# Wuziyi616/SlotDiffusion

Measured on AMD Instinct MI355X. Metric: train-step images/sec, 128x128 7-slot (DPM-Solver denoise-steps/sec in `denoise`), higher is better.
Workload: dtype bf16; 1 GPU; BASELINE configs[1]: img_based SlotDiffusion, CLEVRTex 128x128, 7 slots: train step = slot encoder + frozen VQ-VAE encode + q-sample + UNet eps + MSE, backward, clip, Adam (dropout 0.1); batch_per_gpu=64, hip_graph=True, parallelism=dp1

## Files before the change

### include/sdmi.h

```cpp
#ifndef SDMI_H_
#define SDMI_H_

#ifdef __cplusplus
extern "C" {
#endif

#define SDMI_VERSION 100

enum { SDMI_F32 = 0, SDMI_BF16 = 1, SDMI_FP8 = 2  };
enum { SDMI_ACT_NONE = 0, SDMI_ACT_RELU = 1, SDMI_ACT_SILU = 2, SDMI_ACT_GELU = 3 };
enum { SDMI_OK = 0, SDMI_EINVAL = -1, SDMI_ELAUNCH = -2, SDMI_EUNSUPPORTED = -3 };

int sdmi_version(void);
const char* sdmi_last_error(void);

typedef struct {
  const void* a;
  const void* w;
  void* out;
  const float* bias;
  const float* rowvec;
  const void* residual;
  float* workspace;
  int dtype, out_dtype;
  int M, N, K;
  int lda, ldw, ldc, ldr;
  int B, H, W, Cin, Ho, Wo, KH, KW, stride, pad_t, pad_l, ups;
  int act;
  float alpha;
  int bias_m;
  int split_k;
  int batch;
  int ldrv;
  int zins;
  long long sa, sw, sc, sr;
  int oH, oW, osy, osx, ooy, oox;
  const float* ln_colsum;
  float ln_eps;
  int geglu;
  const void* a2;
  int lda2, K1;
  const void* a3;
  int lda3, K2;
  int softmax8;
  long long s_colsum, s_bias;
  void* out2;
  int ldc2;
  int defer_epilogue;
  float* gn_part;
  int gn_groups;
  const float* alpha_dev;
  int parity4;
} SdmiGemmArgs;
int sdmi_igemm(const SdmiGemmArgs* a, void* stream);
int sdmi_igemm_split_plan(const SdmiGemmArgs* a, void* stream);
int sdmi_splitk_finish(const SdmiGemmArgs* a, void* stream);
enum {
  SDMI_ROUTE_NONE = 0,
  SDMI_ROUTE_CFG = 1,
  SDMI_ROUTE_DMA = 2,
  SDMI_ROUTE_SYM = 3,
  SDMI_ROUTE_HALO = 4,
  SDMI_ROUTE_C64 = 5
};
int sdmi_igemm_last_route(void);

typedef struct {
  const void* a;
  const void* dy;
  float* dw;
  float* dbias;
  float* workspace;
  int dtype;
  int M, N, K, lda, ldy;
  int B, H, W, Cin, Ho, Wo, KH, KW, stride, pad_t, pad_l, ups;
  int splits;
  int accumulate;
  int defer_fold;
} SdmiWgradArgs;
int sdmi_wgrad(const SdmiWgradArgs* a, void* stream);
enum {
  SDMI_WGRAD_KERNEL_IGEMM = 0,
  SDMI_WGRAD_KERNEL_C64 = 1,
  SDMI_WGRAD_KERNEL_HALO = 2,
  SDMI_WGRAD_KERNEL_F32_T128 = 3,
  SDMI_WGRAD_KERNEL_F32_T64 = 4
};
int sdmi_wgrad_kernel(const SdmiWgradArgs* a, void* stream);
int sdmi_wgrad_route(const SdmiWgradArgs* a, void* stream);

typedef struct { const void* problems; int n; } SdmiWgradGroupArgs;
int sdmi_wgrad_group(const SdmiWgradGroupArgs* a, void* stream);
int sdmi_wgrad_fold_group(const SdmiWgradGroupArgs* a, void* stream);

typedef struct {
  const void* dgrad; const void* wgrad; const void* fold;
  int dgrad_cap, wgrad_tile;
} SdmiBwdPairArgs;
int sdmi_bwd_pair(const SdmiBwdPairArgs* a, void* stream);
int sdmi_bwd_pair_route(const SdmiBwdPairArgs* a, void* stream);

typedef struct {
  const void* x;
  void* y;
  const float* gamma;
  const float* beta;
  float* stats;
  float* partial;
  int dtype;
  int B, HW, C, groups;
  float eps;
  int act;
  int nsplit;
  const void* residual;
  float drop_p;
  long long drop_seed;
  const long long* drop_seed_dev;
  void* y8;
  float y8_scale;
  const void* x2;
  int C1;
  const float* part;
  int part_splits;
  float part_alpha;
  const float* part_bias;
  const float* part_rowvec;
  int part_ldrv;
  const void* part_residual;
  void* raw_out;
} SdmiGroupNormArgs;
int sdmi_groupnorm_stats(const SdmiGroupNormArgs* a, void* stream);
int sdmi_groupnorm_apply(const SdmiGroupNormArgs* a, void* stream);
int sdmi_groupnorm(const SdmiGroupNormArgs* a, void* stream);

typedef struct {
  const void* x;
  const void* dy;
  void* dx;
  const float* gamma;
  const float* beta;
  const float* stats;
  float* dgamma;
  float* dbeta;
  float* partial;
  int dtype;
  int B, HW, C, groups;
  int act;
  int nsplit;
  const void* residual;
  void* dresidual;
  int accumulate;
  const void* dextra0;
  const void* dextra1;
  float drop_p;
  long long drop_seed;
  const long long* drop_seed_dev;
  float* dxsum;
  int ld_dxsum;
  int defer_colsum;
} SdmiGroupNormBwdArgs;
int sdmi_groupnorm_bwd(const SdmiGroupNormBwdArgs* a, void* stream);
int sdmi_groupnorm_bwd_fused(const SdmiGroupNormBwdArgs* a, void* unused);
int sdmi_groupnorm_bwd_entries(const SdmiGroupNormBwdArgs* a, void* stream);

typedef struct {
  const void* x; void* y; const float* gamma; const float* beta;
  float* stats;
  int dtype; int rows, C, ldx, ldy; float eps;
} SdmiLayerNormArgs;
int sdmi_layernorm(const SdmiLayerNormArgs* a, void* stream);

typedef struct {
  const void* x; const void* dy; void* dx; const float* gamma; const float* stats;
  float* dgamma; float* dbeta;
  float* partial;
  int dtype; int rows, C; int nblk; int accumulate;
  const void* dextra;
  int defer_colsum;
} SdmiLayerNormBwdArgs;
int sdmi_layernorm_bwd(const SdmiLayerNormBwdArgs* a, void* stream);

typedef struct { const float* partial; float* out0; float* out1; int nblk, C; } SdmiColsumItem;
typedef struct { const void* items; int n; } SdmiColsumGroupArgs;
int sdmi_colsum_group(const SdmiColsumGroupArgs* a, void* stream);


typedef struct {
  const void* q; const void* k; const void* v; void* out; float* lse;
  int dtype; int B, heads, Sq, Skv; int ldq, ldk, ldv, ldo; float scale;
  int head_dim;
} SdmiAttnArgs;
int sdmi_attention(const SdmiAttnArgs* a, void* stream);

typedef struct {
  const void* q; const void* k; const void* v; const void* out; const void* dout; const float* lse;
  void* dq; void* dk; void* dv;
  int dtype; int B, heads, Sq, Skv; int ldq, ldk, ldv, ldo; float scale;
  int head_dim;
} SdmiAttnBwdArgs;
int sdmi_attention_bwd(const SdmiAttnBwdArgs* a, void* stream);

typedef struct { void* x; int dtype; int rows, cols, ld; float scale; } SdmiSoftmaxArgs;
int sdmi_softmax_rows(const SdmiSoftmaxArgs* a, void* stream);

typedef struct {
  const void* k; const void* v;
  const float* slots_in;
  float* slots_out;
  float* seg;
  const float *lnq_g, *lnq_b, *wq;
  const float *w_ih, *w_hh, *b_ih, *b_hh;
  const float *lnm_g, *lnm_b, *w1, *b1, *w2, *b2;
  float* trace;
  int dtype; int B, M, N, D, Hid, iters, ldkv; long long slots_bstride; float eps, scale;
} SdmiSlotAttnArgs;
int sdmi_slot_attention(const SdmiSlotAttnArgs* a, void* stream);

typedef struct {
  const float* z; const float* codebook; long long* idx; float* zq;
  int R, dim, ldz, n_codes; float scale;
  const float* z2; float zc0, zc1, zdiv;
} SdmiVqArgs;
int sdmi_vq_nearest(const SdmiVqArgs* a, void* stream);

enum { SDMI_DPM_EPS = 0, SDMI_DPM_X0 = 1, SDMI_DPM_V = 2 };
enum { SDMI_DPM_UPD_NONE = 0, SDMI_DPM_UPD_FIRST = 1, SDMI_DPM_UPD_SINGLE = 2, SDMI_DPM_UPD_MULTI2 = 3,
       SDMI_DPM_UPD_MULTI3 = 4 };
typedef struct {
  const float* x; const float* out; const float* codebook;
  long long* idx; float* m0;
  const float* base; const float* h1; const float* h2; float* y;
  int R, n_codes, target, mode;
  float scale, sigma, alpha;
  float c0, c1, c2, c3, k0, k1, g, k2;
} SdmiDpmStepArgs;
int sdmi_dpm_step(const SdmiDpmStepArgs* a, void* stream);

typedef struct {
  const float* x; const float* out; const float* codebook;
  long long* idx; float* m0;
  int R, n_codes, target;
  float scale, sigma, alpha;
// ... 373 lines not shown
```

### slotdiffusion_amd/bwd.py

```python
import ctypes
from typing import NamedTuple, Optional

import torch

from . import _lib

_DT = {torch.float32: _lib.F32, torch.bfloat16: _lib.BF16}


def _p(t):
    return 0 if t is None else t.data_ptr()


def _st():
    return torch.cuda.current_stream().cuda_stream


def _cdiv(a, b):
    return (a + b - 1) // b


class LayerProblem(NamedTuple):
    is_conv: bool
    B: int
    H: int
    W: int
    Ho: int
    Wo: int
    Cin: int
    N: int
    K: int
    M: int
    kh: int
    kw: int
    stride: int
    pad: tuple
    ups: bool
    lda: int
    ldy: int
    dt: torch.dtype

    @classmethod
    def of(cls, x, dy, geom, dt, N):
        kh, kw, stride, pad, ups = geom
        Cin = x.shape[-1]
        if x.dim() == 4 and (kh, kw) != (0, 0):
            return cls.conv(x.shape[0], x.shape[1], x.shape[2], dy.shape[1], dy.shape[2], Cin, N, dy.shape[-1], kh, kw,
                            stride, pad, dt, ups)
        rows = x.numel() // Cin
        return cls(False, rows, 1, 1, 1, 1, Cin, N, Cin, rows, 1, 1, 1, (0, 0, 0, 0), False, x.stride(-2), dy.shape[-1], dt)

    @classmethod
    def conv(cls, B, H, W, Ho, Wo, Cin, N, ldy, kh, kw, stride, pad, dt, ups=False):
        return cls(True, B, H, W, Ho, Wo, Cin, N, kh * kw * Cin, B * Ho * Wo, kh, kw, stride, tuple(pad), bool(ups), Cin,
                   ldy, dt)

    @classmethod
    def transposed(cls, x, Cout, k, stride, pad):
        B, H, W, Cin = x.shape
        Ho = (H - 1) * stride - 2 * pad + k + (stride - 1)
        Wo = (W - 1) * stride - 2 * pad + k + (stride - 1)
        return cls.conv(B, Ho, Wo, H, W, Cout, Cin, Cin, k, k, stride, (pad,) * 4, x.dtype)

    @classmethod
    def upsampled(cls, x, Cout):
        B, H, W, Cin = x.shape
        return cls.conv(B, 2 * H, 2 * W, H, W, Cout, Cin, Cin, 4, 4, 2, (1, 1, 1, 1), x.dtype)

    def wgrad_fields(self):
        return dict(dtype=_DT[self.dt], M=self.M, N=self.N, K=self.K, lda=self.lda, ldy=self.ldy, B=self.B, H=self.H,
                    W=self.W, Cin=self.Cin, Ho=self.Ho, Wo=self.Wo, KH=self.kh, KW=self.kw, stride=self.stride,
                    pad_t=self.pad[0], pad_l=self.pad[2], ups=int(self.ups))

    def dgrad_fields(self):
        Hs, Ws = (2 * self.H, 2 * self.W) if self.ups else (self.H, self.W)
        kd = self.kh * self.kw * self.ldy
        return dict(dtype=_DT[self.dt], out_dtype=_DT[self.dt], M=self.B * Hs * Ws, N=self.Cin, K=kd, lda=self.ldy, ldw=kd,
                    ldc=self.Cin, B=self.B, H=self.Ho, W=self.Wo, Cin=self.ldy, Ho=Hs, Wo=Ws, KH=self.kh, KW=self.kw,
                    stride=1, pad_t=self.kh - 1 - self.pad[0], pad_l=self.kw - 1 - self.pad[2], ups=0, act=0, alpha=1.0,
                    batch=1, zins=(self.stride if self.stride > 1 else 0), ldr=self.Cin)

    def parity_dgrads(self):
        s, kh, kw, pad = self.stride, self.kh, self.kw, self.pad
        full = all(len(range((p + pd) % s, k, s)) > 0 for k, pd in ((kh, pad[0]), (kw, pad[2])) for p in range(s))
        subs = []
        for py in range(s):
            ay = (py + pad[0]) % s
            nky, hs = len(range(ay, kh, s)), len(range(py, self.H, s))
            for px in range(s):
                ax = (px + pad[2]) % s
                nkx, ws = len(range(ax, kw, s)), len(range(px, self.W, s))
                if nky == 0 or nkx == 0 or hs == 0 or ws == 0:
                    continue
                K = nky * nkx * self.ldy
                subs.append(((kh - 1 - ay) % s, (kw - 1 - ax) % s, dict(
                    dtype=_DT[self.dt], out_dtype=_DT[self.dt], M=self.B * hs * ws, N=self.Cin, K=K, lda=self.ldy, ldw=K,
                    ldc=self.Cin, B=self.B, H=self.Ho, W=self.Wo, Cin=self.ldy, Ho=hs, Wo=ws, KH=nky, KW=nkx, stride=1,
                    pad_t=(nky - 1) - (py + pad[0] - ay) // s, pad_l=(nkx - 1) - (px + pad[2] - ax) // s, ups=0, act=0,
                    alpha=1.0, batch=1, oH=self.H, oW=self.W, osy=s, osx=s, ooy=py, oox=px, ldr=self.Cin)))
        return full, subs


WG_TARGET, MIN_STEPS, MAX_SPLITS = 192, 8, 512
PAIR_SLOTS, PAIR_DGRAD, PAIR_MIN_STEPS, PAIR_WT64 = 512, 256, 8, 96
WQ_TARGET, WQ_MAX_SPLITS = 512.0, 64


class PairPlan(NamedTuple):
    wgrad_tile: int
    dgrad_cap: int
    splits: int


class LayerPlan(NamedTuple):
    path: str
    splits: int
    kernel: str
    pair: Optional[PairPlan]


def _mstep(P):
    return 64 if P.dt == torch.bfloat16 else 32


def standalone_splits(P):
    tiles = _cdiv(P.N, 128) * _cdiv(P.K, 128)
    return max(1, min(_cdiv(WG_TARGET, tiles), P.M // (MIN_STEPS * _mstep(P)), MAX_SPLITS))


def _standalone(P, n_cus, wgrad_halo):
    splits = 1 if P.M <= 16 * _mstep(P) else standalone_splits(P)
    same3x3 = (P.dt == torch.bfloat16 and P.is_conv and P.kh == 3 and P.kw == 3 and P.stride == 1 and not P.ups
               and P.pad == (1, 1, 1, 1))
    if (same3x3 and P.Cin == 64 and P.N == 64 and P.W % 64 == 0 and P.H % 4 == 0
            and P.B * (P.H // 4) * (P.W // 64) >= 2 * n_cus):
        return n_cus, 'c64'
    hw = P.H * P.W
    if (same3x3 and wgrad_halo and P.W in (16, 32, 64) and P.Cin % 64 == 0 and P.N % 64 == 0 and P.Ho == P.H
            and P.Wo == P.W and hw % 256 == 0 and (hw & (hw - 1)) == 0):
        pairs = (P.N // 64) * (P.Cin // 64)
        halo = min(n_cus // pairs, P.M // 256)
        if halo >= 2 and pairs * halo >= 128:
            return halo, 'halo'
    return splits, 'gemm'


def _pairable(P, direct, has_bias, bias_dst, dalias_cols):
    kh, kw, pad = P.kh, P.kw, P.pad
    same = P.is_conv and P.stride == 1 and not P.ups and P.Ho == P.H and P.Wo == P.W
    one = kh == 1 and kw == 1 and P.stride == 1 and not P.ups and pad[0] == 0 and pad[2] == 0
    kd = kh * kw * P.ldy
    bk = 64 if kd * 2 >= 512 else 32
    return (P.dt == torch.bfloat16 and direct and P.N > 64 and P.K > 64 and P.Cin > 64
            and (not has_bias or bias_dst) and P.Cin % 8 == 0 and P.ldy % 8 == 0
            and (one or (same and kh * kw <= 32 and P.ldy % bk == 0
                         and pad[0] == pad[1] == (kh - 1) // 2 and pad[2] == pad[3] == (kw - 1) // 2))
            and (dalias_cols is None or dalias_cols == P.Cin)
            and (P.M + (kh + 1) * P.W + 128) * max(P.lda, P.ldy, P.Cin) * 2 < (1 << 31) and P.N * kd * 2 < (1 << 31))


def _pair_plan(P, has_bias):
    Md, Nd, Kd = P.B * P.H * P.W, P.Cin, P.kh * P.kw * P.ldy
    t128 = _cdiv(Md, 128) * _cdiv(Nd, 128)
    shallow = P.kh == 1 and P.kw == 1 and Kd * 2 <= 512
    big = t128 >= 192 and not shallow
    tiles_d = t128 if big else _cdiv(Md, 64) * _cdiv(Nd, 64)
    steps = _cdiv(P.M, 64)

    def plan(wt, slots, min_steps):
        tn = _cdiv(P.N, wt)
        tiles_w = tn * _cdiv(P.K, wt) + (tn if has_bias else 0)
        n_d = min(tiles_d, PAIR_DGRAD)
        return tiles_w, n_d, max(1, min((slots - n_d) // tiles_w, steps // min_steps, 256))
    wt = 128
    tiles_w, n_d, splits = plan(128, PAIR_SLOTS, PAIR_MIN_STEPS)
    if not big and PAIR_WT64 and tiles_w * splits < PAIR_WT64:
        wt = 64
        tiles_w, n_d, splits = plan(64, PAIR_SLOTS * 3 // 2, max(2, PAIR_MIN_STEPS // 2))
    return PairPlan(wt, _cdiv(n_d, 8) * 8, splits)


def plan_layer(P, *, need_dx, direct, has_bias, bias_dst, dalias_cols, n_cus, pair_bwd=True, wgrad_halo=True):
    splits, kernel = _standalone(P, n_cus, wgrad_halo)
    if pair_bwd and need_dx and _pairable(P, direct, has_bias, bias_dst, dalias_cols):
        return LayerPlan('pair', splits, kernel, _pair_plan(P, has_bias))
    return LayerPlan('side', splits, kernel, None)


def plan_group(problems):
    tiles = [_cdiv(P.N, 128) * (_cdiv(P.K, 128) + (1 if bias else 0)) for P, bias in problems]
    steps = [_cdiv(P.M, 64) for P, _ in problems]
    total = float(sum(t * st for t, st in zip(tiles, steps)))
    return [max(1, min(max(1, int(round(WQ_TARGET * (t * st) / total / t))), st // MIN_STEPS, WQ_MAX_SPLITS))
            for t, st in zip(tiles, steps)]


class GradSchedule:
    N_SIDE = 4

    def __init__(self, overlap):
        self.overlap = overlap
        self._sides, self._side_of = [], {}
        self._keep = []
        self._pfold = None
        self._side_dst = {}
        self._cq, self._cq_after = [], []
        self._groups = 0
        self._join_queued = False

    def _side_stream(self, key):
        if not self.overlap:
            return None
        if not self._sides:
            self._sides = [torch.cuda.Stream() for _ in range(self.N_SIDE)]
        i = self._side_of.get(key)
        if i is None:
            i = self._side_of[key] = len(self._side_of) % self.N_SIDE
        return self._sides[i]

    def _fold_first(self, dst_ptrs=None):
        pf = self._pfold
        if pf is None:
            return
        if dst_ptrs is not None and pf[0]['dw'] not in dst_ptrs and (not pf[0]['dbias'] or pf[0]['dbias'] not in dst_ptrs):
            return
        self._pfold = None
        self._after_side_writers(pf[0]['dw'], pf[0]['dbias'])
        arr = _lib.struct_array('SdmiWgradArgs', [pf[0]])
        _lib.call('sdmi_wgrad_fold_group', _st(), problems=ctypes.addressof(arr), n=1)

    def _after_side_writers(self, *ptrs):
        for p_ in ptrs:
            side = self._side_dst.pop(p_, None) if p_ else None
            if side is not None:
                torch.cuda.current_stream().wait_stream(side)

    def _on_side(self, side, launch, dst_ptrs):
        if side is None:
            launch()
            return
        ev = torch.cuda.Event()
        ev.record()
        side.wait_event(ev)
        with torch.cuda.stream(side):
            launch()
        for p_ in dst_ptrs:
            if p_:
                self._side_dst[p_] = side

    def _ensure_join(self):
        if not self._join_queued:
            self._join_queued = True
            torch.autograd.Variable._execution_engine.queue_callback(self.join)

    def join_by_hand(self):
        self._join_queued = True

    def launch_pair(self, P, plan, dgrad, wgrad, device):
        N, K, splits = P.N, P.K, plan.splits
        self._fold_first((wgrad['dw'], wgrad['dbias']))
        self._after_side_writers(wgrad['dw'], wgrad['dbias'])
        ws = torch.empty((splits * (N * K + N),), dtype=torch.float32, device=device) if splits > 1 else None
        pf, self._pfold = self._pfold, None
        if pf is not None:
            self._after_side_writers(pf[0]['dw'], pf[0]['dbias'])
# ... 80 lines not shown
```

### slotdiffusion_amd/csrc/bwd_pair.hip

```cpp
#include "common.h"
#include "igemm_body.h"
#include "wgrad_body.h"

namespace {

struct PairGeom {
  int n_fold, n_wgrad, d_begin, n_dgrad;
  int w_tiles_n, w_tiles_k, w_per_split, w_mps;
  int d_tiles_m, d_tiles_n, d_ktps, d_hw_shift;
};

constexpr int pair_wg_lds(int wt) { return 2 * 64 * (wt * 2 + 64 + wt * 2 + 64); }

template <int BM, int BN, int BKB, int MODE, int WT>
__global__ __launch_bounds__(512) __attribute__((amdgpu_waves_per_eu(4, 4))) void bwd_pair_kernel(
    SdmiGemmArgs d, SdmiWgradArgs w, SdmiWgradArgs f, PairGeom g) {
  const int b = (int)blockIdx.x;
  if (b < g.n_fold) {
    wgrad_reduce_body<512>(f, b, g.n_fold);
    return;
  }
  if (b < g.n_fold + g.n_wgrad) {
    const int j = b - g.n_fold;
    const int xc = j & 7, q8 = g.n_wgrad >> 3, r8 = g.n_wgrad & 7;
// ... 2 lines not shown
    wgrad_tr_body<WT, WT, MODE>(w, g.w_tiles_n, g.w_tiles_k, g.w_mps, idx - split * g.w_per_split, split);
    return;
  }
  if (b < g.d_begin) return;
  igemm_body<bf16_t, BM, BN, BKB, MODE>(d, g.d_tiles_m, g.d_tiles_n, g.d_ktps, g.d_hw_shift, b - g.d_begin,
                                        g.n_dgrad, 0);
}

template <int BM, int BN, int BKB, int MODE, int WT>
int launch_pair(const SdmiGemmArgs& d, const SdmiWgradArgs& w, const SdmiWgradArgs* f, int dgrad_cap,
                int hw_shift, hipStream_t st) {
  constexpr int BK = BKB / 2;
  constexpr int d_lds = 2 * (BM + BN) * (BKB + 16);
  constexpr int smem = d_lds > pair_wg_lds(WT) ? d_lds : pair_wg_lds(WT);
  auto kern = bwd_pair_kernel<BM, BN, BKB, MODE, WT>;
  SDMI_OPTIN_LDS(kern, smem, "bwd_pair");
  PairGeom g;
  SdmiWgradArgs fz = {};
  if (f) {
    fz = *f;
    const long long v4 = (long long)f->N * f->K / 4 * wgrad_fold_lanes(f->splits);
    long long nf = (v4 + 512 * 4 - 1) / (512 * 4);
    g.n_fold = (int)(nf < 1 ? 1 : (nf > 128 ? 128 : nf));
  } else {
    g.n_fold = 0;
  }
  g.w_tiles_n = (w.N + WT - 1) / WT;
  g.w_tiles_k = (w.K + WT - 1) / WT;
  g.w_per_split = g.w_tiles_n * g.w_tiles_k + (w.dbias ? g.w_tiles_n : 0);
  int mps = (w.M + w.splits - 1) / w.splits;
  g.w_mps = (mps + 63) / 64 * 64;
  g.n_wgrad = g.w_per_split * w.splits;
  g.d_begin = (g.n_fold + g.n_wgrad + 7) & ~7;
  g.d_tiles_m = (d.M + BM - 1) / BM;
  g.d_tiles_n = (d.N + BN - 1) / BN;
  g.d_ktps = (d.K + BK - 1) / BK;
  g.d_hw_shift = hw_shift;
  const int tiles = g.d_tiles_m * g.d_tiles_n;
  constexpr int SLOTS = smem <= 49152 ? 768 : 512;
  int cap = dgrad_cap > 0 ? dgrad_cap : SLOTS - g.d_begin;
  cap = cap < 64 ? 64 : (cap > SLOTS ? SLOTS : cap);
  cap &= ~7;
  g.n_dgrad = tiles <= cap ? tiles : cap;
  SdmiGemmArgs q = d;
  q.split_k = 1;
  hipLaunchKernelGGL(kern, dim3(g.d_begin + g.n_dgrad), dim3(512), smem, st, q, w, fz, g);
  return sdmi_check_launch("bwd_pair");
}

struct PairRoute { int bm, bn, bkb, mode, wt, hw_shift; };

#define PAIR_REQUIRE(cond, msg)              \
  do {                                       \
    if (!(cond)) {                           \
      sdmi_set_error("%s: %s", who, msg);    \
      return SDMI_EINVAL;                    \
    }                                        \
  } while (0)
int pair_route(const SdmiBwdPairArgs* a, PairRoute& route, const char* who) {
  PAIR_REQUIRE(a && a->dgrad && a->wgrad, "null pointer");
  const SdmiGemmArgs& d = *(const SdmiGemmArgs*)a->dgrad;
  const SdmiWgradArgs& w = *(const SdmiWgradArgs*)a->wgrad;
  const SdmiWgradArgs* f = (const SdmiWgradArgs*)a->fold;
  PAIR_REQUIRE(d.a && d.w && d.out && w.a && w.dy && w.dw, "null operand");
  PAIR_REQUIRE(d.dtype == SDMI_BF16 && d.out_dtype == SDMI_BF16 && w.dtype == SDMI_BF16, "bf16 operands only");
  const bool d1x1 = d.KH == 1 && d.KW == 1 && d.stride == 1 && d.pad_t == 0 && d.pad_l == 0 && !d.ups && d.zins <= 1;
  const bool dplain = !d1x1 && !d.ups && d.zins <= 1 && d.stride == 1;
  PAIR_REQUIRE(d1x1 || dplain, "data gradient: 1x1 or plain stride-1 convolution");
  PAIR_REQUIRE(d.M > 0 && d.N > 64 && d.K > 0 && d.K == d.KH * d.KW * d.Cin && d.M == d.B * d.Ho * d.Wo, "bad dgrad geometry");
  PAIR_REQUIRE(d.Cin % 8 == 0 && d.lda % 8 == 0 && d.ldw % 8 == 0 && ((uintptr_t)d.a & 15) == 0 && ((uintptr_t)d.w & 15) == 0,
               "dgrad operands must keep 16-byte vectors");
  PAIR_REQUIRE(!d.a2 && !d.ln_colsum && !d.geglu && !d.softmax8 && !d.out2 && d.osy == 0 && !(d.batch > 1) && !d.rowvec &&
               !d.bias_m && d.split_k <= 1, "data gradient: plain epilogue (alpha, bias, residual) only");
  const long long a_bytes = ((long long)d.B * d.H * d.W + (long long)(d.KH + 1) * d.W) * d.lda * 2;
  PAIR_REQUIRE(a_bytes < (1ll << 31) && (long long)d.N * d.ldw * 2 < (1ll << 31), "dgrad operands beyond 31-bit offsets");
  const bool w1x1 = w.KH == 1 && w.KW == 1 && w.stride == 1 && w.pad_t == 0 && w.pad_l == 0 && !w.ups && w.H == w.Ho &&
                    w.W == w.Wo;
  const bool wlin = !w1x1 && !w.ups && w.stride == 1 && w.H == w.Ho && w.W == w.Wo;
  PAIR_REQUIRE((d1x1 && w1x1) || (dplain && wlin), "both gradients must be 1x1, or both a stride-1 same-size convolution");
  PAIR_REQUIRE(w.N > 64 && w.K > 64 && w.K == w.KH * w.KW * w.Cin && w.M == w.B * w.Ho * w.Wo && w.Cin % 8 == 0 &&
               w.lda % 8 == 0 && w.ldy % 8 == 0, "bad wgrad geometry");
  PAIR_REQUIRE(w.splits >= 1 && (w.splits == 1 || w.workspace), "splits > 1 need a workspace");
  const long long mps = ((long long)w.M + w.splits - 1) / w.splits + 64;
  const long long ld = w.lda > w.ldy ? w.lda : w.ldy;
  PAIR_REQUIRE((mps + (long long)(w.KH + 1) * w.W + 64) * ld * 2 < (1ll << 31), "wgrad split beyond 31-bit offsets");
  if (f) PAIR_REQUIRE(f->dw && f->workspace && f->splits > 1 && f->N > 0 && f->K > 0 && ((long long)f->N * f->K) % 4 == 0 &&
                      f->dw != w.dw && (!f->dbias || f->dbias != w.dbias), "bad fold problem (or it targets this layer's dW)");
  int hw_shift = -1;
  {
    const int hw = d.Ho * d.Wo;
    if (hw > 0 && (hw & (hw - 1)) == 0) {
      hw_shift = 0;
      while ((1 << hw_shift) < hw) ++hw_shift;
    }
  }
  const long long t128 = (long long)((d.M + 127) / 128) * ((d.N + 127) / 128);
  bool big = t128 >= 192;
  const int kbytes = d.K * 2;
  if (d1x1 && kbytes <= 512) big = false;
  const bool wide = kbytes >= 512;
  const int bk = (wide ? 128 : 64) / 2;
  if (!d1x1) PAIR_REQUIRE(d.KH * d.KW <= 32 && d.Cin % bk == 0, "convolution data gradient: K tiles must lie inside one filter tap");
  PAIR_REQUIRE(a->wgrad_tile == 0 || a->wgrad_tile == 128 || (a->wgrad_tile == 64 && !big),
               "wgrad_tile: 128, or 64 next to 64 x 64 data-gradient tiles");
  const int t = big ? 128 : 64;
  route = {t, t, wide ? 128 : 64, d1x1 ? 1 : 2, a->wgrad_tile == 64 ? 64 : 128, hw_shift};
  return 0;
}
#undef PAIR_REQUIRE

}

extern "C" int sdmi_bwd_pair(const SdmiBwdPairArgs* a, void* stream) {
  PairRoute r;
  if (const int rc = pair_route(a, r, __func__)) return rc;
  const SdmiGemmArgs& d = *(const SdmiGemmArgs*)a->dgrad;
  const SdmiWgradArgs& w = *(const SdmiWgradArgs*)a->wgrad;
  const SdmiWgradArgs* f = (const SdmiWgradArgs*)a->fold;
  hipStream_t st = (hipStream_t)stream;
#define PAIR_GO(BM, BN, BKB, WT)                                                                       \
  return r.mode == 1 ? launch_pair<BM, BN, BKB, 1, WT>(d, w, f, a->dgrad_cap, r.hw_shift, st)           \
                     : launch_pair<BM, BN, BKB, 2, WT>(d, w, f, a->dgrad_cap, r.hw_shift, st)
  if (r.bm == 128) {
    if (r.bkb == 128) PAIR_GO(128, 128, 128, 128);
    PAIR_GO(128, 128, 64, 128);
  }
  if (r.wt == 64) {
    if (r.bkb == 128) PAIR_GO(64, 64, 128, 64);
    PAIR_GO(64, 64, 64, 64);
  }
  if (r.bkb == 128) PAIR_GO(64, 64, 128, 128);
  PAIR_GO(64, 64, 64, 128);
#undef PAIR_GO
}

extern "C" int sdmi_bwd_pair_route(const SdmiBwdPairArgs* a, void*) {
  PairRoute r;
  if (const int rc = pair_route(a, r, __func__)) return rc;
  return (r.bm / 64) | (r.bn / 64) << 3 | (r.bkb / 64) << 6 | r.mode << 9 | (r.wt / 64) << 12;
}
```

### slotdiffusion_amd/csrc/norm_bwd.hip

```cpp
#include "common.h"
#include "gn_geom.h"
#include "gn_dev.h"
#include <type_traits>

namespace {

__device__ __forceinline__ int next_pow2(int v) {
  int p = 1;
  while (p < v) p <<= 1;
  return p;
}

template <typename T>
__global__ __launch_bounds__(256) void gn_bwd_stats_kernel(SdmiGroupNormBwdArgs p) {
  constexpr int VEC = Elem<T>::VEC;
  __shared__ float part[256][VEC][2];
  const int b = blockIdx.y, split = blockIdx.x;
  const int CV = p.C / VEC, CVp = next_pow2(CV);
  const int R = 256 / CVp;
  const int cv = threadIdx.x % CVp, r0 = threadIdx.x / CVp;
  const int rows_per = (p.HW + p.nsplit - 1) / p.nsplit;
  const int row_begin = split * rows_per;
  int row_end = row_begin + rows_per;
  if (row_end > p.HW) row_end = p.HW;
  const int cpg = p.C / p.groups;
  float A[VEC], Bv[VEC];
#pragma unroll
  for (int j = 0; j < VEC; ++j) A[j] = Bv[j] = 0.f;
  if (cv < CV) {
    float mu[VEC], rs[VEC], ga[VEC], be[VEC];
#pragma unroll
    for (int j = 0; j < VEC; ++j) {
      const int c = cv * VEC + j, g = c / cpg;
      mu[j] = p.stats[(b * p.groups + g) * 2];
      rs[j] = p.stats[(b * p.groups + g) * 2 + 1];
      ga[j] = p.gamma[c];
      be[j] = p.beta[c];
    }
    const long long base = (long long)b * p.HW * p.C + cv * VEC;
    const T* xb = (const T*)p.x + base;
    const T* db = (const T*)p.dy + base;
    const T* rb = p.residual ? (const T*)p.residual + base : nullptr;
    const bool drop = p.drop_p > 0.f;
    const unsigned long long dseed = drop ? sdmi_drop_seed(p.drop_seed, p.drop_seed_dev) : 0ULL;
    const unsigned thr16 = (unsigned)(p.drop_p * 65536.f);
    const float dinv = 1.f / (1.f - p.drop_p);
    for (int row = row_begin + r0; row < row_end; row += R) {
      const long long o = (long long)row * p.C;
      float x[VEC], dy[VEC], rr[VEC];
      unpack16<T>(*reinterpret_cast<const uint4*>(xb + o), x);
      unpack16<T>(*reinterpret_cast<const uint4*>(db + o), dy);
      if (drop) sdmi_drop_apply<VEC>(dy, dseed, (base + o) / VEC, thr16, dinv);
      if (rb) unpack16<T>(*reinterpret_cast<const uint4*>(rb + o), rr);
#pragma unroll
      for (int j = 0; j < VEC; ++j) {
        const float xh = (x[j] - mu[j]) * rs[j];
        const float z = xh * ga[j] + be[j] + (rb ? rr[j] : 0.f);
        const float dz = dy[j] * act_grad<sizeof(T) == 2>(z, p.act);
        A[j] += dz;
        Bv[j] += dz * xh;
      }
    }
  }
#pragma unroll
  for (int j = 0; j < VEC; ++j) { part[threadIdx.x][j][0] = A[j]; part[threadIdx.x][j][1] = Bv[j]; }
  __syncthreads();
  if (r0 == 0 && cv < CV) {
#pragma unroll
    for (int j = 0; j < VEC; ++j) {
      double sa = 0.0, sb = 0.0;
      for (int r = 0; r < R; ++r) { sa += part[r * CVp + cv][j][0]; sb += part[r * CVp + cv][j][1]; }
      float* q = p.partial + ((((long long)b * p.nsplit + split) * p.C) + cv * VEC + j) * 2;
      q[0] = (float)sa;
      q[1] = (float)sb;
    }
  }
}

template <typename T, int THREADS, int NV>
__global__ __launch_bounds__(THREADS) void gn_bwd_fused_kernel(SdmiGroupNormBwdArgs p) {
  constexpr int VEC = Elem<T>::VEC;
  extern __shared__ __attribute__((aligned(16))) float gnb_smem[];
  const int b = blockIdx.x;
  const int S = gridDim.y, sidx = blockIdx.y;
  const int CV = p.C / VEC / S, CVp = next_pow2(CV);
  const int c_lo = sidx * CV * VEC;
  const int R = THREADS / CVp;
  const int RR = CVp < 64 ? THREADS / 64 : R;
  float (*part)[VEC][2] = reinterpret_cast<float (*)[VEC][2]>(gnb_smem);
  float (*gsum)[2] = reinterpret_cast<float (*)[2]>(gnb_smem + RR * CVp * VEC * 2);
  const int cv = threadIdx.x % CVp, r0 = threadIdx.x / CVp;
  const bool act_c = cv < CV;
  const int cpg = p.C / p.groups;
  const int gs = p.groups / S;
  float mu[VEC], rs[VEC], ga[VEC], be[VEC];
#pragma unroll
  for (int j = 0; j < VEC; ++j) {
    const int c = c_lo + (act_c ? cv : 0) * VEC + j, g = c / cpg;
    mu[j] = p.stats[(b * p.groups + g) * 2];
    rs[j] = p.stats[(b * p.groups + g) * 2 + 1];
    ga[j] = p.gamma[c];
    be[j] = p.beta[c];
  }
  const long long base = (long long)b * p.HW * p.C + c_lo + (act_c ? cv : 0) * VEC;
  const T* xb = (const T*)p.x + base;
  const T* db = (const T*)p.dy + base;
  const T* rb = p.residual ? (const T*)p.residual + base : nullptr;
  uint4 xr[NV], dr[NV];
#pragma unroll
  for (int i = 0; i < NV; ++i) {
    const int row = r0 + i * R;
    if (act_c && row < p.HW) {
      xr[i] = *reinterpret_cast<const uint4*>(xb + (long long)row * p.C);
      dr[i] = *reinterpret_cast<const uint4*>(db + (long long)row * p.C);
    }
  }
  float A[VEC], Bv[VEC];
#pragma unroll
  for (int j = 0; j < VEC; ++j) A[j] = Bv[j] = 0.f;
  const bool drop = p.drop_p > 0.f;
  const unsigned long long dseed = drop ? sdmi_drop_seed(p.drop_seed, p.drop_seed_dev) : 0ULL;
  const unsigned thr16 = (unsigned)(p.drop_p * 65536.f);
  const float dinv = 1.f / (1.f - p.drop_p);
#pragma unroll
  for (int i = 0; i < NV; ++i) {
    const int row = r0 + i * R;
    if (act_c && row < p.HW) {
      float x[VEC], dy[VEC], rr[VEC];
      unpack16<T>(xr[i], x);
      unpack16<T>(dr[i], dy);
      if (drop) sdmi_drop_apply<VEC>(dy, dseed, (base + (long long)row * p.C) / VEC, thr16, dinv);
      if (rb) unpack16<T>(*reinterpret_cast<const uint4*>(rb + (long long)row * p.C), rr);
#pragma unroll
      for (int j = 0; j < VEC; ++j) {
        const float xh = (x[j] - mu[j]) * rs[j];
        const float z = xh * ga[j] + be[j] + (rb ? rr[j] : 0.f);
        const float dz = dy[j] * act_grad<sizeof(T) == 2>(z, p.act);
        dy[j] = dz;
        A[j] += dz;
        Bv[j] += dz * xh;
      }
      dr[i] = pack16<T>(dy);
    }
  }
  for (int off = CVp; off < 64; off <<= 1) {
#pragma unroll
    for (int j = 0; j < VEC; ++j) {
      A[j] += __shfl_xor(A[j], off, 64);
      Bv[j] += __shfl_xor(Bv[j], off, 64);
    }
  }
  if (CVp >= 64 || (int)(threadIdx.x & 63) < CVp) {
    const int slot = CVp < 64 ? (threadIdx.x >> 6) * CVp + cv : threadIdx.x;
#pragma unroll
    for (int j = 0; j < VEC; ++j) { part[slot][j][0] = A[j]; part[slot][j][1] = Bv[j]; }
  }
  __syncthreads();
  if (r0 == 0 && act_c) {
#pragma unroll
    for (int j = 0; j < VEC; ++j) {
      double sa = 0.0, sb = 0.0;
      for (int r = 0; r < RR; ++r) { sa += part[r * CVp + cv][j][0]; sb += part[r * CVp + cv][j][1]; }
      part[cv][j][0] = (float)sa;
      part[cv][j][1] = (float)sb;
      float* q = p.partial + (((long long)b * p.C) + c_lo + cv * VEC + j) * 2;
      q[0] = (float)sa;
      q[1] = (float)sb;
    }
  }
  __syncthreads();
  for (int g = threadIdx.x; g < gs; g += THREADS) {
    double s1 = 0.0, s2 = 0.0;
    for (int c = g * cpg; c < (g + 1) * cpg; ++c) {
      s1 += (double)p.gamma[c_lo + c] * part[c / VEC][c % VEC][0];
      s2 += (double)p.gamma[c_lo + c] * part[c / VEC][c % VEC][1];
    }
    gsum[g][0] = (float)s1;
    gsum[g][1] = (float)s2;
  }
  __syncthreads();
  const float inv_n = 1.f / ((float)p.HW * (float)cpg);
  float sd[VEC];
#pragma unroll
  for (int j = 0; j < VEC; ++j) sd[j] = 0.f;
  if (act_c) {
  float s1[VEC], s2[VEC];
#pragma unroll
  for (int j = 0; j < VEC; ++j) {
    const int g = (cv * VEC + j) / cpg;
    s1[j] = gsum[g][0] * inv_n;
    s2[j] = gsum[g][1] * inv_n;
  }
  T* dxb = (T*)p.dx + base;
  T* drb = p.dresidual ? (T*)p.dresidual + base : nullptr;
  const T* e0 = p.dextra0 ? (const T*)p.dextra0 + base : nullptr;
  const T* e1 = p.dextra1 ? (const T*)p.dextra1 + base : nullptr;
#pragma unroll
  for (int i = 0; i < NV; ++i) {
    const int row = r0 + i * R;
    if (row < p.HW) {
      const long long o = (long long)row * p.C;
      float x[VEC], dz[VEC], dx[VEC];
      unpack16<T>(xr[i], x);
      unpack16<T>(dr[i], dz);
#pragma unroll
      for (int j = 0; j < VEC; ++j) {
        const float xh = (x[j] - mu[j]) * rs[j];
        dx[j] = rs[j] * (ga[j] * dz[j] - (s1[j] + xh * s2[j]));
      }
      if (e0) {
        float ex[VEC];
        unpack16<T>(*reinterpret_cast<const uint4*>(e0 + o), ex);
#pragma unroll
        for (int j = 0; j < VEC; ++j) dx[j] += ex[j];
      }
      if (e1) {
        float ex[VEC];
        unpack16<T>(*reinterpret_cast<const uint4*>(e1 + o), ex);
#pragma unroll
        for (int j = 0; j < VEC; ++j) dx[j] += ex[j];
      }
#pragma unroll
      for (int j = 0; j < VEC; ++j) sd[j] += dx[j];
      *reinterpret_cast<uint4*>(dxb + o) = pack16<T>(dx);
      if (drb) *reinterpret_cast<uint4*>(drb + o) = dr[i];
    }
  }
  }
  if (p.dxsum) {
    for (int off = CVp; off < 64; off <<= 1) {
#pragma unroll
      for (int j = 0; j < VEC; ++j) sd[j] += __shfl_xor(sd[j], off, 64);
    }
    __syncthreads();
    if (CVp >= 64 || (int)(threadIdx.x & 63) < CVp) {
      const int slot = CVp < 64 ? (threadIdx.x >> 6) * CVp + cv : threadIdx.x;
#pragma unroll
      for (int j = 0; j < VEC; ++j) part[slot][j][0] = sd[j];
    }
    __syncthreads();
    if (r0 == 0 && act_c) {
#pragma unroll
      for (int j = 0; j < VEC; ++j) {
        float t = 0.f;
        for (int r = 0; r < RR; ++r) t += part[r * CVp + cv][j][0];
        p.dxsum[(long long)b * p.ld_dxsum + c_lo + cv * VEC + j] = t;
      }
    }
  }
}

template <typename T, int THREADS, int NV>
__global__ __launch_bounds__(THREADS) void gn_bwd_fused2_kernel(SdmiGroupNormBwdArgs p) {
  constexpr int VEC = Elem<T>::VEC;
  constexpr int VSH = VEC == 8 ? 3 : 2;
  extern __shared__ __attribute__((aligned(16))) float gnb_smem[];
  const int b = blockIdx.x;
  const int S = gridDim.y, sidx = blockIdx.y;
  const int CV = p.C / VEC / S;
  const int csh = CV <= 1 ? 0 : 32 - __builtin_clz(CV - 1);
  const int CVp = 1 << csh;
  const int c_lo = sidx * CV * VEC;
  const int R = THREADS >> csh;
  const int RR = CVp < 64 ? THREADS / 64 : R;
  float4* part = reinterpret_cast<float4*>(gnb_smem);
  double* colsum = reinterpret_cast<double*>(gnb_smem + RR * CVp * 4);
  float (*chpart)[VEC][2] = reinterpret_cast<float (*)[VEC][2]>(gnb_smem + RR * CVp * 4 + CVp * 8);
  const int tid = threadIdx.x;
  const int cv = tid & (CVp - 1), r0 = tid >> csh;
  const bool act_c = cv < CV;
  const int cvc = act_c ? cv : 0;
  const int cpg = p.C / p.groups;
  const int cl0 = cvc * VEC;
  const int g0 = cl0 / cpg;
  const int bnd = (g0 + 1) * cpg - cl0;
  const long long base = (long long)b * p.HW * p.C + c_lo + cl0;
  const T* xb = (const T*)p.x + base;
  const T* db = (const T*)p.dy + base;
  const T* rb = p.residual ? (const T*)p.residual + base : nullptr;
  uint4 xr[NV], dr[NV];
#pragma unroll
  for (int i = 0; i < NV; ++i) {
    const int row = r0 + i * R;
    if (act_c && row < p.HW) {
      xr[i] = *reinterpret_cast<const uint4*>(xb + (long long)row * p.C);
      dr[i] = *reinterpret_cast<const uint4*>(db + (long long)row * p.C);
    }
  }
  const int gg = b * p.groups + sidx * (p.groups / S) + g0;
  const float2 st0 = *reinterpret_cast<const float2*>(p.stats + gg * 2);
  const float2 st1 = bnd < VEC ? *reinterpret_cast<const float2*>(p.stats + gg * 2 + 2) : st0;
  float ga[VEC], be[VEC];
  load_fvec<VEC>(p.gamma + c_lo + cl0, ga);
  load_fvec<VEC>(p.beta + c_lo + cl0, be);
#define GNB_MU(j) ((j) < bnd ? st0.x : st1.x)
#define GNB_RS(j) ((j) < bnd ? st0.y : st1.y)
  float A[VEC], Bv[VEC];
#pragma unroll
  for (int j = 0; j < VEC; ++j) A[j] = Bv[j] = 0.f;
  const bool drop = p.drop_p > 0.f;
  const unsigned long long dseed = drop ? sdmi_drop_seed(p.drop_seed, p.drop_seed_dev) : 0ULL;
  const unsigned thr16 = (unsigned)(p.drop_p * 65536.f);
  const float dinv = 1.f / (1.f - p.drop_p);
  auto first = [&](auto actc) __attribute__((always_inline)) {
    constexpr int ACT = decltype(actc)::value;
#pragma unroll
    for (int i = 0; i < NV; ++i) {
      const int row = r0 + i * R;
      if (act_c && row < p.HW) {
        float x[VEC], dy[VEC], rr[VEC];
        unpack16<T>(xr[i], x);
        unpack16<T>(dr[i], dy);
        if (drop) sdmi_drop_apply<VEC>(dy, dseed, (base + (long long)row * p.C) / VEC, thr16, dinv);
        if (rb) unpack16<T>(*reinterpret_cast<const uint4*>(rb + (long long)row * p.C), rr);
#pragma unroll
        for (int j = 0; j < VEC; ++j) {
          const float xh = (x[j] - GNB_MU(j)) * GNB_RS(j);
          const float z = xh * ga[j] + be[j] + (rb ? rr[j] : 0.f);
          const float dz = dy[j] * act_grad<sizeof(T) == 2>(z, ACT);
          dy[j] = dz;
          A[j] += dz;
          Bv[j] += dz * xh;
        }
        dr[i] = pack16<T>(dy);
      }
    }
  };
  if (p.act == SDMI_ACT_SILU) first(std::integral_constant<int, SDMI_ACT_SILU>{});
  else if (p.act == SDMI_ACT_RELU) first(std::integral_constant<int, SDMI_ACT_RELU>{});
  else if (p.act == SDMI_ACT_GELU) first(std::integral_constant<int, SDMI_ACT_GELU>{});
  else first(std::integral_constant<int, SDMI_ACT_NONE>{});
  float a0 = 0.f, q0 = 0.f, a1 = 0.f, q1 = 0.f;
#pragma unroll
  for (int j = 0; j < VEC; ++j) {
    const bool lo = j < bnd;
    const float ta = ga[j] * A[j], tb = ga[j] * Bv[j];
    a0 += lo ? ta : 0.f;
    q0 += lo ? tb : 0.f;
    a1 += lo ? 0.f : ta;
    q1 += lo ? 0.f : tb;
  }
  if (CVp < 64) {
    a0 = col_allreduce(a0, CVp);
    q0 = col_allreduce(q0, CVp);
    a1 = col_allreduce(a1, CVp);
    q1 = col_allreduce(q1, CVp);
#pragma unroll
    for (int j = 0; j < VEC; ++j) { A[j] = col_allreduce(A[j], CVp); Bv[j] = col_allreduce(Bv[j], CVp); }
    if ((tid & 63) < CVp) {
      const int e = (tid >> 6) * CVp + cv;
      part[e] = make_float4(a0, q0, a1, q1);
#pragma unroll
      for (int j = 0; j < VEC; ++j) { chpart[e][j][0] = A[j]; chpart[e][j][1] = Bv[j]; }
    }
  } else {
    part[tid] = make_float4(a0, q0, a1, q1);
#pragma unroll
    for (int j = 0; j < VEC; ++j) { chpart[tid][j][0] = A[j]; chpart[tid][j][1] = Bv[j]; }
  }
  __syncthreads();
  if (tid < CVp) {
    double d0 = 0.0, d1 = 0.0, d2 = 0.0, d3 = 0.0;
    for (int r = 0; r < RR; ++r) {
      const float4 v = part[r * CVp + tid];
      d0 += (double)v.x; d1 += (double)v.y; d2 += (double)v.z; d3 += (double)v.w;
    }
    colsum[tid * 4 + 0] = d0; colsum[tid * 4 + 1] = d1; colsum[tid * 4 + 2] = d2; colsum[tid * 4 + 3] = d3;
  }
  for (int u = THREADS - 1 - tid; u < CVp * VEC * 2; u += THREADS) {
    const int ccv = u / (VEC * 2), j = (u >> 1) & (VEC - 1), which = u & 1;
    if (ccv < CV) {
      double sa = 0.0;
      for (int r = 0; r < RR; ++r) sa += (double)chpart[r * CVp + ccv][j][which];
      p.partial[(((long long)b * p.C) + c_lo + ccv * VEC + j) * 2 + which] = (float)sa;
    }
  }
  __syncthreads();
  const float inv_n = 1.f / ((float)p.HW * (float)cpg);
  float s1_[2], s2_[2];
#pragma unroll
  for (int k = 0; k < 2; ++k) {
    if (k == 1 && bnd >= VEC) { s1_[1] = s1_[0]; s2_[1] = s2_[0]; break; }
    const int f = (g0 + k) * cpg, l = f + cpg - 1;
    const int ca = f >> VSH, cb = l >> VSH;
    double sm = 0.0, sq = 0.0;
    for (int c = ca; c <= cb; ++c) {
      const int o = c * 4 + (((c << VSH) >= f) ? 0 : 2);
      sm += colsum[o];
      sq += colsum[o + 1];
    }
    s1_[k] = (float)sm * inv_n;
    s2_[k] = (float)sq * inv_n;
  }
  float sd[VEC];
#pragma unroll
  for (int j = 0; j < VEC; ++j) sd[j] = 0.f;
  if (act_c) {
    T* dxb = (T*)p.dx + base;
    T* drb = p.dresidual ? (T*)p.dresidual + base : nullptr;
    const T* e0 = p.dextra0 ? (const T*)p.dextra0 + base : nullptr;
    const T* e1 = p.dextra1 ? (const T*)p.dextra1 + base : nullptr;
#pragma unroll
    for (int i = 0; i < NV; ++i) {
      const int row = r0 + i * R;
      if (row < p.HW) {
        const long long o = (long long)row * p.C;
        float x[VEC], dz[VEC], dx[VEC];
        unpack16<T>(xr[i], x);
        unpack16<T>(dr[i], dz);
#pragma unroll
        for (int j = 0; j < VEC; ++j) {
          const float rsj = GNB_RS(j);
          const float xh = (x[j] - GNB_MU(j)) * rsj;
          dx[j] = rsj * (ga[j] * dz[j] - ((j < bnd ? s1_[0] : s1_[1]) + xh * (j < bnd ? s2_[0] : s2_[1])));
        }
        if (e0) {
          float ex[VEC];
          unpack16<T>(*reinterpret_cast<const uint4*>(e0 + o), ex);
#pragma unroll
          for (int j = 0; j < VEC; ++j) dx[j] += ex[j];
        }
        if (e1) {
          float ex[VEC];
          unpack16<T>(*reinterpret_cast<const uint4*>(e1 + o), ex);
#pragma unroll
          for (int j = 0; j < VEC; ++j) dx[j] += ex[j];
        }
#pragma unroll
        for (int j = 0; j < VEC; ++j) sd[j] += dx[j];
        *reinterpret_cast<uint4*>(dxb + o) = pack16<T>(dx);
        if (drb) *reinterpret_cast<uint4*>(drb + o) = dr[i];
      }
    }
  }
#undef GNB_MU
#undef GNB_RS
  if (p.dxsum) {
    if (CVp < 64) {
#pragma unroll
      for (int j = 0; j < VEC; ++j) sd[j] = col_allreduce(sd[j], CVp);
    }
    __syncthreads();
    if (CVp >= 64 || (tid & 63) < CVp) {
      const int e = CVp < 64 ? (tid >> 6) * CVp + cv : tid;
#pragma unroll
      for (int j = 0; j < VEC; ++j) chpart[e][j][0] = sd[j];
    }
    __syncthreads();
    for (int u = tid; u < CVp * VEC; u += THREADS) {
      const int ccv = u / VEC, j = u & (VEC - 1);
      if (ccv < CV) {
        float t = 0.f;
        for (int r = 0; r < RR; ++r) t += chpart[r * CVp + ccv][j][0];
        p.dxsum[(long long)b * p.ld_dxsum + c_lo + ccv * VEC + j] = t;
      }
    }
  }
}

__global__ __launch_bounds__(256) void pair_colsum_kernel(const float* partial, int nblk, int C,
                                                          float* out0, float* out1,
                                                          int accumulate) {
  __shared__ float red[16][16][2];
  const int cl = threadIdx.x & 15, kg = threadIdx.x >> 4;
  const int c = blockIdx.x * 16 + cl;
  float s0 = 0.f, s1 = 0.f;
  if (c < C) {
    const float2* q = reinterpret_cast<const float2*>(partial) + c;
    int k = kg;
    for (; k + 48 < nblk; k += 64) {
      const float2 v0 = q[(long long)k * C], v1 = q[(long long)(k + 16) * C];
      const float2 v2 = q[(long long)(k + 32) * C], v3 = q[(long long)(k + 48) * C];
      s0 += (v0.x + v1.x) + (v2.x + v3.x);
      s1 += (v0.y + v1.y) + (v2.y + v3.y);
    }
    for (; k < nblk; k += 16) {
      const float2 v = q[(long long)k * C];
      s0 += v.x;
      s1 += v.y;
    }
  }
  red[kg][cl][0] = s0;
  red[kg][cl][1] = s1;
  __syncthreads();
  if (kg == 0 && c < C) {
    float a = 0.f, b = 0.f;
#pragma unroll
    for (int k = 0; k < 16; ++k) { a += red[k][cl][0]; b += red[k][cl][1]; }
    out0[c] = (accumulate ? out0[c] : 0.f) + a;
    out1[c] = (accumulate ? out1[c] : 0.f) + b;
  }
}

constexpr int CS_MAX = 64;
struct ColsumGroup { int n; SdmiColsumItem it[CS_MAX]; };
__global__ __launch_bounds__(256) void colsum_group_kernel(ColsumGroup g) {
  const SdmiColsumItem& q_ = g.it[blockIdx.y];
  const int C = q_.C, nblk = q_.nblk;
  if ((int)blockIdx.x * 16 >= C) return;
  __shared__ float red[16][16][2];
  const int cl = threadIdx.x & 15, kg = threadIdx.x >> 4;
  const int c = blockIdx.x * 16 + cl;
  float s0 = 0.f, s1 = 0.f;
  const bool two = q_.out1 != nullptr;
  if (c < C && !two) {
    const float* q = q_.partial + c;
    for (int k = kg; k < nblk; k += 16) s0 += q[(long long)k * C];
  } else if (c < C) {
    const float2* q = reinterpret_cast<const float2*>(q_.partial) + c;
    int k = kg;
    for (; k + 48 < nblk; k += 64) {
      const float2 v0 = q[(long long)k * C], v1 = q[(long long)(k + 16) * C];
      const float2 v2 = q[(long long)(k + 32) * C], v3 = q[(long long)(k + 48) * C];
      s0 += (v0.x + v1.x) + (v2.x + v3.x);
      s1 += (v0.y + v1.y) + (v2.y + v3.y);
    }
    for (; k < nblk; k += 16) {
      const float2 v = q[(long long)k * C];
      s0 += v.x;
      s1 += v.y;
    }
  }
  red[kg][cl][0] = s0;
  red[kg][cl][1] = s1;
  __syncthreads();
  if (kg == 0 && c < C) {
    float a = 0.f, b = 0.f;
#pragma unroll
    for (int k = 0; k < 16; ++k) { a += red[k][cl][0]; b += red[k][cl][1]; }
    q_.out0[c] += a;
    if (two) q_.out1[c] += b;
  }
}

template <typename T>
__global__ __launch_bounds__(256) void gn_bwd_apply_kernel(SdmiGroupNormBwdArgs p, int rows_per) {
  constexpr int VEC = Elem<T>::VEC;
  __shared__ float gsum[256][2];
  const int b = blockIdx.y;
  const int cpg = p.C / p.groups;
  {
    const int l8 = threadIdx.x & 7;
    const int ne = cpg * p.nsplit;
    for (int g = threadIdx.x >> 3; g < p.groups; g += 32) {
      double s1 = 0.0, s2 = 0.0;
      for (int e = l8; e < ne; e += 8) {
        const int k = e / cpg, c = g * cpg + (e - k * cpg);
        const float2 v = reinterpret_cast<const float2*>(p.partial)[((long long)b * p.nsplit + k) * p.C + c];
        const double ga = (double)p.gamma[c];
        s1 += ga * v.x;
        s2 += ga * v.y;
      }
      for (int off = 1; off < 8; off <<= 1) {
        s1 += __shfl_xor(s1, off, 64);
        s2 += __shfl_xor(s2, off, 64);
      }
      if (l8 == 0) { gsum[g][0] = (float)s1; gsum[g][1] = (float)s2; }
    }
  }
  __syncthreads();
  const int CV = p.C / VEC, CVp = next_pow2(CV);
  const int R = 256 / CVp;
  const int cv = threadIdx.x % CVp, r0 = threadIdx.x / CVp;
  if (cv >= CV) return;
  const int row_begin = blockIdx.x * rows_per;
  int row_end = row_begin + rows_per;
  if (row_end > p.HW) row_end = p.HW;
  const float inv_n = 1.f / ((float)p.HW * (float)cpg);
  float mu[VEC], rs[VEC], ga[VEC], be[VEC], s1[VEC], s2[VEC];
#pragma unroll
  for (int j = 0; j < VEC; ++j) {
    const int c = cv * VEC + j, g = c / cpg;
    mu[j] = p.stats[(b * p.groups + g) * 2];
    rs[j] = p.stats[(b * p.groups + g) * 2 + 1];
    ga[j] = p.gamma[c];
    be[j] = p.beta[c];
    s1[j] = gsum[g][0] * inv_n;
    s2[j] = gsum[g][1] * inv_n;
  }
  const long long base = (long long)b * p.HW * p.C + cv * VEC;
  const T* xb = (const T*)p.x + base;
  const T* db = (const T*)p.dy + base;
  const T* rb = p.residual ? (const T*)p.residual + base : nullptr;
  T* dxb = (T*)p.dx + base;
  T* drb = p.dresidual ? (T*)p.dresidual + base : nullptr;
  const T* e0 = p.dextra0 ? (const T*)p.dextra0 + base : nullptr;
  const T* e1 = p.dextra1 ? (const T*)p.dextra1 + base : nullptr;
  const bool drop = p.drop_p > 0.f;
  const unsigned long long dseed = drop ? sdmi_drop_seed(p.drop_seed, p.drop_seed_dev) : 0ULL;
  const unsigned thr16 = (unsigned)(p.drop_p * 65536.f);
  const float dinv = 1.f / (1.f - p.drop_p);
  for (int row = row_begin + r0; row < row_end; row += R) {
    const long long o = (long long)row * p.C;
    float x[VEC], dy[VEC], rr[VEC], dx[VEC], dz[VEC];
    unpack16<T>(*reinterpret_cast<const uint4*>(xb + o), x);
    unpack16<T>(*reinterpret_cast<const uint4*>(db + o), dy);
    if (drop) sdmi_drop_apply<VEC>(dy, dseed, (base + o) / VEC, thr16, dinv);
    if (rb) unpack16<T>(*reinterpret_cast<const uint4*>(rb + o), rr);
#pragma unroll
    for (int j = 0; j < VEC; ++j) {
      const float xh = (x[j] - mu[j]) * rs[j];
      const float z = xh * ga[j] + be[j] + (rb ? rr[j] : 0.f);
      dz[j] = dy[j] * act_grad<sizeof(T) == 2>(z, p.act);
      dx[j] = rs[j] * (ga[j] * dz[j] - (s1[j] + xh * s2[j]));
    }
    if (e0) {
      float ex[VEC];
      unpack16<T>(*reinterpret_cast<const uint4*>(e0 + o), ex);
#pragma unroll
      for (int j = 0; j < VEC; ++j) dx[j] += ex[j];
    }
    if (e1) {
      float ex[VEC];
      unpack16<T>(*reinterpret_cast<const uint4*>(e1 + o), ex);
#pragma unroll
      for (int j = 0; j < VEC; ++j) dx[j] += ex[j];
    }
    *reinterpret_cast<uint4*>(dxb + o) = pack16<T>(dx);
    if (drb) *reinterpret_cast<uint4*>(drb + o) = pack16<T>(dz);
  }
}

template <typename T, int VPL>
__global__ __launch_bounds__(256) void ln_bwd_kernel(SdmiLayerNormBwdArgs p, int rows_per_blk,
                                                     int LPR) {
  constexpr int VEC = Elem<T>::VEC;
  __shared__ float red[4][1024][2];
  const int lane = threadIdx.x & 63, wave = threadIdx.x >> 6;
  const int sub = lane & (LPR - 1), slot = lane / LPR, RW = 64 / LPR;
  const int CV = p.C / VEC;
  const int row0 = blockIdx.x * rows_per_blk;
  int row1 = row0 + rows_per_blk;
  if (row1 > p.rows) row1 = p.rows;
  float ga[VPL][VEC], dg[VPL][VEC], dbt[VPL][VEC];
  bool act[VPL];
#pragma unroll
  for (int i = 0; i < VPL; ++i) {
    const int cv = sub + i * LPR;
    act[i] = cv < CV;
#pragma unroll
    for (int j = 0; j < VEC; ++j) {
      ga[i][j] = act[i] ? p.gamma[cv * VEC + j] : 0.f;
      dg[i][j] = dbt[i][j] = 0.f;
    }
  }
  const float invC = 1.f / (float)p.C;
  uint4 xq[VPL], dq[VPL];
  float mean_n = 0.f, rstd_n = 1.f;
  auto fetch = [&](int rbase) __attribute__((always_inline)) {
    const int row = rbase + slot;
    const long long rr = (row < row1) ? row : row0;
    const T* x = (const T*)p.x + rr * p.C;
    const T* dy = (const T*)p.dy + rr * p.C;
    mean_n = p.stats[rr * 2];
    rstd_n = p.stats[rr * 2 + 1];
#pragma unroll
    for (int i = 0; i < VPL; ++i) {
      const int cc = act[i] ? sub + i * LPR : 0;
      xq[i] = *reinterpret_cast<const uint4*>(x + cc * VEC);
      dq[i] = *reinterpret_cast<const uint4*>(dy + cc * VEC);
    }
  };
  if (row0 + wave * RW < row1) fetch(row0 + wave * RW);
  for (int rbase = row0 + wave * RW; rbase < row1; rbase += 4 * RW) {
    const int row = rbase + slot;
    const bool rok = row < row1;
    const long long ro = (long long)(rok ? row : row0) * p.C;
    float xh[VPL][VEC], dxh[VPL][VEC];
    float s1 = 0.f, s2 = 0.f;
    const float mean = mean_n, rstd = rstd_n;
    uint4 xc[VPL], dc[VPL];
#pragma unroll
    for (int i = 0; i < VPL; ++i) { xc[i] = xq[i]; dc[i] = dq[i]; }
    const T* ex = p.dextra ? (const T*)p.dextra + ro : nullptr;
    uint4 eq[VPL];
    if (ex) {
#pragma unroll
      for (int i = 0; i < VPL; ++i) eq[i] = *reinterpret_cast<const uint4*>(ex + (act[i] ? sub + i * LPR : 0) * VEC);
    }
    if (rbase + 4 * RW < row1) fetch(rbase + 4 * RW);
#pragma unroll
    for (int i = 0; i < VPL; ++i) {
      float xv[VEC], dv[VEC];
      unpack16<T>(xc[i], xv);
      unpack16<T>(dc[i], dv);
#pragma unroll
      for (int j = 0; j < VEC; ++j) {
        const float d = (act[i] && rok) ? dv[j] : 0.f;
        xh[i][j] = (xv[j] - mean) * rstd;
        dxh[i][j] = d * ga[i][j];
        dg[i][j] += d * xh[i][j];
        dbt[i][j] += d;
        s1 += dxh[i][j];
        s2 += dxh[i][j] * xh[i][j];
      }
    }
    for (int off = 1; off < LPR; off <<= 1) {
      s1 += __shfl_xor(s1, off, 64);
      s2 += __shfl_xor(s2, off, 64);
    }
    s1 *= invC;
    s2 *= invC;
    if (rok) {
      T* dx = (T*)p.dx + ro;
#pragma unroll
      for (int i = 0; i < VPL; ++i) {
        if (!act[i]) continue;
        float o[VEC];
#pragma unroll
        for (int j = 0; j < VEC; ++j) o[j] = rstd * (dxh[i][j] - s1 - xh[i][j] * s2);
        if (ex) {
          float ev[VEC];
          unpack16<T>(eq[i], ev);
#pragma unroll
          for (int j = 0; j < VEC; ++j) o[j] += ev[j];
        }
        *reinterpret_cast<uint4*>(dx + (sub + i * LPR) * VEC) = pack16<T>(o);
      }
    }
  }
  for (int off = LPR; off < 64; off <<= 1) {
#pragma unroll
    for (int i = 0; i < VPL; ++i)
#pragma unroll
      for (int j = 0; j < VEC; ++j) {
        dg[i][j] += __shfl_xor(dg[i][j], off, 64);
        dbt[i][j] += __shfl_xor(dbt[i][j], off, 64);
      }
  }
  if (slot == 0) {
#pragma unroll
    for (int i = 0; i < VPL; ++i)
      if (act[i]) {
#pragma unroll
        for (int j = 0; j < VEC; ++j) {
          const int c = (sub + i * LPR) * VEC + j;
          red[wave][c][0] = dg[i][j];
          red[wave][c][1] = dbt[i][j];
        }
      }
  }
  __syncthreads();
  for (int c = threadIdx.x; c < p.C; c += 256) {
    float* q = p.partial + ((long long)blockIdx.x * p.C + c) * 2;
    q[0] = (red[0][c][0] + red[1][c][0]) + (red[2][c][0] + red[3][c][0]);
    q[1] = (red[0][c][1] + red[1][c][1]) + (red[2][c][1] + red[3][c][1]);
  }
}
}

extern "C" int sdmi_groupnorm_bwd_fused(const SdmiGroupNormBwdArgs* a, void*) {
  if (!a || a->C <= 0 || a->groups <= 0) return 0;
  const int vec = a->dtype == SDMI_BF16 ? 8 : 4;
  int nv_of_T[3] = {16, 16, a->dtype == SDMI_BF16 ? 4 : 8};
  return gn_pick(a->B, a->HW, a->C, a->groups, vec, nv_of_T).T ? 1 : 0;
}

extern "C" int sdmi_groupnorm_bwd_entries(const SdmiGroupNormBwdArgs* a, void*) {
  if (!a || a->C <= 0 || a->groups <= 0) return 0;
  const int vec = a->dtype == SDMI_BF16 ? 8 : 4;
  int nv_of_T[3] = {16, 16, a->dtype == SDMI_BF16 ? 4 : 8};
  const GnGeom gg = gn_pick(a->B, a->HW, a->C, a->groups, vec, nv_of_T);
  return gg.T ? a->B : a->B * a->nsplit;
}

extern "C" int sdmi_groupnorm_bwd(const SdmiGroupNormBwdArgs* a, void* stream) {
  SDMI_REQUIRE(a && a->x && a->dy && a->dx && a->gamma && a->beta && a->stats && a->dgamma &&
                   a->dbeta && a->partial, "null pointer");
  const int vec = a->dtype == SDMI_BF16 ? 8 : 4;
  SDMI_REQUIRE(a->C % vec == 0 && a->C <= 1024, "C must be a vector multiple <= 1024");
  SDMI_REQUIRE(a->groups > 0 && a->C % a->groups == 0 && a->nsplit >= 1, "bad groups/nsplit");
  hipStream_t st = (hipStream_t)stream;
  dim3 g1(a->nsplit, a->B);
  const long long row_bytes = (long long)a->C * (a->dtype == SDMI_BF16 ? 2 : 4);
  int rows_per = (int)((32768 + row_bytes - 1) / row_bytes);
  if (rows_per < 4) rows_per = 4;
  if (rows_per > a->HW) rows_per = a->HW;
  dim3 g3((a->HW + rows_per - 1) / rows_per, a->B);
  {
    int nv_of_T[3] = {16, 16, a->dtype == SDMI_BF16 ? 4 : 8};
    const GnGeom gg = gn_pick(a->B, a->HW, a->C, a->groups, vec, nv_of_T);
    if (gg.T) {
      dim3 gf(a->B, gg.S);
      const int cv = a->C / vec / gg.S;
      int cvp = 1;
      while (cvp < cv) cvp <<= 1;
      const int RR = cvp < 64 ? gg.T / 64 : gg.T / cvp;
      const size_t smem = ((size_t)RR * cvp * vec * 2 + 2 * 256) * sizeof(float);
      constexpr int v2 = 1;
      const int cpg = a->C / a->groups;
      const bool two = v2 && (cpg * 2 == vec || cpg >= vec - 1) && (gg.T != 1024 || v2 >= 2) && gg.need <= 8;
      const size_t smem2 = (size_t)RR * cvp * (16 + vec * 8) + (size_t)cvp * 32;
#define GNB_GO(T_, TH, NV_)                                                                        \
  do {                                                                                             \
    if (two) {                                                                                     \
      SDMI_OPTIN_LDS((gn_bwd_fused2_kernel<T_, TH, NV_>), 96 * 1024, "groupnorm_bwd");             \
      hipLaunchKernelGGL((gn_bwd_fused2_kernel<T_, TH, NV_>), gf, dim3(TH), smem2, st, *a);        \
    } else {                                                                                       \
      SDMI_OPTIN_LDS((gn_bwd_fused_kernel<T_, TH, NV_>), 80 * 1024, "groupnorm_bwd");              \
      hipLaunchKernelGGL((gn_bwd_fused_kernel<T_, TH, NV_>), gf, dim3(TH), smem, st, *a);          \
    }                                                                                              \
  } while (0)
#define GNB_PICK(T_, TH)                                                                           \
  do {                                                                                             \
    if (gg.need <= 4) GNB_GO(T_, TH, 4); else if (gg.need <= 8) GNB_GO(T_, TH, 8); else GNB_GO(T_, TH, 16); \
  } while (0)
      if (a->dtype == SDMI_BF16) {
        if (gg.T == 1024) GNB_GO(bf16_t, 1024, 4); else if (gg.T == 512) GNB_PICK(bf16_t, 512); else GNB_PICK(bf16_t, 256);
      } else {
        if (gg.T == 1024) { if (gg.need <= 4) GNB_GO(float, 1024, 4); else GNB_GO(float, 1024, 8); }
        else if (gg.T == 512) GNB_PICK(float, 512); else GNB_PICK(float, 256);
      }
#undef GNB_PICK
#undef GNB_GO
      if (!a->defer_colsum)
        hipLaunchKernelGGL(pair_colsum_kernel, dim3((a->C + 15) / 16), dim3(256), 0, st, a->partial,
                           a->B, a->C, a->dbeta, a->dgamma, a->accumulate);
      return sdmi_check_launch("groupnorm_bwd (fused)");
    }
  }
  if (a->dtype == SDMI_BF16)
    hipLaunchKernelGGL(gn_bwd_stats_kernel<bf16_t>, g1, dim3(256), 0, st, *a);
  else
    hipLaunchKernelGGL(gn_bwd_stats_kernel<float>, g1, dim3(256), 0, st, *a);
  SDMI_REQUIRE(a->groups <= 256, "at most 256 groups");
  if (!a->defer_colsum)
    hipLaunchKernelGGL(pair_colsum_kernel, dim3((a->C + 15) / 16), dim3(256), 0, st, a->partial,
                       a->B * a->nsplit, a->C, a->dbeta, a->dgamma, a->accumulate);
  if (a->dtype == SDMI_BF16)
    hipLaunchKernelGGL(gn_bwd_apply_kernel<bf16_t>, g3, dim3(256), 0, st, *a, rows_per);
  else
    hipLaunchKernelGGL(gn_bwd_apply_kernel<float>, g3, dim3(256), 0, st, *a, rows_per);
  return sdmi_check_launch("groupnorm_bwd");
}

extern "C" int sdmi_layernorm_bwd(const SdmiLayerNormBwdArgs* a, void* stream) {
  SDMI_REQUIRE(a && a->x && a->dy && a->dx && a->gamma && a->stats && a->dgamma && a->dbeta &&
                   a->partial, "null pointer");
  SDMI_REQUIRE(a->C > 0 && a->C <= 1024 && a->nblk >= 1, "C <= 1024");
  hipStream_t st = (hipStream_t)stream;
  const int rows_per_blk = (a->rows + a->nblk - 1) / a->nblk;
  const int vec = a->dtype == SDMI_BF16 ? 8 : 4;
  SDMI_REQUIRE(a->C % vec == 0, "C must be a multiple of the 16-byte vector width");
  const int cv = a->C / vec;
  int lpr = 1;
  while (lpr < cv && lpr < 64) lpr <<= 1;
  const int vpl = (cv + 63) / 64;
#define LN_GO(T, V) \
  hipLaunchKernelGGL((ln_bwd_kernel<T, V>), dim3(a->nblk), dim3(256), 0, st, *a, rows_per_blk, lpr)
  if (a->dtype == SDMI_BF16) {
    if (vpl <= 1) LN_GO(bf16_t, 1); else LN_GO(bf16_t, 2);
  } else {
    if (vpl <= 1) LN_GO(float, 1); else if (vpl == 2) LN_GO(float, 2); else LN_GO(float, 4);
  }
// ... 22 lines not shown
```

### slotdiffusion_amd/csrc/wgrad.hip

```cpp
#include "common.h"
#include "wgrad_body.h"

namespace {

template <typename T> struct WCfg;
template <> struct WCfg<bf16_t> { [[maybe_unused]] static constexpr int MTB = 256; };
template <> struct WCfg<float> { static constexpr int MTB = 128; };

__device__ __forceinline__ void transpose_block(const u32x4 (&r)[8], u32x4 (&c)[8], bf16_t) {
#pragma unroll
  for (int n = 0; n < 8; ++n) {
#pragma unroll
    for (int e = 0; e < 4; ++e) {
      const unsigned a = r[2 * e][n >> 1], b = r[2 * e + 1][n >> 1];
      c[n][e] = __builtin_amdgcn_perm(b, a, (n & 1) ? 0x07060302u : 0x05040100u);
    }
  }
}
__device__ __forceinline__ void transpose_block(const u32x4 (&r)[4], u32x4 (&c)[4], float) {
#pragma unroll
  for (int n = 0; n < 4; ++n)
#pragma unroll
    for (int e = 0; e < 4; ++e) c[n][e] = r[e][n];
}
// ... 624 lines not shown
      const int tap = tp0 + 2 * u;
#pragma unroll
      for (int j = 0; j < 2; ++j)
#pragma unroll
        for (int r = 0; r < 16; ++r) {
          const int n = nb * 64 + chh * 32 + (r & 3) + 8 * (r >> 2) + row_l;
          ws[(long long)n * p.K + tap * p.Cin + cb * 64 + j * 32 + col] = acc[u][j][r];
        }
    }
  }
  if (!want_bias) return;
  __syncthreads();
  float* red = reinterpret_cast<float*>(smem);
#pragma unroll
  for (int j = 0; j < 8; ++j) red[tid * 8 + j] = bsum[j];
  __syncthreads();
  if (tid < 64) {
    const int c = tid >> 3, j = tid & 7;
    float sacc = 0.f;
    for (int r = 0; r < 32; ++r) sacc += red[(r * 8 + c) * 8 + j];
    p.workspace[(long long)nsplit * p.N * p.K + (long long)split * p.N + nb * 64 + tid] = sacc;
  }
}

template <int LOGW>
static int launch_wgrad3x3_halo(const SdmiWgradArgs& a, hipStream_t st) {
  constexpr int W = 1 << LOGW, HALO = (256 / W + 2) * (W + 2);
  constexpr int smem = (HALO + 256) * W33_PIX;
  auto kern = wgrad3x3_halo_kernel<LOGW>;
  SDMI_OPTIN_LDS(kern, smem, "wgrad (direct 3x3, halo)");
  const int ncb = a.Cin / 64, nnb = a.N / 64;
  hipLaunchKernelGGL(kern, dim3(a.splits, nnb * ncb), dim3(256), smem, st, a, ncb);
  return sdmi_check_launch("wgrad (direct 3x3, halo)");
}

static bool wgrad_is1x1(const SdmiWgradArgs& a) {
  return a.KH == 1 && a.KW == 1 && a.stride == 1 && a.pad_t == 0 && a.pad_l == 0 && !a.ups &&
         a.H == a.Ho && a.W == a.Wo;
}

struct WgradRoute {
  int family;
  int tn, tk;
  int mode;
  int logw;
};

WgradRoute select_wgrad_f32(const SdmiWgradArgs& a) {
  const long long wg128 = (long long)((a.N + 127) / 128) * ((a.K + 127) / 128) * a.splits;
  const bool small = a.N <= 64 || a.K <= 64 || wg128 < 96;
  const int t = small ? 64 : 128;
  return {small ? SDMI_WGRAD_KERNEL_F32_T64 : SDMI_WGRAD_KERNEL_F32_T128, t, t, wgrad_is1x1(a) ? 1 : 0, 0};
}

int dispatch_wgrad_f32(const SdmiWgradArgs& a, hipStream_t st) {
  const WgradRoute r = select_wgrad_f32(a);
  if (r.tn == 64)
    return r.mode ? launch_wgrad<float, 64, 64, true>(a, st)
                  : launch_wgrad<float, 64, 64, false>(a, st);
  return r.mode ? launch_wgrad<float, 128, 128, true>(a, st)
                : launch_wgrad<float, 128, 128, false>(a, st);
}

WgradRoute select_wgrad_bf16(const SdmiWgradArgs& a) {
  if (a.KH == 3 && a.KW == 3 && a.stride == 1 && a.pad_t == 1 && a.pad_l == 1 && !a.ups && a.Cin == 64 &&
      a.N == 64 && a.K == 576 && a.H == a.Ho && a.W == a.Wo && a.W % 64 == 0 && a.H % 4 == 0 && a.splits >= 2 &&
      (long long)a.B * (a.H / 4) * (a.W / 64) >= a.splits && (long long)a.B * a.H * a.W * (a.lda > a.ldy ? a.lda : a.ldy) < (1ll << 40))
    return {SDMI_WGRAD_KERNEL_C64, 0, 0, 0, 0};
  static int halo = -1;
  if (halo < 0) {
    const char* e = getenv("SDMI_WGRAD_HALO");
    halo = e ? atoi(e) : 1;
  }
  const int logw = a.W == 16 ? 4 : (a.W == 32 ? 5 : (a.W == 64 ? 6 : 0));
  const long long hw = (long long)a.H * a.W;
  if (halo && logw && a.KH == 3 && a.KW == 3 && a.stride == 1 && a.pad_t == 1 && a.pad_l == 1 && !a.ups && a.H == a.Ho &&
      a.W == a.Wo && a.Cin % 64 == 0 && a.N % 64 == 0 && a.K == 9 * a.Cin && hw % 256 == 0 && (hw & (hw - 1)) == 0 &&
      a.splits >= 2 && a.M / 256 >= a.splits && (a.N / 64) * (a.Cin / 64) * a.splits >= 128 &&
      (long long)a.M * (a.lda > a.ldy ? a.lda : a.ldy) < (1ll << 40))
    return {SDMI_WGRAD_KERNEL_HALO, 0, 0, 0, logw};
  const bool is1x1 = wgrad_is1x1(a);
  const bool lin = !is1x1 && !a.ups && a.stride == 1 && a.H == a.Ho && a.W == a.Wo;
  const long long mps = ((long long)a.M + a.splits - 1) / a.splits + 64;
  const long long ld = a.lda > a.ldy ? a.lda : a.ldy;
  const bool fits = (mps + (long long)(a.KH + 1) * a.W + 64) * ld * 2 < (1ll << 31);
  return {SDMI_WGRAD_KERNEL_IGEMM, a.N <= 64 ? 64 : 128, a.K <= 64 ? 64 : 128,
          is1x1 && fits ? 1 : (lin && fits ? 2 : 0), 0};
}

int dispatch_wgrad_bf16(const SdmiWgradArgs& a, hipStream_t st) {
  const WgradRoute r = select_wgrad_bf16(a);
  if (r.family == SDMI_WGRAD_KERNEL_C64) return launch_wgrad3x3_c64(a, st);
  if (r.family == SDMI_WGRAD_KERNEL_HALO)
    return r.logw == 4 ? launch_wgrad3x3_halo<4>(a, st) : (r.logw == 5 ? launch_wgrad3x3_halo<5>(a, st) : launch_wgrad3x3_halo<6>(a, st));
#define WG_TR(TN, TK)                                                              \
  (r.mode == 1   ? launch_wgrad_tr<TN, TK, 1>(a, st)                               \
   : r.mode == 2 ? launch_wgrad_tr<TN, TK, 2>(a, st) : launch_wgrad_tr<TN, TK, 0>(a, st))
  if (r.tn == 64) return r.tk == 64 ? WG_TR(64, 64) : WG_TR(64, 128);
  return r.tk == 64 ? WG_TR(128, 64) : WG_TR(128, 128);
#undef WG_TR
}

const char* wgrad_geometry_error(const SdmiWgradArgs& a) {
  if (a.dtype != SDMI_F32 && a.dtype != SDMI_BF16) return "bad dtype";
  const int vec = a.dtype == SDMI_BF16 ? 8 : 4;
  if (a.K != a.KH * a.KW * a.Cin) return "K != KH*KW*Cin";
  if (a.Cin % vec != 0 || a.lda % vec != 0 || a.ldy % vec != 0) return "Cin/lda/ldy must be multiples of the 16-byte vector width";
  if (a.M != a.B * a.Ho * a.Wo) return "M != B*Ho*Wo";
  if (a.splits < 1) return "splits";
  return nullptr;
}

}

extern "C" int sdmi_wgrad_group(const SdmiWgradGroupArgs* ga, void* stream) {
  SDMI_REQUIRE(ga && ga->problems && ga->n >= 1 && ga->n <= WG_MAX, "1 .. 16 problems");
  const SdmiWgradArgs* ps = (const SdmiWgradArgs*)ga->problems;
  hipStream_t st = (hipStream_t)stream;
  WgradGroup g;
  g.n = ga->n;
  int items = 0, red = 0;
  if (ps[0].dtype == SDMI_F32) {
    constexpr int MT = WCfg<float>::MTB / 4;
    for (int i = 0; i < ga->n; ++i) {
      const SdmiWgradArgs& a = ps[i];
      SDMI_REQUIRE(a.a && a.dy && a.dw, "null pointer");
      SDMI_REQUIRE(a.dtype == SDMI_F32 && wgrad_is1x1(a), "grouped wgrad: one dtype per group, 1x1 / linear problems");
      SDMI_REQUIRE(a.K == a.Cin && a.Cin % 4 == 0 && a.lda % 4 == 0 && a.ldy % 4 == 0 && a.M == a.B * a.Ho * a.Wo,
                   "bad geometry");
      SDMI_REQUIRE(a.splits >= 1 && (a.splits == 1 || a.workspace), "splits / workspace");
      g.p[i] = a;
      g.tiles_n[i] = (a.N + 63) / 64;
      g.tiles_k[i] = (a.K + 63) / 64;
      g.per_split[i] = g.tiles_n[i] * g.tiles_k[i] + (a.dbias ? g.tiles_n[i] : 0);
      const int mps = (a.M + a.splits - 1) / a.splits;
      g.mps[i] = (mps + MT - 1) / MT * MT;
      g.item_begin[i] = items;
      items += g.per_split[i] * a.splits;
      g.red_begin[i] = red;
      if (a.splits > 1) {
        long long blocks = wgrad_fold_blocks(a);
        red += (int)(blocks > 512 ? 512 : blocks);
      }
    }
    for (int i = ga->n; i <= WG_MAX; ++i) { g.item_begin[i] = items; g.red_begin[i] = red; }
    constexpr int smem32 = 2 * (64 + 64) * (WCfg<float>::MTB + 16);
    SDMI_OPTIN_LDS(wgrad_group_f32_kernel, smem32, "wgrad group (fp32)");
    hipLaunchKernelGGL(wgrad_group_f32_kernel, dim3(items), dim3(512), smem32, st, g);
    int rc = sdmi_check_launch("wgrad group (fp32)");
    if (rc || red == 0) return rc;
    hipLaunchKernelGGL(wgrad_group_reduce_kernel, dim3(red), dim3(256), 0, st, g);
    return sdmi_check_launch("wgrad group reduce");
  }
  for (int i = 0; i < ga->n; ++i) {
    const SdmiWgradArgs& a = ps[i];
    SDMI_REQUIRE(a.a && a.dy && a.dw, "null pointer");
    SDMI_REQUIRE(a.dtype == SDMI_BF16 && wgrad_is1x1(a) && a.N > 64 && a.K > 64,
                 "grouped wgrad: bf16 1x1 / linear problems with N, K > 64");
    SDMI_REQUIRE(a.K == a.Cin && a.Cin % 8 == 0 && a.lda % 8 == 0 && a.ldy % 8 == 0 && a.M == a.B * a.Ho * a.Wo,
                 "bad geometry");
    SDMI_REQUIRE(a.splits >= 1 && (a.splits == 1 || a.workspace), "splits / workspace");
    const long long mps_ = ((long long)a.M + a.splits - 1) / a.splits + 64;
    const long long ld = a.lda > a.ldy ? a.lda : a.ldy;
    SDMI_REQUIRE((mps_ + 64) * ld * 2 < (1ll << 31), "split too large for 31-bit offsets");
    g.p[i] = a;
    g.tiles_n[i] = (a.N + 127) / 128;
    g.tiles_k[i] = (a.K + 127) / 128;
    g.per_split[i] = g.tiles_n[i] * g.tiles_k[i] + (a.dbias ? g.tiles_n[i] : 0);
    int mps = (a.M + a.splits - 1) / a.splits;
    g.mps[i] = (mps + 63) / 64 * 64;
    g.item_begin[i] = items;
    items += g.per_split[i] * a.splits;
    g.red_begin[i] = red;
    if (a.splits > 1) {
      long long blocks = wgrad_fold_blocks(a);
      red += (int)(blocks > 512 ? 512 : blocks);
    }
  }
  for (int i = ga->n; i <= WG_MAX; ++i) { g.item_begin[i] = items; g.red_begin[i] = red; }
  constexpr int smem = 2 * 64 * (128 * 2 + 64 + 128 * 2 + 64);
  SDMI_OPTIN_LDS(wgrad_group_kernel, smem, "wgrad group");
  hipLaunchKernelGGL(wgrad_group_kernel, dim3(items), dim3(512), smem, st, g);
  int rc = sdmi_check_launch("wgrad group");
  if (rc || red == 0) return rc;
  hipLaunchKernelGGL(wgrad_group_reduce_kernel, dim3(red), dim3(256), 0, st, g);
  return sdmi_check_launch("wgrad group reduce");
}

extern "C" int sdmi_wgrad_fold_group(const SdmiWgradGroupArgs* ga, void* stream) {
  SDMI_REQUIRE(ga && ga->problems && ga->n >= 1 && ga->n <= WG_MAX, "1 .. 16 problems");
  const SdmiWgradArgs* ps = (const SdmiWgradArgs*)ga->problems;
  WgradGroup g;
  g.n = ga->n;
  int red = 0;
  for (int i = 0; i < ga->n; ++i) {
    SDMI_REQUIRE(ps[i].dw && ps[i].workspace && ps[i].splits > 1 && ps[i].N > 0 && ps[i].K > 0 &&
                 ((long long)ps[i].N * ps[i].K) % 4 == 0, "bad problem");
    g.p[i] = ps[i];
    g.item_begin[i] = 0;
    g.red_begin[i] = red;
    long long blocks = wgrad_fold_blocks(ps[i]);
    red += (int)(blocks > 512 ? 512 : blocks);
  }
  for (int i = ga->n; i <= WG_MAX; ++i) { g.item_begin[i] = 0; g.red_begin[i] = red; }
  hipLaunchKernelGGL(wgrad_group_reduce_kernel, dim3(red), dim3(256), 0, (hipStream_t)stream, g);
  return sdmi_check_launch("wgrad fold group");
}

extern "C" int sdmi_wgrad(const SdmiWgradArgs* a, void* stream) {
  SDMI_REQUIRE(a && a->a && a->dy && a->dw && a->workspace, "null pointer");
  const char* err = wgrad_geometry_error(*a);
  SDMI_REQUIRE(!err, err);
  hipStream_t st = (hipStream_t)stream;
  int rc;
  rc = a->dtype == SDMI_BF16 ? dispatch_wgrad_bf16(*a, st) : dispatch_wgrad_f32(*a, st);
  if (rc || a->splits == 1 || a->defer_fold) return rc;
  int blocks = (int)wgrad_fold_blocks(*a);
  if (blocks > 4096) blocks = 4096;
  hipLaunchKernelGGL(wgrad_reduce_kernel, dim3(blocks), dim3(256), 0, st, *a);
  return sdmi_check_launch("wgrad reduce");
}

extern "C" int sdmi_wgrad_kernel(const SdmiWgradArgs* a, void*) {
  SDMI_REQUIRE(a, "null pointer");
  const char* err = wgrad_geometry_error(*a);
  SDMI_REQUIRE(!err, err);
  return (a->dtype == SDMI_BF16 ? select_wgrad_bf16(*a) : select_wgrad_f32(*a)).family;
}

extern "C" int sdmi_wgrad_route(const SdmiWgradArgs* a, void*) {
  SDMI_REQUIRE(a, "null pointer");
  const char* err = wgrad_geometry_error(*a);
  SDMI_REQUIRE(!err, err);
  const WgradRoute r = a->dtype == SDMI_BF16 ? select_wgrad_bf16(*a) : select_wgrad_f32(*a);
  return r.family | (r.tn / 64) << 4 | (r.tk / 64) << 7 | r.mode << 10 | r.logw << 12;
}
```

### slotdiffusion_amd/csrc/wgrad_body.h

```cpp
#pragma once
#include "common.h"

namespace {

template <typename T, int TN>
__device__ __forceinline__ void bias_tile(const SdmiWgradArgs& p, int tile_n, int split,
                                          int m_per_split, char* smem) {
  constexpr int VEC = 16 / sizeof(T);
  constexpr int CV = TN / VEC, R = 256 / CV;
  float* red = reinterpret_cast<float*>(smem);
  const int tid = threadIdx.x;
  if (tid >= 256) return;
  const int cv = tid % CV, r0 = tid / CV;
  const int n = tile_n * TN + cv * VEC;
  const int m0 = split * m_per_split;
  int m1 = m0 + m_per_split;
  if (m1 > p.M) m1 = p.M;
  float acc[VEC];
#pragma unroll
  for (int j = 0; j < VEC; ++j) acc[j] = 0.f;
  if (n < p.N) {
    const T* base = (const T*)p.dy + n;
    int m = m0 + r0;
    for (; m + 3 * R < m1; m += 4 * R) {
      float f0[VEC], f1[VEC], f2[VEC], f3[VEC];
      unpack16<T>(*reinterpret_cast<const uint4*>(base + (long long)m * p.ldy), f0);
      unpack16<T>(*reinterpret_cast<const uint4*>(base + (long long)(m + R) * p.ldy), f1);
      unpack16<T>(*reinterpret_cast<const uint4*>(base + (long long)(m + 2 * R) * p.ldy), f2);
      unpack16<T>(*reinterpret_cast<const uint4*>(base + (long long)(m + 3 * R) * p.ldy), f3);
#pragma unroll
      for (int j = 0; j < VEC; ++j) acc[j] += (f0[j] + f1[j]) + (f2[j] + f3[j]);
    }
    for (; m < m1; m += R) {
      float f0[VEC];
      unpack16<T>(*reinterpret_cast<const uint4*>(base + (long long)m * p.ldy), f0);
#pragma unroll
      for (int j = 0; j < VEC; ++j) acc[j] += f0[j];
    }
  }
#pragma unroll
  for (int j = 0; j < VEC; ++j) red[tid * VEC + j] = acc[j];
  __syncthreads();
  if (tid < TN && tile_n * TN + tid < p.N) {
    const int c = tid / VEC, j = tid % VEC;
    float s = 0.f;
    for (int r = 0; r < R; ++r) s += red[(r * CV + c) * VEC + j];
    const int nn = tile_n * TN + tid;
    if (p.splits == 1)
      p.dbias[nn] = (p.accumulate ? p.dbias[nn] : 0.f) + s;
    else
      p.workspace[(long long)p.splits * p.N * p.K + (long long)split * p.N + nn] = s;
  }
}


typedef short s16x4 __attribute__((ext_vector_type(4)));
typedef short s16x8 __attribute__((ext_vector_type(8)));
#define SDMI_LDS_V4(p) ((__attribute__((address_space(3))) s16x4*)(p))

template <int TN, int TK, int MODE>
__device__ __forceinline__ void wgrad_tr_body(const SdmiWgradArgs& p, int tiles_n, int tiles_k,
                                              int m_per_split, int tile, int split_idx) {
  typedef bf16_t T;
  constexpr bool IS1X1 = MODE == 1;
  constexpr bool FAST = MODE != 0;
  constexpr int MT = 64;
  constexpr int PY = TN * 2 + 64, PA = TK * 2 + 64;
  constexpr int STAGE = MT * (PY + PA);
  constexpr int CHY = TN / 8, CHA = TK / 8;
  constexpr int Y_PER = MT * CHY / 256, A_PER = MT * CHA / 256;
  constexpr int RSY = 256 / CHY, RSA = 256 / CHA;
  constexpr int WTN = TN / 2, WTK = TK / 2;
  constexpr int FN = WTN / 32, FK = WTK / 32;

  extern __shared__ __attribute__((aligned(16))) char smem[];

  if (tile >= tiles_n * tiles_k) {
    bias_tile<T, TN>(p, tile - tiles_n * tiles_k, split_idx, m_per_split, smem);
    return;
  }
  const int tile_n = tile / tiles_k, tile_k = tile - tile_n * tiles_k;
  const int split = split_idx;
  const int n0 = tile_n * TN, k0 = tile_k * TK;
  const int m_begin = split * m_per_split;
  int m_end = m_begin + m_per_split;
  if (m_end > p.M) m_end = p.M;
  const int n_steps = m_begin < m_end ? (m_end - m_begin + MT - 1) / MT : 0;

  if (threadIdx.x >= 256) {
    const int tid = threadIdx.x - 256;
    const T* __restrict__ Ag = (const T*)p.a;
    const T* __restrict__ Yg = (const T*)p.dy;
    const int ycc = tid % CHY, yr0 = tid / CHY;
    const int acc_ = tid % CHA, ar0 = tid / CHA;
    const int yn = n0 + ycc * 8;
    const bool y_act = yn < p.N;
    const int ak = k0 + acc_ * 8;
    const bool a_act = ak < p.K;
    int a_ci = a_act ? ak : 0, a_kh = 0, a_kw = 0;
    int pb[A_PER], poy[A_PER], pox[A_PER];
    int adv_b = 0, adv_y = 0, adv_x = 0;
    if constexpr (!IS1X1) {
      const int tap = a_ci / p.Cin;
      a_ci -= tap * p.Cin;
      a_kh = tap / p.KW;
      a_kw = tap - a_kh * p.KW;
      const int HoWo = p.Ho * p.Wo;
#pragma unroll
      for (int i = 0; i < A_PER; ++i) {
        const int m = m_begin + ar0 + i * RSA;
        pb[i] = m / HoWo;
        const int rem = m - pb[i] * HoWo;
        poy[i] = rem / p.Wo;
        pox[i] = rem - poy[i] * p.Wo;
      }
      adv_b = MT / HoWo;
      const int rr = MT - adv_b * HoWo;
      adv_y = rr / p.Wo;
      adv_x = rr - adv_y * p.Wo;
    }
    const u32x4 zero4 = {0u, 0u, 0u, 0u};
    constexpr unsigned OOB = 0x80000000u;
    const long long a_bias = MODE == 2 ? (long long)p.pad_t * p.W + p.pad_l : 0;
    const __amdgpu_buffer_rsrc_t rsY = __builtin_amdgcn_make_buffer_rsrc(
        (void*)(Yg + (long long)m_begin * p.ldy), 0, (int)OOB, 0x00020000);
    const __amdgpu_buffer_rsrc_t rsA = __builtin_amdgcn_make_buffer_rsrc(
        (void*)(Ag + ((long long)m_begin - a_bias) * p.lda), 0, (int)OOB, 0x00020000);
    unsigned y_vo[Y_PER], a_vo[A_PER];
    int lw_sh = 0;
    if constexpr (FAST) {
#pragma unroll
      for (int i = 0; i < Y_PER; ++i)
        y_vo[i] = y_act ? ((unsigned)(yr0 + i * RSY) * (unsigned)p.ldy + yn) * 2u : OOB;
#pragma unroll
      for (int i = 0; i < A_PER; ++i) {
        const unsigned r = ar0 + i * RSA + (MODE == 2 ? a_kh * p.W + a_kw : 0);
        a_vo[i] = a_act ? (r * (unsigned)p.lda + a_ci) * 2u : OOB;
      }
      while ((1 << lw_sh) < p.W) ++lw_sh;
    }
    const bool pow2 = (p.H & (p.H - 1)) == 0 && (p.W & (p.W - 1)) == 0;

    auto issue = [&](int mt, u32x4 (&ry)[Y_PER], u32x4 (&ra)[A_PER], unsigned& mask)
                     __attribute__((always_inline)) {
      mask = 0;
      if constexpr (FAST) {
        const int rel = mt - m_begin;
        const bool tail = mt + MT > m_end;
        const unsigned so_y = (unsigned)rel * (unsigned)p.ldy * 2u;
        const unsigned so_a = (unsigned)rel * (unsigned)p.lda * 2u;
#pragma unroll
        for (int i = 0; i < Y_PER; ++i) {
          unsigned vo = y_vo[i];
          if (tail && mt + yr0 + i * RSY >= m_end) vo = OOB;
          ry[i] = __builtin_amdgcn_raw_buffer_load_b128(rsY, (int)vo, (int)so_y, 0);
        }
#pragma unroll
        for (int i = 0; i < A_PER; ++i) {
          unsigned vo = a_vo[i];
          const int m = mt + ar0 + i * RSA;
          if constexpr (MODE == 2) {
            int ox, oy;
            if (pow2) {
              ox = m & (p.W - 1);
              oy = (m >> lw_sh) & (p.H - 1);
            } else {
              ox = pox[i];
              oy = poy[i];
              pox[i] += adv_x;
              poy[i] += adv_y;
              if (pox[i] >= p.Wo) { pox[i] -= p.Wo; ++poy[i]; }
              if (poy[i] >= p.Ho) poy[i] -= p.Ho;
            }
            const bool bad = (unsigned)(oy + a_kh - p.pad_t) >= (unsigned)p.H ||
                             (unsigned)(ox + a_kw - p.pad_l) >= (unsigned)p.W;
            vo = bad ? OOB : vo;
          }
          if (tail && m >= m_end) vo = OOB;
          ra[i] = __builtin_amdgcn_raw_buffer_load_b128(rsA, (int)vo, (int)so_a, 0);
        }
        return;
      }
#pragma unroll
      for (int i = 0; i < Y_PER; ++i) {
        const int m = mt + yr0 + i * RSY;
        const bool ok = y_act && m < m_end;
        mask |= (ok ? 1u : 0u) << i;
        const long long off = ok ? (long long)m * p.ldy + yn : 0;
        ry[i] = *reinterpret_cast<const u32x4*>(Yg + off);
      }
#pragma unroll
      for (int i = 0; i < A_PER; ++i) {
        const int m = mt + ar0 + i * RSA;
        bool ok = a_act && m < m_end;
        long long off;
        if constexpr (IS1X1) {
          off = (long long)m * p.lda + a_ci;
        } else {
          int iy = poy[i] * p.stride - p.pad_t + a_kh, ix = pox[i] * p.stride - p.pad_l + a_kw;
          if (p.ups) {
            ok = ok && iy >= 0 && iy < 2 * p.H && ix >= 0 && ix < 2 * p.W;
            iy >>= 1;
            ix >>= 1;
          } else {
            ok = ok && (unsigned)iy < (unsigned)p.H && (unsigned)ix < (unsigned)p.W;
          }
          off = (((long long)pb[i] * p.H + iy) * p.W + ix) * p.lda + a_ci;
          pb[i] += adv_b; poy[i] += adv_y; pox[i] += adv_x;
          if (pox[i] >= p.Wo) { pox[i] -= p.Wo; ++poy[i]; }
          if (poy[i] >= p.Ho) { poy[i] -= p.Ho; ++pb[i]; }
        }
        mask |= (ok ? 1u : 0u) << (16 + i);
        ra[i] = *reinterpret_cast<const u32x4*>(Ag + (ok ? off : 0));
      }
    };
    auto commit = [&](char* buf, const u32x4 (&ry)[Y_PER], const u32x4 (&ra)[A_PER],
                      unsigned mask) __attribute__((always_inline)) {
      char* Ys = buf;
      char* As = buf + MT * PY;
#pragma unroll
      for (int i = 0; i < Y_PER; ++i)
        *reinterpret_cast<u32x4*>(Ys + (yr0 + i * RSY) * PY + ycc * 16) =
            (FAST || ((mask >> i) & 1u)) ? ry[i] : zero4;
#pragma unroll
      for (int i = 0; i < A_PER; ++i)
        *reinterpret_cast<u32x4*>(As + (ar0 + i * RSA) * PA + acc_ * 16) =
            (FAST || ((mask >> (16 + i)) & 1u)) ? ra[i] : zero4;
    };

    u32x4 ry0[Y_PER], ra0[A_PER], ry1[Y_PER], ra1[A_PER];
    unsigned mk0 = 0, mk1 = 0;
    if (n_steps > 0) issue(m_begin, ry0, ra0, mk0);
    if (n_steps > 1) issue(m_begin + MT, ry1, ra1, mk1);
    for (int s = 0; s < n_steps; s += 2) {
      commit(smem, ry0, ra0, mk0);
      if (s + 2 < n_steps) issue(m_begin + (s + 2) * MT, ry0, ra0, mk0);
      __syncthreads();
      if (s + 1 < n_steps) {
        commit(smem + STAGE, ry1, ra1, mk1);
        if (s + 3 < n_steps) issue(m_begin + (s + 3) * MT, ry1, ra1, mk1);
        __syncthreads();
      }
    }
    return;
  }

  const int tid = threadIdx.x, lane = tid & 63, wave = tid >> 6;
  const int wn = wave >> 1, wk = wave & 1;
  f32x16 acc[FN][FK];
#pragma unroll
  for (int i = 0; i < FN; ++i)
#pragma unroll
    for (int j = 0; j < FK; ++j)
#pragma unroll
      for (int r = 0; r < 16; ++r) acc[i][j][r] = 0.f;

  const int g = lane >> 4, t = lane & 15;
  const int lrow = (g >> 1) * 8 + (t >> 2);
  const int lcol = (g & 1) * 16 + (t & 3) * 4;
  const int yoff = lrow * PY + (wn * WTN + lcol) * 2;
  const int aoff = MT * PY + lrow * PA + (wk * WTK + lcol) * 2;
  constexpr int KS = MT / 16;
  auto read_frags = [&](const char* Yf, const char* Af, int ks, s16x8 (&fy)[FN], s16x8 (&fa)[FK])
                        __attribute__((always_inline)) {
#pragma unroll
    for (int i = 0; i < FN; ++i) {
      const s16x4 lo =
          __builtin_amdgcn_ds_read_tr16_b64_v4i16(SDMI_LDS_V4(Yf + (ks * 16) * PY + i * 64));
      const s16x4 hi =
          __builtin_amdgcn_ds_read_tr16_b64_v4i16(SDMI_LDS_V4(Yf + (ks * 16 + 4) * PY + i * 64));
      fy[i] = __builtin_shufflevector(lo, hi, 0, 1, 2, 3, 4, 5, 6, 7);
    }
#pragma unroll
    for (int j = 0; j < FK; ++j) {
      const s16x4 lo =
          __builtin_amdgcn_ds_read_tr16_b64_v4i16(SDMI_LDS_V4(Af + (ks * 16) * PA + j * 64));
      const s16x4 hi =
          __builtin_amdgcn_ds_read_tr16_b64_v4i16(SDMI_LDS_V4(Af + (ks * 16 + 4) * PA + j * 64));
      fa[j] = __builtin_shufflevector(lo, hi, 0, 1, 2, 3, 4, 5, 6, 7);
    }
  };
  for (int s = 0; s < n_steps; ++s) {
    __syncthreads();
    const char* buf = smem + (s & 1) * STAGE;
    const char* Yf = buf + yoff;
    const char* Af = buf + aoff;
    s16x8 fy[2][FN], fa[2][FK];
    read_frags(Yf, Af, 0, fy[0], fa[0]);
#pragma unroll
    for (int ks = 0; ks < KS; ++ks) {
// ... 100 lines not shown
```

### slotdiffusion_amd/kern.py

```python
import ctypes
import os
from types import SimpleNamespace

import numpy as np
import torch

from . import _lib, bwd, derived, ops, policy
from ._lib import call

_DT = {torch.float32: _lib.F32, torch.bfloat16: _lib.BF16}


def _p(t):
    return 0 if t is None else t.data_ptr()


def _st():
    return torch.cuda.current_stream().cuda_stream


_DEBUG = False


def _dbg(tag, **tensors):
    if _DEBUG:
        msg = ' '.join(f'{k}={float(v.float().norm()):.4e}' if v is not None else f'{k}=None'
                       for k, v in tensors.items())
        print(f'[bwd] {tag}: {msg}', flush=True)


FP8_ACT_SCALE = 8.0
_LAZY_CAT = bool(policy.flag('LAZY_CAT'))
_GEGLU_FUSE = bool(policy.flag('GEGLU_FUSE'))


class CatPair:

    def __init__(self, a, b):
        self.a, self.b = a, b
        self.shape = tuple(a.shape[:-1]) + (a.shape[-1] + b.shape[-1],)
        self.dtype, self.device = a.dtype, a.device

    def dim(self):
        return self.a.dim()

    def materialize(self):
        return ops.concat_channels(self.a, self.b)


_RES_MERGE = bool(policy.flag('RES_MERGE'))
_FF_MERGE = bool(policy.flag('FF_MERGE'))
_CROSS_FOLD = bool(policy.flag('CROSS_FOLD'))
_CROSS_MAX_SLOTS = 16
_LN_FOLD = bool(policy.flag('LN_FOLD'))
_ST_FUSED = bool(policy.flag('ST_FUSED'))
_ST_FF_SPLIT = bool(policy.flag('ST_FF_SPLIT'))
_WGRAD_HALO = bool(policy.flag('WGRAD_HALO'))
_CROSS_ONE = 64
_ROLLOUT_FUSED = bool(policy.flag('ROLLOUT_FUSED'))
_UPS_PARITY = bool(policy.flag('UPS_PARITY'))
_UPS_TRAIN = policy.flag('UPS_PARITY') == 1
_ST_MIN_WGS = 128
_ST_ROWS = 0


def _copy_group(items):
    for c0 in range(0, len(items), 32):
        arr = _lib.struct_array('SdmiCopyItem', (dict(src=sp, dst=dp, bytes=nb) for sp, dp, nb in items[c0:c0 + 32]))
        call('sdmi_copy_group', _st(), items=ctypes.addressof(arr), n=len(arr))


def _scatter_add(segs):
    for c0 in range(0, len(segs), 32):
        arr = _lib.struct_array('SdmiScatterItem', (dict(src=sp, dst=dp, count=cnt) for sp, dp, cnt in segs[c0:c0 + 32]))
        call('sdmi_scatter_add', _st(), items=ctypes.addressof(arr), n=len(arr))


def _st_unit_index(entries):
    r = np.arange(16, dtype=np.int64)[:, None, None]
    p_ = np.arange(8, dtype=np.int64)[None, :, None]
    e = np.arange(8, dtype=np.int64)[None, None, :]
    col = (p_ ^ ((r >> 1) & 7)) * 8 + e
    out = []
    for ent in entries:
        for off, ld, row0, k0 in ent:
            out.append((off + (row0 + r) * ld + k0 + col).reshape(-1))
    return torch.from_numpy(np.concatenate(out))


def st_geometry(C):
    NSL, KT = C // 128, C // 64
    return dict(NSL=NSL, KT=KT, NHC=C // 32, R=C // 32 * 8, UA=4 * KT * NSL, UB1=KT * NSL,
                UIMG=KT + 2 * NSL, UB2=KT * NSL + (C // 32) * (2 * KT + 2 * NSL))


def st_index_a(C):
    g = st_geometry(C)
    ent = []
    for w in range(8):
        e = []
        for m in range(4):
            for kt in range(g['KT']):
                for s_ in range(g['NSL']):
                    e.append((m * C * C, C, (w * g['NSL'] + s_) * 16, kt * 64))
        ent.append(e)
    return _st_unit_index(ent)


def st_index_b(C):
    g = st_geometry(C)
    NSL, KT = g['NSL'], g['KT']
    o_po, o_1, o_m = C * C, 2 * C * C, 2 * C * C + 8 * C * C
    ent = []
    for w in range(8):
        e = []
        for kt in range(KT):
            for s_ in range(NSL):
                e.append((0, C, (w * NSL + s_) * 16, kt * 64))
        for kt in range(KT):
            for s_ in range(NSL):
                e.append((o_po, C, (w * NSL + s_) * 16, kt * 64))
        for hc in range(g['NHC']):
            for kt in range(KT):
                e.append((o_1, C, hc * 128 + w * 16, kt * 64))
                e.append((o_1, C, 4 * C + hc * 128 + w * 16, kt * 64))
            for k2 in range(2):
                for s_ in range(NSL):
                    e.append((o_m, 4 * C, (w * NSL + s_) * 16, hc * 128 + k2 * 64))
        ent.append(e)
    return _st_unit_index(ent)
# ... 984 lines not shown
        return ops.cast2d(x, dtype, cols=cols, ldd=ldd)

    def dropout(self, x, site='unet'):
        return x

    def linear_drop_res(self, x, wname, bname, res):
        return self.linear(x, wname, bname, residual=res)

    def slot_attention(self, kv, init, name, iters, eps):
        wb = self.wb
        D = kv.shape[-1] // 2
        P = dict(lnq_g=wb.f(f'{name}.project_q.0.weight'), lnq_b=wb.f(f'{name}.project_q.0.bias'),
                 wq=wb.f(f'{name}.project_q.1.weight'), w_ih=wb.f(f'{name}.gru.weight_ih'),
                 w_hh=wb.f(f'{name}.gru.weight_hh'), b_ih=wb.f(f'{name}.gru.bias_ih'),
                 b_hh=wb.f(f'{name}.gru.bias_hh'), lnm_g=wb.f(f'{name}.mlp.0.weight'),
                 lnm_b=wb.f(f'{name}.mlp.0.bias'), w1=wb.f(f'{name}.mlp.1.weight'),
                 b1=wb.f(f'{name}.mlp.1.bias'), w2=wb.f(f'{name}.mlp.3.weight'),
                 b2=wb.f(f'{name}.mlp.3.bias'))
        return ops.slot_attention(kv[..., :D], kv[..., D:], init, P, iters=iters, eps=eps)


def _grads_of(wb, names):
    m = wb.model
    g = m.grad_arena()
    if isinstance(names, str):
        names = (names,)
    offs = [m._offsets[n] for n in names]
    for i in range(len(offs) - 1):
        if offs[i][0] + offs[i][1] != offs[i + 1][0]:
            return None
    return g[offs[0][0]:offs[-1][0] + offs[-1][1]]


class _RowvecSink:

    def __init__(self, B, total):
        self.B, self.total, self.buf = B, total, None
        self.filled = set()

    def buffer(self, device):
        if self.buf is None:
            self.buf = torch.empty((self.B, self.total), dtype=torch.float32, device=device)
        return self.buf


class RowvecSplitFn(torch.autograd.Function):

    @staticmethod
    def forward(ctx, rowvecs, bounds):
        B, total = rowvecs.shape
        assert bounds[0][0] == 0 and bounds[-1][0] + bounds[-1][1] == total
        sink = _RowvecSink(B, total)
        ctx.sink = sink
        outs = []
        for off, c in bounds:
            v = rowvecs[:, off:off + c]
            outs.append(v)
        ctx.set_materialize_grads(False)
        ctx.n = len(bounds)
        return tuple(outs)

    @staticmethod
    def backward(ctx, *grads):
        sink = ctx.sink
        assert sink.buf is not None and all(g is not None for g in grads), 'every slice needs its consumer'
        buf, sink.buf = sink.buf, None
        sink.filled.clear()
        return buf, None


_CUS = {}


def _n_cus(device):
    key = str(device)
    if key not in _CUS:
        _CUS[key] = int(torch.cuda.get_device_properties(device).multi_processor_count)
    return _CUS[key]


class GemmFn(torch.autograd.Function):

    @staticmethod
    def forward(ctx, x, rowvec, residual, anchor, wb, wnames, bnames, geom, out_dtype, ldc, n_alias=0):
        kh, kw, stride, pad, ups = geom
        w = wb.w(wnames, x.dtype)
        b = wb.b(bnames)
        x8 = getattr(x, '_sdmi_fp8', None)
        ctx.ups4 = wb.ups_train_ok(x, wnames, geom, rowvec is None and residual is None and out_dtype is None
                                   and ldc is None)
        if ctx.ups4:
            out = torch.empty((x.shape[0], 2 * x.shape[1], 2 * x.shape[2], w.shape[0]), dtype=x.dtype, device=x.device)
            ops.conv2d(x, wb.ups_fwd(wnames, x.dtype), b, kh=2, kw=2, out=out, parity4=True)
        elif x8 is not None and x8.shape == x.shape and wb.fp8_train_ok(x, wnames, geom):
            w8, inv = wb.w8_dev(wnames)
            out = ops.conv2d(x8, w8, b, kh=kh, kw=kw, stride=stride, pad=pad,
                             rowvec=rowvec, residual=residual, out_dtype=out_dtype or x.dtype, ldc=ldc,
                             alpha=1.0 / FP8_ACT_SCALE, alpha_dev=inv)
        elif x.dim() == 4 and (kh, kw) != (0, 0):
            out = ops.conv2d(x, w, b, kh=kh, kw=kw, stride=stride, pad=pad, ups=ups, rowvec=rowvec,
                             residual=residual, out_dtype=out_dtype, ldc=ldc)
        else:
            out = ops.linear(x, w, b, residual=residual, out_dtype=out_dtype)
        ctx.save_for_backward(x)
        ctx.cfg = (wb, wnames, bnames, geom, rowvec is not None, residual is not None,
                   rowvec.shape if rowvec is not None else None)
        ctx.rv_sink = getattr(rowvec, '_sdmi_sink', None)
        ctx.set_materialize_grads(False)
        if n_alias:
            return out, x.view_as(x)
        return out

    @staticmethod
    def backward(ctx, dy, dalias=None):
        (x,) = ctx.saved_tensors
        if dalias is not None:
            dalias = dalias.contiguous()
        wb, wnames, bnames, geom, has_rv, has_res, rv_shape = ctx.cfg
        dx, dy, (N, ldy, B, Ho, Wo, dt) = GemmFn.core(wb, x, dy, wnames, bnames, geom,
                                                       ctx.needs_input_grad[0], dalias, ctx.ups4)
        drv = None
        if has_rv and ctx.needs_input_grad[1]:
            if ctx.rv_sink is not None:
                sink, off = ctx.rv_sink
                drv = sink.buffer(x.device)[:, off:off + N]
                if off not in sink.filled:
                    call('sdmi_rowgroup_sum', _st(), x=_p(dy), out=_p(drv), dtype=_DT[dt], groups=B,
                         rows_per=Ho * Wo, N=N, ldx=ldy, ldo=drv.stride(0))
            else:
                drv = torch.empty(rv_shape, dtype=torch.float32, device=x.device)
                call('sdmi_rowgroup_sum', _st(), x=_p(dy), out=_p(drv), dtype=_DT[dt], groups=B,
                     rows_per=Ho * Wo, N=N, ldx=ldy)
        dres = None
        if has_res and ctx.needs_input_grad[2]:
            dres = dy if dy.shape[-1] == N else None
            assert dres is not None
        _dbg(f'gemm {wnames if isinstance(wnames, str) else wnames[0]}', dy=dy, dx=dx, drv=drv)
        return dx, drv, dres, None, None, None, None, None, None, None, None

    @staticmethod
    def core(wb, x, dy, wnames, bnames, geom, need_dx, dalias=None, ups4=False):
        dt = x.dtype
        vec = ops.vec_of(dt)
        N = wb.w(wnames, dt).shape[0]
        dy = dy.contiguous()
        if dy.dtype != dt or dy.shape[-1] % vec:
            npad = (N + vec - 1) // vec * vec
            dy = ops.cast2d(dy, dt, cols=N, ldd=npad)
        if ups4:
            return GemmFn._ups4(wb, x, dy, wnames, bnames, N, need_dx, dalias)
        P = bwd.LayerProblem.of(x, dy, geom, dt, N)
        info = (N, P.ldy, P.B, P.Ho, P.Wo, dt)
        names = (wnames,) if isinstance(wnames, str) else tuple(wnames)
        dst = _grads_of(wb, names)
        bdst = _grads_of(wb, bnames) if bnames is not None else None
        direct = dst is not None and wb.t[names[0]].numel() // wb.t[names[0]].shape[0] == P.K
        plan = bwd.plan_layer(P, need_dx=need_dx, direct=direct, has_bias=bnames is not None, bias_dst=bdst is not None,
                              dalias_cols=(dalias.shape[-1] if dalias is not None else None), n_cus=_n_cus(x.device),
                              pair_bwd=wb.pair_bwd, wgrad_halo=_WGRAD_HALO)
        if plan.path == 'pair':
            wd = wb.wd(wnames, dt, P.kh, P.kw, P.Cin)
            dx = torch.empty(x.shape if not P.is_conv else (P.B, P.H, P.W, P.Cin), dtype=dt, device=x.device)
            wb.sched.launch_pair(
                P, plan.pair,
                dict(P.dgrad_fields(), a=_p(dy), w=_p(wd), out=_p(dx), split_k=1, residual=_p(dalias)),
                dict(P.wgrad_fields(), a=_p(x), dy=_p(dy), dw=_p(dst), dbias=_p(bdst), accumulate=1), x.device)
            return dx, dy, info
        wb.sched.side_wgrad(names[0], (_p(dst), _p(bdst)),
                            lambda: GemmFn._wgrad(wb, x, dy, P, plan, names, bnames, dst, direct), (x, dy))
        dx = None
        if need_dx:
            wd = wb.wd(wnames, dt, P.kh, P.kw, P.Cin)
            if P.is_conv and P.stride > 1 and not P.ups:
                dx, dalias = GemmFn._dgrad_strided(
                    dy, wd, P.B, P.H, P.W, P.Ho, P.Wo, P.Cin, P.ldy, P.kh, P.kw, P.stride, P.pad, dt, dalias,
                    sub_of=lambda a0, b0: wb.wd_sub(wnames, dt, P.kh, P.kw, P.Cin, a0, b0, P.stride))
            elif P.is_conv:
                f = P.dgrad_fields()
                out = torch.empty((P.B, f['Ho'], f['Wo'], P.Cin), dtype=dt, device=x.device)
                ws = None if P.stride > 1 else ops.splitk_workspace(f['M'], P.Cin, f['K'], dy.element_size(), x.device)
                fuse = dalias is not None and not P.ups
                call('sdmi_igemm', _st(), a=_p(dy), w=_p(wd), out=_p(out), workspace=_p(ws),
                     split_k=(0 if ws is not None else 1), residual=(_p(dalias) if fuse else 0), **f)
                if fuse:
                    dalias = None
                if P.ups:
                    dx = torch.empty_like(x)
                    call('sdmi_pool2x2_sum', _st(), x=_p(out), y=_p(dx), dtype=_DT[dt], B=P.B, H=P.H, W=P.W, C=P.Cin)
                else:
                    dx = out
            else:
                dx = ops.linear(dy.view(-1, P.ldy), wd,
                                residual=(dalias.view(-1, P.Cin) if dalias is not None else None)).view(x.shape)
                dalias = None
            if dalias is not None:
                call('sdmi_add', _st(), x=_p(dx), z=_p(dalias), y=_p(dx), dtype=_DT[dt], n=dx.numel())
        elif dalias is not None:
            dx = dalias
        return dx, dy, info

    @staticmethod
    def _dgrad_strided(dy, wd, B, H, W_, Ho, Wo, Cin, ldy, kh, kw, s, pad, dt, extra=None, sub_of=None):
        full, subs = bwd.LayerProblem.conv(B, H, W_, Ho, Wo, Cin, ldy, ldy, kh, kw, s, pad, dt).parity_dgrads()
        w4 = wd.view(Cin, kh, kw, ldy)
        dx = torch.empty((B, H, W_, Cin), dtype=dt, device=dy.device)
        if not full:
            ops.zero_(dx)
        fuse = extra is not None and full
        for a0, b0, f in subs:
            sub = sub_of(a0, b0) if sub_of is not None else w4[:, a0::s, b0::s, :].contiguous()
            call('sdmi_igemm', _st(), a=_p(dy), w=_p(sub), out=_p(dx), split_k=1, residual=(_p(extra) if fuse else 0), **f)
        return dx, (None if fuse else extra)

    @staticmethod
    def _ups4(wb, x, dy, wname, bname, N, need_dx, dalias):
        dt = x.dtype
        P = bwd.LayerProblem.upsampled(x, N)
        dst = _grads_of(wb, wname)
        bias = {}
        if bname is not None:
            rows = P.B * P.H * P.W
            chunk = next((c for c in (256, 128, 64) if rows % c == 0), rows)
            part = torch.empty((rows // chunk, N), dtype=torch.float32, device=x.device)
            bias = dict(dy=_p(dy), bias_part=_p(part), dtype=_DT[dt], rows=rows, rows_per=chunk)
        done = []

        def wgrad():
            splits = bwd.standalone_splits(P)
            ws = torch.empty((splits * (P.N * P.K + P.N),), dtype=torch.float32, device=x.device)
            call('sdmi_wgrad', _st(), a=_p(dy), dy=_p(x), dw=_p(ws), dbias=0, workspace=_p(ws), splits=splits,
                 accumulate=0, defer_fold=1, **P.wgrad_fields())
            call('sdmi_ups_fold_dw', _st(), dw4=_p(ws), dw=_p(dst), Cin=P.N, Cout=P.Cin, accumulate=1, splits=splits,
                 **bias)
            done.append(torch.cuda.Event())
            done[0].record()
        wb.sched.side_wgrad(wname, (_p(dst), 0), wgrad, (x, dy))
        if bias:
            wb.queue_colsum(part, rows // chunk, N, _grads_of(wb, bname), None, after=done[0])
        dx = dalias
        if need_dx:
            dx = ops.conv2d(dy, wb.ups_wd(wname, dt), None, kh=4, kw=4, stride=2, pad=(1, 1, 1, 1), residual=dalias)
        return dx, dy, (N, N, P.B, P.H, P.W, dt)

    @staticmethod
    def _wgrad(wb, x, dy, P, plan, names, bnames, dst, direct):
        N, K, Cin = P.N, P.K, P.Cin
        ws = torch.empty((plan.splits * (N * K + N),), dtype=torch.float32, device=x.device)
        acc = 1 if direct else 0
        dwbuf = dst if direct else torch.empty((N, K), dtype=torch.float32, device=x.device)
        btmp, stage_bias = None, False
        if bnames is not None:
            bdst = _grads_of(wb, bnames)
            if direct and bdst is not None:
                btmp = bdst
            else:
                stage_bias = True
                btmp = torch.empty((N,), dtype=torch.float32, device=x.device)
                if acc:
                    ops.zero_(btmp)
        call('sdmi_wgrad', _st(), a=_p(x), dy=_p(dy), dw=_p(dwbuf), dbias=_p(btmp), workspace=_p(ws), splits=plan.splits,
             accumulate=acc, **P.wgrad_fields())
        if not direct:
            g = wb.model.grad_arena()
            taps = P.kh * P.kw
            o, segs, keep = 0, [], []
            for nme in names:
                off, cnt = wb.model._offsets[nme]
                rows = wb.t[nme].shape[0]
                ci_true = cnt // (rows * taps)
                src = dwbuf[o:o + rows]
                if ci_true != Cin:
                    src = ops.cast2d(src.reshape(rows * taps, Cin), torch.float32, cols=ci_true, ldd=ci_true)
                    keep.append(src)
                segs.append((_p(src), _p(g[off:]), cnt))
                o += rows
            _scatter_add(segs)
        if stage_bias:
            g = wb.model.grad_arena()
            o, segs = 0, []
            for nme in (bnames if not isinstance(bnames, str) else (bnames,)):
                off, cnt = wb.model._offsets[nme]
                segs.append((_p(btmp[o:]), _p(g[off:]), cnt))
                o += cnt
            _scatter_add(segs)


class MultiLinearFn(torch.autograd.Function):

    @staticmethod
    def forward(ctx, x, anchor, wb, wname_list):
        ctx.save_for_backward(x)
        ctx.cfg = (wb, wname_list)
        ctx.set_materialize_grads(False)
        return tuple(ops.linear(x, wb.w(n, x.dtype)) for n in wname_list)

    @staticmethod
    def backward(ctx, *dys):
        (x,) = ctx.saved_tensors
        wb, wname_list = ctx.cfg
        geom = (0, 0, 1, (0, 0, 0, 0), False)
        dx = None
        for n, dy in zip(wname_list, dys):
            if dy is None:
                continue
            d, _, _ = GemmFn.core(wb, x, dy, n, None, geom, ctx.needs_input_grad[0], dx)
            dx = d if d is not None else dx
        return dx, None, None, None


class GroupNormFn(torch.autograd.Function):
    @staticmethod
    def forward(ctx, x, residual, anchor, wb, name, eps, act, n_alias=0, drop=None, rsink=None, f8=None):
        gamma, beta = wb.f(name + '.weight'), wb.f(name + '.bias')
        y, stats = ops.group_norm(x, gamma, beta, eps=eps, act=act, residual=residual,
                                  return_stats=True, drop=drop, fp8_scale=(f8[0] if f8 else None),
                                  fp8_also=(f8 if f8 else None))
        ctx.save_for_backward(x, stats, residual)
        ctx.cfg = (wb, name, act)
        ctx.drop = drop if (drop is not None and drop[0] > 0.0) else None
        ctx.rsink = rsink
        ctx.set_materialize_grads(False)
        if n_alias:
            return (y,) + tuple(x.view_as(x) for _ in range(n_alias))
        return y

    @staticmethod
    def backward(ctx, dy, *dal):
        x, stats, residual = ctx.saved_tensors
        wb, name, act = ctx.cfg
        extras = [d.contiguous() for d in dal if d is not None]
        assert len(extras) <= 2 and all(e.dtype == x.dtype for e in extras)
        if dy is None:
            dx = extras[0]
            for e in extras[1:]:
                dx = AddFn.apply(dx, e)
            return dx, None, None, None, None, None, None, None, None, None, None
        dy = dy.contiguous()
        B, C = x.shape[0], x.shape[-1]
        HW = x.numel() // (B * C)
        G = 32
        nsplit = max(1, min(16, HW // 64))
        partial = torch.empty((B * nsplit * C * 2 + B * G * 2,), dtype=torch.float32,
                              device=x.device)
        dx = torch.empty_like(x)
        dres = torch.empty_like(x) if residual is not None else None
        dg = _grads_of(wb, name + '.weight')
        db = _grads_of(wb, name + '.bias')
        geo = dict(dtype=_DT[x.dtype], B=B, HW=HW, C=C, groups=G, nsplit=nsplit)
        defer = wb.defer_colsum
        if defer:
            wb.queue_colsum(partial, _lib.query('sdmi_groupnorm_bwd_entries', **geo), C, db, dg)
        rs_kw, rs_view = {}, None
        if ctx.rsink is not None and not extras:
            sink, off = ctx.rsink
            rs_view = sink.buffer(x.device)[:, off:off + C]
            if _lib.query('sdmi_groupnorm_bwd_fused', **geo):
                rs_kw = dict(dxsum=_p(rs_view), ld_dxsum=rs_view.stride(0))
        call('sdmi_groupnorm_bwd', _st(), x=_p(x), dy=_p(dy), dx=_p(dx), gamma=_p(wb.f(name + '.weight')),
             beta=_p(wb.f(name + '.bias')), stats=_p(stats), dgamma=_p(dg), dbeta=_p(db),
             partial=_p(partial), defer_colsum=int(defer), **geo, **rs_kw,
             act=_lib.ACT[act], residual=_p(residual), dresidual=_p(dres), accumulate=1,
             dextra0=(_p(extras[0]) if extras else 0), dextra1=(_p(extras[1]) if len(extras) > 1 else 0),
             **(dict(drop_p=float(ctx.drop[0]), drop_seed=int(ctx.drop[1]), drop_seed_dev=_p(ctx.drop[2]))
                if ctx.drop else {}))
        if rs_view is not None:
            if not rs_kw:
                call('sdmi_rowgroup_sum', _st(), x=_p(dx), out=_p(rs_view), dtype=_DT[dx.dtype], groups=B,
                     rows_per=HW, N=C, ldx=C, ldo=rs_view.stride(0))
            ctx.rsink[0].filled.add(ctx.rsink[1])
        _dbg(f'gn {name}', dy=dy, dx=dx, dres=dres)
        return dx, dres, None, None, None, None, None, None, None, None, None


class LayerNormFn(torch.autograd.Function):
    @staticmethod
    def forward(ctx, x, anchor, wb, name, n_alias=0):
        C = x.shape[-1]
        stats = torch.empty((x.numel() // C, 2), dtype=torch.float32, device=x.device)
        y = ops.layer_norm(x, wb.f(name + '.weight'), wb.f(name + '.bias'), stats=stats)
        ctx.save_for_backward(x, stats)
        ctx.cfg = (wb, name)
        ctx.set_materialize_grads(False)
        if n_alias:
            return y, x.view_as(x)
        return y

    @staticmethod
    def backward(ctx, dy, dalias=None):
        x, stats = ctx.saved_tensors
        wb, name = ctx.cfg
        if dalias is not None:
            dalias = dalias.contiguous()
        if dy is None:
            return dalias, None, None, None, None
        return LayerNormFn.bwd_core(wb, name, x, stats, dy.contiguous(), dalias), None, None, None, None

    @staticmethod
    def bwd_core(wb, name, x, stats, dy, dalias=None):
        C = x.shape[-1]
        rows = x.numel() // C
        nblk = max(1, min(512, rows // 16))
        partial = torch.empty((nblk * C * 2,), dtype=torch.float32, device=x.device)
        dx = torch.empty_like(x)
        dg, db = _grads_of(wb, name + '.weight'), _grads_of(wb, name + '.bias')
        defer = wb.defer_colsum
        if defer:
            wb.queue_colsum(partial, nblk, C, dg, db)
        call('sdmi_layernorm_bwd', _st(), x=_p(x), dy=_p(dy), dx=_p(dx),
             gamma=_p(wb.f(name + '.weight')), stats=_p(stats), dgamma=_p(dg), dbeta=_p(db),
             partial=_p(partial), dtype=_DT[x.dtype], rows=rows, C=C, nblk=nblk, accumulate=1,
             dextra=_p(dalias), defer_colsum=int(defer))
        _dbg(f'ln {name}', dy=dy, dx=dx)
        return dx


class AttnFn(torch.autograd.Function):

    @staticmethod
    def forward(ctx, q_or_qkv, kv, heads, head_dim=32):
        C = heads * head_dim
        if kv is None:
            q, k, v = q_or_qkv[..., :C], q_or_qkv[..., C:2 * C], q_or_qkv[..., 2 * C:]
        else:
            q, k, v = q_or_qkv, kv[..., :C], kv[..., C:]
        B, Sq = q.shape[0], q.shape[1]
        lse = torch.empty((B, heads, Sq), dtype=torch.float32, device=q.device)
        out = ops.attention(q, k, v, heads, lse=lse, head_dim=head_dim)
        ctx.save_for_backward(q_or_qkv, kv, out, lse)
        ctx.heads, ctx.hd = heads, head_dim
        return out

    @staticmethod
    def backward(ctx, dout):
        a, kv, out, lse = ctx.saved_tensors
        da, dkv = AttnFn.bwd_core(a, kv, out, lse, dout.contiguous(), ctx.heads, ctx.hd)
        return da, dkv, None, None

    @staticmethod
    def bwd_core(a, kv, out, lse, dout, heads, hd=32):
        C = heads * hd
        da = torch.empty_like(a)
        dkv = torch.empty_like(kv) if kv is not None else None
        if kv is None:
            q, k, v = a[..., :C], a[..., C:2 * C], a[..., 2 * C:]
            dq, dk, dv = da[..., :C], da[..., C:2 * C], da[..., 2 * C:]
        else:
            q, k, v = a, kv[..., :C], kv[..., C:]
            dq, dk, dv = da, dkv[..., :C], dkv[..., C:]
        B, Sq, Skv = q.shape[0], q.shape[1], k.shape[1]
        call('sdmi_attention_bwd', _st(), q=_p(q), k=_p(k), v=_p(v), out=_p(out), dout=_p(dout),
             lse=_p(lse), dq=_p(dq), dk=_p(dk), dv=_p(dv), dtype=_DT[q.dtype], B=B, heads=heads,
             Sq=Sq, Skv=Skv, ldq=q.stride(1), ldk=k.stride(1), ldv=v.stride(1), ldo=out.stride(1),
             scale=hd ** -0.5, head_dim=hd)
        _dbg(f'attn Sq={Sq} Skv={Skv}', dout=dout, da=da, dkv=dkv)
# ... 16 lines not shown
    def backward(ctx, dout):
        qkv, P = ctx.saved_tensors
        heads, hd = ctx.heads, ctx.hd
        C = heads * hd
        B, S, _ = qkv.shape
        dout = dout.contiguous()
        dqkv = torch.empty_like(qkv)
        dp = torch.empty((B, S, S), dtype=qkv.dtype, device=qkv.device)
        for h in range(heads):
            q, k, v = (qkv[..., j * C + h * hd:j * C + (h + 1) * hd] for j in range(3))
            dq, dk, dv = (dqkv[..., j * C + h * hd:j * C + (h + 1) * hd] for j in range(3))
            do = dout[..., h * hd:(h + 1) * hd]
            p = P[h]
            ops.bmm_nt(do, v, dp)
            ops.bmm_nt(ops.transpose2d(p), ops.transpose2d(do), dv)
            ops.softmax_rows_bwd_(p, dp, scale=float(hd) ** -0.5)
            ops.bmm_nt(dp, ops.transpose2d(k), dq)
            ops.bmm_nt(ops.transpose2d(dp), ops.transpose2d(q), dk)
        return dqkv, None, None


class GegluFn(torch.autograd.Function):
    @staticmethod
    def forward(ctx, h):
        ctx.save_for_backward(h)
        return ops.geglu(h)

    @staticmethod
    def backward(ctx, dy):
        (h,) = ctx.saved_tensors
        dy = dy.contiguous()
        dh = torch.empty_like(h)
        C = h.shape[-1] // 2
        call('sdmi_geglu_bwd', _st(), h=_p(h), dy=_p(dy), dh=_p(dh), dtype=_DT[h.dtype],
             rows=h.numel() // (2 * C), C=C)
        return dh


class GegluLinearFn(torch.autograd.Function):

    @staticmethod
    def forward(ctx, x, anchor, wb, wname, bname):
        w = wb.w(wname, x.dtype)
        h = torch.empty(x.shape[:-1] + (w.shape[0],), dtype=x.dtype, device=x.device)
        y = ops.linear(x, w, wb.b(bname), geglu=True, out2=h)
        ctx.save_for_backward(x, h)
        ctx.cfg = (wb, wname, bname)
        return y

    @staticmethod
    def backward(ctx, dy):
        x, h = ctx.saved_tensors
        wb, wname, bname = ctx.cfg
        dy = dy.contiguous()
        dh = torch.empty_like(h)
        C = h.shape[-1] // 2
        call('sdmi_geglu_bwd', _st(), h=_p(h), dy=_p(dy), dh=_p(dh), dtype=_DT[h.dtype],
             rows=h.numel() // (2 * C), C=C)
        dx = GemmFn.core(wb, x, dh, wname, bname, (0, 0, 1, (0, 0, 0, 0), False), ctx.needs_input_grad[0])[0]
        return dx, None, None, None, None


def _gn_bwd_plain(wb, name, x, stats, dy, extras=()):
    B, C = x.shape[0], x.shape[-1]
    HW = x.numel() // (B * C)
    G = 32
    nsplit = max(1, min(16, HW // 64))
    partial = torch.empty((B * nsplit * C * 2 + B * G * 2,), dtype=torch.float32, device=x.device)
    dx = torch.empty_like(x)
    dg, db = _grads_of(wb, name + '.weight'), _grads_of(wb, name + '.bias')
    geo = dict(dtype=_DT[x.dtype], B=B, HW=HW, C=C, groups=G, nsplit=nsplit)
    defer = wb.defer_colsum
    if defer:
        wb.queue_colsum(partial, _lib.query('sdmi_groupnorm_bwd_entries', **geo), C, db, dg)
    call('sdmi_groupnorm_bwd', _st(), x=_p(x), dy=_p(dy), dx=_p(dx), gamma=_p(wb.f(name + '.weight')),
         beta=_p(wb.f(name + '.bias')), stats=_p(stats), dgamma=_p(dg), dbeta=_p(db), partial=_p(partial),
         defer_colsum=int(defer), **geo, act=0, residual=0, dresidual=0, accumulate=1,
         dextra0=(_p(extras[0]) if extras else 0), dextra1=(_p(extras[1]) if len(extras) > 1 else 0))
    return dx


_ST_TRAIN = bool(policy.flag('ST_TRAIN'))
_ST_TRAIN_MIN_WGS = 200
_ST_TRAIN_BWD = bool(policy.flag('ST_TRAIN_BWD'))
_ST_WGRAD_GROUP = bool(policy.flag('ST_WGRAD_GROUP'))


class StBlockFn(torch.autograd.Function):

    capture = None
    SAVED = ('hgn', 'gn_stats', 'tok', 'n1', 'st1', 'qkv', 'a1', 'lse1', 'x1', 'n2', 'st2', 'q2', 'a2', 'lse2', 'x2', 'n3',
             'st3', 'h', 'g', 'x3')

    @staticmethod
    def run_forward(wb, x, kv, n, heads, rows):
        B, H, W, C = x.shape
        S = H * W
        dev, bf, f32 = x.device, torch.bfloat16, torch.float32
        e = lambda *sh: torch.empty(sh, dtype=bf, device=dev)
        f = lambda *sh: torch.empty(sh, dtype=f32, device=dev)
        sv = dict(hgn=e(B, S, C), gn_stats=f(B, 32, 2), tok=e(B, S, C), n1=e(B, S, C), st1=f(B * S, 2), qkv=e(B, S, 3 * C),
                  a1=e(B, S, C), lse1=f(B, heads, S), x1=e(B, S, C), n2=e(B, S, C), st2=f(B * S, 2), q2=e(B, S, C),
                  a2=e(B, S, C), lse2=f(B, heads, S), x2=e(B, S, C), n3=e(B, S, C), st3=f(B * S, 2), h=e(B, S, 8 * C),
                  g=e(B, S, 4 * C), x3=e(B, S, C))
        out = torch.empty_like(x)
        st = wb.st_train_streams(n)
        t = n + '.transformer_blocks.0'
        F_ = lambda k: _p(wb.f(k))
        flops = 2.0 * B * S * C * C * 20 + 4.0 * B * S * S * C + 4.0 * B * S * kv.shape[1] * C
        call('sdmi_st_train_fwd', _st(), x=_p(x), out=_p(out), **{k: _p(v) for k, v in sv.items()},
             kv2=_p(kv), ldkv=kv.stride(1), wstream_a=_p(st['wa']), wstream_b=_p(st['wb']),
             gn_gamma=F_(n + '.norm.weight'), gn_beta=F_(n + '.norm.bias'), b_in=F_(n + '.proj_in.bias'),
             ln1_g=F_(t + '.norm1.weight'), ln1_b=F_(t + '.norm1.bias'), b_o=F_(t + '.attn1.to_out.0.bias'),
             ln2_g=F_(t + '.norm2.weight'), ln2_b=F_(t + '.norm2.bias'), b_o2=F_(t + '.attn2.to_out.0.bias'),
             ln3_g=F_(t + '.norm3.weight'), ln3_b=F_(t + '.norm3.bias'), b_ff1=F_(t + '.ff.net.0.proj.bias'),
             b_ff2=F_(t + '.ff.net.2.bias'), b_po=F_(n + '.proj_out.bias'), B=B, S=S, C=C, slots=kv.shape[1], phase=0,
             rows=rows, gn_eps=1e-6, ln_eps=1e-5, attn_scale=32.0 ** -0.5,
             _meta=dict(flops=flops, bytes=2.0 * B * S * C * 23 + 2.0 * 36.5 * C * C))
        return out, sv

    @staticmethod
    def forward(ctx, x, kv, anchor, wb, n, heads, rows):
        out, sv = StBlockFn.run_forward(wb, x, kv, n, heads, rows)
        ctx.save_for_backward(x, kv, *[sv[k] for k in StBlockFn.SAVED])
        ctx.cfg = (wb, n, heads, rows)
        return out

    @staticmethod
    def backward(ctx, dout):
        x, kv = ctx.saved_tensors[:2]
        sv = dict(zip(StBlockFn.SAVED, ctx.saved_tensors[2:]))
        wb, n, heads, rows = ctx.cfg
        if _ST_TRAIN_BWD:
            dx, dkv = StBlockFn.backward_fused(wb, n, heads, x, kv, sv, dout.contiguous(), rows)
        else:
            dx, dkv = StBlockFn.backward_layers(wb, n, heads, x, kv, sv, dout.contiguous())
        return dx, dkv, None, None, None, None, None

    @staticmethod
    def backward_fused(wb, n, heads, x, kv, sv, dout, rows):
        t = n + '.transformer_blocks.0'
        lin = (0, 0, 1, (0, 0, 0, 0), False)
        B, S, C = sv['tok'].shape
        dev = x.device
        do = dout.view(B, S, C)
        nwg = B * S // rows
        st = wb.st_train_streams(n)
        e = lambda *sh: torch.empty(sh, dtype=torch.bfloat16, device=dev)
        part = lambda: torch.empty((nwg * C * 2,), dtype=torch.float32, device=dev)
        grp = []

        def wgrad(a, dy, wn, bn):
            names = (wn,) if isinstance(wn, str) else tuple(wn)
            dst, bdst = _grads_of(wb, names), (_grads_of(wb, bn) if bn is not None else None)
            if not _ST_WGRAD_GROUP or dst is None or (bn is not None and bdst is None):
                GemmFn.core(wb, a, dy, wn, bn, lin, False)
                return
            P = bwd.LayerProblem.of(a, dy, lin, torch.bfloat16, dy.shape[-1])
            grp.append((P, bn is not None, a, dy,
                        dict(P.wgrad_fields(), a=_p(a), dy=_p(dy), dw=_p(dst), dbias=_p(bdst), accumulate=1)))

        def flush_group():
            if not grp:
                return
            wb.sched.launch_group([g[4] for g in grp], bwd.plan_group([g[:2] for g in grp]),
                                  [t_ for g in grp for t_ in g[2:4]], dev)
            del grp[:]
# ... 49 lines not shown
        dx2 = LayerNormFn.bwd_core(wb, t + '.norm3', sv['x2'], sv['st3'], dn3, dx3)
        da2 = core(sv['a2'], dx2, t + '.attn2.to_out.0.weight', t + '.attn2.to_out.0.bias')
        dq2, dkv = AttnFn.bwd_core(sv['q2'], kv, sv['a2'], sv['lse2'], da2, heads)
        dn2 = core(sv['n2'], dq2, t + '.attn2.to_q.weight', None)
        dx1 = LayerNormFn.bwd_core(wb, t + '.norm2', sv['x1'], sv['st2'], dn2, dx2)
        da1 = core(sv['a1'], dx1, t + '.attn1.to_out.0.weight', t + '.attn1.to_out.0.bias')
        dqkv, _ = AttnFn.bwd_core(sv['qkv'], None, sv['a1'], sv['lse1'], da1, heads)
        dn1 = core(sv['n1'], dqkv, (t + '.attn1.to_q.weight', t + '.attn1.to_k.weight', t + '.attn1.to_v.weight'), None)
        dtok = LayerNormFn.bwd_core(wb, t + '.norm1', sv['tok'], sv['st1'], dn1, dx1)
        dhgn = core(sv['hgn'], dtok, n + '.proj_in.weight', n + '.proj_in.bias')
        dx = _gn_bwd_plain(wb, n + '.norm', x.view(B, S, C), sv['gn_stats'], dhgn, (do,))
        if StBlockFn.capture is not None:
            StBlockFn.capture.update(dx3=dx3, dh=dh, dx2=dx2, da2=da2, dq2=dq2, dx1=dx1, da1=da1, dqkv=dqkv, dtok=dtok,
                                     dhgn=dhgn)
        return dx.view_as(x), dkv


class ActFn(torch.autograd.Function):
    @staticmethod
    def forward(ctx, x, kind):
        ctx.save_for_backward(x)
        ctx.kind = kind
        return ops.act(x, kind)

    @staticmethod
    def backward(ctx, dy):
        (x,) = ctx.saved_tensors
        dy = dy.contiguous()
        dx = torch.empty_like(x)
        call('sdmi_act_bwd', _st(), x=_p(x), dy=_p(dy), dx=_p(dx), dtype=_DT[x.dtype],
             act=_lib.ACT[ctx.kind], n=x.numel())
        return dx, None


class CastFn(torch.autograd.Function):
    @staticmethod
    def forward(ctx, x, dtype):
        ctx.src = x.dtype
        return ops.act(x, None, dtype)

    @staticmethod
    def backward(ctx, dy):
        return ops.act(dy.contiguous(), None, ctx.src), None


class CastPadFn(torch.autograd.Function):
    @staticmethod
    def forward(ctx, x, dtype, cols, ldd):
        ctx.src, ctx.ld, ctx.cols = x.dtype, x.shape[-1], cols
        return ops.cast2d(x, dtype, cols=cols, ldd=ldd)

    @staticmethod
    def backward(ctx, dy):
        return ops.cast2d(dy.contiguous(), ctx.src, cols=ctx.cols, ldd=ctx.ld), None, None, None


class AddPosFn(torch.autograd.Function):
    @staticmethod
    def forward(ctx, x, pos):
        ctx.pshape = pos.shape
        return ops.add_pos(x, pos)

    @staticmethod
    def backward(ctx, dy):
        dy = dy.contiguous()
        dpos = None
        if ctx.needs_input_grad[1]:
            B = dy.shape[0]
            per = dy.numel() // B
            dpos = torch.empty(ctx.pshape, dtype=torch.float32, device=dy.device)
            call('sdmi_rowgroup_sum', _st(), x=_p(dy), out=_p(dpos), dtype=_DT[dy.dtype], groups=1,
                 rows_per=B, N=per, ldx=per)
        return dy, dpos


class ConcatFn(torch.autograd.Function):
    @staticmethod
    def forward(ctx, a, b):
        ctx.ca, ctx.cb = a.shape[-1], b.shape[-1]
        return ops.concat_channels(a, b)

    @staticmethod
    def backward(ctx, dy):
        dy = dy.contiguous()
        da = torch.empty(dy.shape[:-1] + (ctx.ca,), dtype=dy.dtype, device=dy.device)
        db = torch.empty(dy.shape[:-1] + (ctx.cb,), dtype=dy.dtype, device=dy.device)
        call('sdmi_split_channels', _st(), y=_p(dy), a=_p(da), b=_p(db), dtype=_DT[dy.dtype],
             rows=dy.numel() // (ctx.ca + ctx.cb), Ca=ctx.ca, Cb=ctx.cb)
        return da, db


class SaAttendFn(torch.autograd.Function):

    @staticmethod
    def forward(ctx, kv, q, eps, chain=False):
        B, M, D2 = kv.shape
        D = D2 // 2
        N = q.shape[1]
        attn = torch.empty((B, M, N), dtype=torch.float32, device=kv.device)
        upd = torch.empty((B, N, D), dtype=torch.float32, device=kv.device)
        den = torch.empty((B, N), dtype=torch.float32, device=kv.device)
        q = q.contiguous()
        ws = torch.empty((B * ((M + 63) // 64) * N * (D + 1),), dtype=torch.float32,
                         device=kv.device)
        call('sdmi_sa_attend_fwd', _st(), k=_p(kv), v=_p(kv[..., D:]), q=_p(q), attn=_p(attn),
             upd=_p(upd), den=_p(den), dtype=_DT[kv.dtype], B=B, M=M, N=N, D=D, ldkv=D2, eps=eps,
             scale=D ** -0.5, workspace=_p(ws))
        ctx.save_for_backward(kv, q, attn, upd, den)
        ctx.eps = eps
        ctx.mark_non_differentiable(attn)
        ctx.set_materialize_grads(False)
        if chain:
            return upd, attn, kv.view_as(kv)
        return upd, attn

    @staticmethod
    def backward(ctx, dupd, _dattn, dkv_next=None):
        kv, q, attn, upd, den = ctx.saved_tensors
        B, M, D2 = kv.shape
        D = D2 // 2
        N = q.shape[1]
        dupd = dupd.contiguous()
        dq = torch.empty_like(q)
        acc = dkv_next is not None and dkv_next.is_contiguous()
        dkv = dkv_next if acc else torch.empty_like(kv)
        ws = torch.empty((B * ((M + 63) // 64) * N * D,), dtype=torch.float32, device=kv.device)
        call('sdmi_sa_attend_bwd', _st(), k=_p(kv), v=_p(kv[..., D:]), q=_p(q), attn=_p(attn),
             upd=_p(upd), den=_p(den), dupd=_p(dupd), dq=_p(dq), dk=_p(dkv), dv=_p(dkv[..., D:]),
             dtype=_DT[kv.dtype], B=B, M=M, N=N, D=D, ldkv=D2, eps=ctx.eps, scale=D ** -0.5,
             workspace=_p(ws), accumulate=int(acc))
        if dkv_next is not None and not acc:
            dkv = AddFn.apply(dkv, dkv_next)
        _dbg('sa_attend', dupd=dupd, dkv=dkv, dq=dq)
        return dkv, dq, None, None


class GruGatesFn(torch.autograd.Function):
    @staticmethod
    def forward(ctx, gi, gh, h):
        R, D = h.shape
        out = torch.empty_like(h)
        call('sdmi_gru_gates', _st(), gi=_p(gi), gh=_p(gh), h=_p(h), hout=_p(out), R=R, D=D)
        ctx.save_for_backward(gi, gh, h)
        return out

    @staticmethod
    def backward(ctx, dout):
        gi, gh, h = ctx.saved_tensors
        R, D = h.shape
        dout = dout.contiguous()
        dgi, dgh, dh = torch.empty_like(gi), torch.empty_like(gh), torch.empty_like(h)
        call('sdmi_gru_gates_bwd', _st(), gi=_p(gi), gh=_p(gh), h=_p(h), dhout=_p(dout),
             dgi=_p(dgi), dgh=_p(dgh), dh=_p(dh), R=R, D=D)
        return dgi, dgh, dh


class LstmCellFn(torch.autograd.Function):

    @staticmethod
    def forward(ctx, z, c_prev):
        h, c, gates = ops.lstm_cell(z, c_prev, want_gates=True)
        ctx.has_prev = c_prev is not None
        ctx.save_for_backward(*((gates, c, c_prev) if ctx.has_prev else (gates, c)))
        ctx.set_materialize_grads(False)
        return h, c

    @staticmethod
    def backward(ctx, dh, dc):
        if dh is None and dc is None:
            return None, None
        gates, c = ctx.saved_tensors[:2]
        c_prev = ctx.saved_tensors[2] if ctx.has_prev else None
# ... 345 lines not shown
        G, R, C = dy.shape
        dx = torch.empty((G, C), dtype=torch.float32, device=dy.device)
        call('sdmi_rowgroup_sum', _st(), x=_p(dy), out=_p(dx), dtype=_DT[dy.dtype], groups=G,
             rows_per=R, N=C, ldx=C)
        dpos = torch.empty((R, C), dtype=torch.float32, device=dy.device)
        call('sdmi_rowgroup_sum', _st(), x=_p(dy), out=_p(dpos), dtype=_DT[dy.dtype], groups=1,
             rows_per=G, N=R * C, ldx=R * C)
        return dx, dpos, None


class SaCombineFn(torch.autograd.Function):

    @staticmethod
    def forward(ctx, o, B, N):
        BN, H, W_, ld = o.shape
        recon = torch.empty((B, H, W_, 4), dtype=torch.float32, device=o.device)
        masks = torch.empty((B, N, H * W_), dtype=torch.float32, device=o.device)
        call('sdmi_sa_combine', _st(), o=_p(o), recon=_p(recon), masks=_p(masks), dtype=_DT[o.dtype],
             B=B, N=N, HW=H * W_, ldo=ld)
        ctx.save_for_backward(o, masks)
        ctx.mark_non_differentiable(masks)
        ctx.set_materialize_grads(False)
        return recon, masks

    @staticmethod
    def backward(ctx, drecon, _dm):
        o, masks = ctx.saved_tensors
        B, N = masks.shape[0], masks.shape[1]
        dout = torch.empty_like(o)
        call('sdmi_sa_combine_bwd', _st(), o=_p(o), masks=_p(masks), drecon=_p(drecon.contiguous()),
             dout=_p(dout), dtype=_DT[o.dtype], B=B, N=N, HW=masks.shape[2], ldo=o.shape[-1])
        return dout, None, None


class NhwcToNchwFn(torch.autograd.Function):

    @staticmethod
    def forward(ctx, x, C):
        ctx.cpad = x.shape[-1]
        return ops.nhwc_to_nchw(x, C)

    @staticmethod
    def backward(ctx, dy):
        return ops.nchw_to_nhwc(dy.contiguous(), torch.float32, ctx.cpad), None


class KernGrad(Kern):
    training = True
    dropout_p = 0.0
    _drop_ctr = 0

    def __init__(self, wb):
        super().__init__(wb)
        rank = int(os.environ.get('RANK', 0))
        self.seed = ((int(getattr(wb.model, 'seed', 0)) * 1000003 + rank * 7919 + 1) & 0xffffffff)

    def _p_drop(self, site):
        attr = 'train_dropout' if site == 'unet' else 'pred_dropout'
        return float(getattr(self.wb.model, attr, 0.0))

    def linear_drop_res(self, x, wname, bname, res):
        if self._p_drop('pred') <= 0.0:
            return self.linear(x, wname, bname, residual=res)
        return AddFn.apply(res, self.dropout(self.linear(x, wname, bname), site='pred'))

    def dropout(self, x, site='unet'):
        p = self._p_drop(site)
        if p <= 0.0:
            return x
        self._drop_ctr += 1
        return DropoutFn.apply(x, p, (self.seed << 20) + self._drop_ctr,
                               getattr(self.wb.model, 'step_seed', None))

    def begin_step(self):
        m = self.wb.model
        dev = m.arena().device
        if getattr(m, 'step_seed', None) is None or m.step_seed.device != dev:
            m.step_seed = torch.zeros(1, dtype=torch.int64, device=dev)
        call('sdmi_counters_inc', _st(), seed=_p(m.step_seed))
        self._drop_ctr = 0

    def conv(self, x, wname, bname=None, *, kh=3, kw=3, stride=1, pad=(1, 1, 1, 1), ups=False,
             rowvec=None, residual=None, out_dtype=None, ldc=None):
        return GemmFn.apply(x, rowvec, residual, self.wb.anchor_for(wname), self.wb, wname, bname,
                            (kh, kw, stride, pad, ups), out_dtype, ldc)

    def linear(self, x, wnames, bnames=None, *, act=None, residual=None, out_dtype=None):
        y = GemmFn.apply(x, None, residual, self.wb.anchor_for(wnames), self.wb, wnames, bnames,
                         (0, 0, 1, (0, 0, 0, 0), False), out_dtype, None)
        return ActFn.apply(y, act) if act else y

    def gn(self, x, name, *, eps, act=None, residual=None, dropout=None, for_conv=None, rowsum_of=None):
        drop = None
        if dropout is not None:
            p = self._p_drop(dropout)
            if p > 0.0:
                self._drop_ctr += 1
                drop = (p, (self.seed << 20) + self._drop_ctr, getattr(self.wb.model, 'step_seed', None))
        f8 = self._f8_for(x, for_conv)
        y = GroupNormFn.apply(x, residual, self.wb.anchor_for(name), self.wb, name, eps, act, 0, drop,
                              getattr(rowsum_of, '_sdmi_sink', None), f8)
        if f8 is not None and len(f8) > 1:
            y._sdmi_fp8 = f8[1]
        return y

    def _f8_for(self, x, for_conv):
        return [FP8_ACT_SCALE] if (for_conv and self.fp8_ok(x, for_conv, 9, False)) else None

    def st_train(self, x, n, heads, kv):
        B, H, W, C = x.shape
        S = H * W
        if not (_ST_TRAIN and torch.is_tensor(kv) and x.dtype == torch.bfloat16 and kv.dtype == torch.bfloat16 and
                C in (256, 384) and heads * 32 == C and S % 32 == 0 and S <= 256 and kv.shape[1] <= 16 and
                kv.shape[-1] == 2 * C and kv.stride(-1) == 1 and x.is_contiguous()):
            return None
        rows = _ST_ROWS or (64 if (S % 64 == 0 and B * S // 64 >= 192) else 32)
        if S % rows or B * S // rows < _ST_TRAIN_MIN_WGS:
            return None
        return StBlockFn.apply(x, kv, self.wb.anchor_for(n), self.wb, n, heads, rows)

    def ff_out_proj(self, g, tres, xres, t, n):
        tok = self.linear(g, t + '.ff.net.2.weight', t + '.ff.net.2.bias', residual=tres)
        return self.linear(tok, n + '.proj_out.weight', n + '.proj_out.bias', residual=xres)

    def res_tail(self, h, n, skip):
        if (n + '.skip_connection.weight') in self.wb.t:
            skip = self.conv(skip, n + '.skip_connection.weight', n + '.skip_connection.bias', kh=1, kw=1,
                             pad=(0, 0, 0, 0))
        return self.conv(h, n + '.out_layers.3.weight', n + '.out_layers.3.bias', residual=skip)

    def rowvec_slices(self, rowvecs, bounds):
        if not rowvecs.requires_grad:
            return [rowvecs[:, off:off + c] for off, c in bounds]
        outs = RowvecSplitFn.apply(rowvecs, tuple(bounds))
        sink = outs[0].grad_fn.sink if hasattr(outs[0].grad_fn, 'sink') else None
        for v, (off, c) in zip(outs, bounds):
            v._sdmi_sink = (sink, off)
        return list(outs)

    def gn_fan(self, x, name, *, eps, act=None, residual=None, n_alias=1, for_conv=None):
        f8 = self._f8_for(x, for_conv)
        outs = GroupNormFn.apply(x, residual, self.wb.anchor_for(name), self.wb, name, eps, act, n_alias, None, None, f8)
        if f8 is not None and len(f8) > 1:
            outs[0]._sdmi_fp8 = f8[1]
        return outs

    def linear_fan(self, x, wnames, bnames=None):
        return GemmFn.apply(x, None, None, self.wb.anchor_for(wnames), self.wb, wnames, bnames,
                            (0, 0, 1, (0, 0, 0, 0), False), None, None, 1)

    def linear_multi(self, x, wname_list):
        wname_list = tuple(wname_list)
        return MultiLinearFn.apply(x, self.wb.anchor_for(wname_list[0]), self.wb, wname_list)

    def ln_fan(self, x, name):
        return LayerNormFn.apply(x, self.wb.anchor_for(name), self.wb, name, 1)

    def ln_linear_fan(self, x, ln_name, wnames, bnames=None, *, act=None, geglu=False, eps=1e-5):
        n, xres = self.ln_fan(x, ln_name)
        if geglu and _GEGLU_FUSE and act is None and isinstance(wnames, str) and n.dtype == torch.bfloat16 \
                and n.shape[-1] % 64 == 0:
            return GegluLinearFn.apply(n, self.wb.anchor_for(wnames), self.wb, wnames, bnames), xres
        h = self.linear(n, wnames, bnames, act=act)
        return (self.geglu(h) if geglu else h), xres

    def conv_fan(self, x, wname, bname=None, *, kh=3, kw=3, stride=1, pad=(1, 1, 1, 1), ups=False,
                 rowvec=None, residual=None, out_dtype=None, ldc=None):
        return GemmFn.apply(x, rowvec, residual, self.wb.anchor_for(wname), self.wb, wname, bname,
                            (kh, kw, stride, pad, ups), out_dtype, ldc, 1)

    def deconv(self, x, wname, bname, *, k, stride, pad, act='relu'):
        return DeconvFn.apply(x, self.wb.anchor_for(wname), self.wb, wname, bname, k, stride, pad, act)

    def broadcast_pos(self, x, pos, dtype):
        return BroadcastPosFn.apply(x, pos, dtype)

    def sa_combine(self, o, B, N):
        return SaCombineFn.apply(o, B, N)

    def ln(self, x, name):
        return LayerNormFn.apply(x, self.wb.anchor_for(name), self.wb, name)

    def attn_self(self, qkv, heads, head_dim=32):
        fits = ops.ATTN_MFMA_MAX_KV if (qkv.dtype == torch.bfloat16 and head_dim == 32) else ops.ATTN_LDS_MAX_KV
        if qkv.shape[1] > fits:
            return LongAttnFn.apply(qkv, heads, head_dim)
        return AttnFn.apply(qkv, None, heads, head_dim)

    def attn_cross(self, q, kv, heads):
        return AttnFn.apply(q, kv, heads)

    def vae_attn_core(self, qkv):
        return VaeAttnFn.apply(qkv)

    def geglu(self, h):
        return GegluFn.apply(h)

    def add_pos(self, x, pos):
        return AddPosFn.apply(x, pos)

    def shift_window(self, win, new, L):
        return ShiftWindowFn.apply(win, new, L)

    def tail_tokens(self, x, n, L):
        return TailTokensFn.apply(x, n, L)

    def concat(self, a, b):
        return ConcatFn.apply(a, b)

    def cast(self, x, dtype):
        return x if x.dtype == dtype else CastFn.apply(x, dtype)

    def lstm_cell(self, z, c_prev):
        return LstmCellFn.apply(z, c_prev)

    def pred_step(self, x, base, wrap, norm_first, state):
        return None

    def pred_tf(self, x, base, layers, heads):
        return None

    def cast_pad(self, x, dtype, cols, ldd):
        return CastPadFn.apply(x, dtype, cols, ldd)

    def slot_attention(self, kv, init, name, iters, eps):
        B, M, D2 = kv.shape
        D = D2 // 2
        if init.dim() == 2:
            init = init.unsqueeze(0).expand(B, -1, -1)
        slots = init.contiguous()
        N = slots.shape[1]
        seg = None
        for it in range(iters):
            nq, s_alias = self.ln_fan(slots, f'{name}.project_q.0')
            q = self.linear(nq, f'{name}.project_q.1.weight')
            if it + 1 < iters:
                upd, attn, kv = SaAttendFn.apply(kv, q, eps, True)
            else:
                upd, attn = SaAttendFn.apply(kv, q, eps)
            seg = attn
            gi = self.linear(upd.reshape(B * N, D), f'{name}.gru.weight_ih', f'{name}.gru.bias_ih')
            gh, prev = self.linear_fan(s_alias.reshape(B * N, D), f'{name}.gru.weight_hh',
                                       f'{name}.gru.bias_hh')
            h = GruGatesFn.apply(gi, gh, prev)
            nh, h_alias = self.ln_fan(h, f'{name}.mlp.0')
            hid = self.linear(nh, f'{name}.mlp.1.weight', f'{name}.mlp.1.bias', act='relu')
            slots = self.linear(hid, f'{name}.mlp.3.weight', f'{name}.mlp.3.bias',
                                residual=h_alias).view(B, N, D)
        return slots, seg
```

### slotdiffusion_amd/policy.py

```python
import os

SWITCHES = {
    'ST_FUSED':      (1, 'fused SpatialTransformer block at inference (sdmi_st_block: 2 launches instead of 10-13)'),
    'ST_FF_SPLIT':   (1, 'feed-forward of that block split over workgroup pairs where its grid leaves half the chip idle'),
    'CROSS_FOLD':    (1, 'slot cross-attention folded into per-image projection weights (<= 16 slots)'),
    'LN_FOLD':       (1, 'LayerNorm folded into the linear layer behind it (bf16 inference)'),
    'RES_MERGE':     (1, 'ResBlock out_layers.3 + 1x1 skip convolution as one implicit GEMM'),
    'FF_MERGE':      (1, 'ff.net.2 + proj_out as one GEMM over [g | tok] with pre-multiplied weights'),
    'UPS_PARITY':    (1, 'upsample convolutions as four 2x2 parity convolutions in one launch -- 1: sampler and training '
                         '(4x4 stride-2 transposed form: parity forward, strided data gradient, folded weight '
                         'gradient), 2: sampler only, 0: off'),
    'DEFER_SPLITK':  (1, 'split-K second stage finished by the GroupNorm behind the convolution'),
    'LAZY_CAT':      (1, 'UNet skip concatenations read in place by their two consumers'),
    'ROLLOUT_FUSED': (1, 'fused SlotFormer rollout layer at inference (sdmi_rollout_layer: 2 launches instead of ~8)'),
    'ST_TRAIN':      (1, 'fused training forward of the SpatialTransformer block (sdmi_st_train_fwd)'),
    'ST_TRAIN_BWD':  (1, 'fused backward data path of that block (sdmi_st_train_bwd)'),
    'ST_WGRAD_GROUP': (1, "the block's eight weight gradients as two grouped launches"),
    'BWD_PAIR':      (1, 'data + weight gradient of a conv / linear layer in one launch (sdmi_bwd_pair)'),
    'WGRAD_STREAM':  (1, 'stand-alone weight gradients on side HIP streams'),
    'WGRAD_HALO':    (1, 'direct 3x3 weight gradient on channel pairs where the layer leaves the pair launch'),
    'GEGLU_FUSE':    (1, 'GEGLU in the epilogue of the ff.net.0.proj GEMM (per-layer training path)'),
    'DEFER_COLSUM':  (1, 'dgamma / dbeta column sums of the whole step folded by a few grouped launches'),
    'DEBUG_DEFER':   (0, 'poison the outputs of deferred split-K launches until their second stage ran (tests)'),
}


def flag(name):
    default = SWITCHES[name][0]
    v = os.environ.get('SDMI_' + name)
    return default if v is None else int(v)
```

Baseline: 2420 images/s.

## Read UNet skip concatenations in place during training via two-source GroupNorm and 1x1 wgrad

Training UNet skip concatenations become a lazy TrainCat object instead of a materialized tensor. The GroupNorm forward and backward read and write the two halves directly through x2/dx2 with a channel split C1. The 1x1 skip convolution's GEMM and weight gradient take a two-source A operand (a2/lda2/K1). This removes the concat copy and the split-channels copy in backward, at the cost of more complex kernels and a fallback to materializing when the geometry constraints are not met.

```diff
diff --git a/include/sdmi.h b/include/sdmi.h
--- a/include/sdmi.h
+++ b/include/sdmi.h
@@ -77,6 +77,8 @@
   int splits;
   int accumulate;
   int defer_fold;
+  const void* a2;
+  int lda2, K1;
 } SdmiWgradArgs;
 int sdmi_wgrad(const SdmiWgradArgs* a, void* stream);
 enum {
@@ -158,6 +160,9 @@
   float* dxsum;
   int ld_dxsum;
   int defer_colsum;
+  const void* x2;
+  void* dx2;
+  int C1;
 } SdmiGroupNormBwdArgs;
 int sdmi_groupnorm_bwd(const SdmiGroupNormBwdArgs* a, void* stream);
 int sdmi_groupnorm_bwd_fused(const SdmiGroupNormBwdArgs* a, void* unused);
diff --git a/slotdiffusion_amd/bwd.py b/slotdiffusion_amd/bwd.py
--- a/slotdiffusion_amd/bwd.py
+++ b/slotdiffusion_amd/bwd.py
@@ -39,11 +39,18 @@
     lda: int
     ldy: int
     dt: torch.dtype
+    K1: int = 0
+    lda2: int = 0
 
     @classmethod
-    def of(cls, x, dy, geom, dt, N):
+    def of(cls, x, dy, geom, dt, N, x2=None):
         kh, kw, stride, pad, ups = geom
         Cin = x.shape[-1]
+        if x2 is not None:
+            assert x.dim() == 4 and (kh, kw) == (1, 1) and x2.shape[:-1] == x.shape[:-1]
+            C2 = x2.shape[-1]
+            return cls.conv(x.shape[0], x.shape[1], x.shape[2], dy.shape[1], dy.shape[2], Cin + C2, N, dy.shape[-1], kh, kw,
+                            stride, pad, dt, ups)._replace(lda=Cin, K1=Cin, lda2=C2)
         if x.dim() == 4 and (kh, kw) != (0, 0):
             return cls.conv(x.shape[0], x.shape[1], x.shape[2], dy.shape[1], dy.shape[2], Cin, N, dy.shape[-1], kh, kw,
                             stride, pad, dt, ups)
@@ -67,10 +74,16 @@
         B, H, W, Cin = x.shape
         return cls.conv(B, 2 * H, 2 * W, H, W, Cout, Cin, Cin, 4, 4, 2, (1, 1, 1, 1), x.dtype)
 
+    def materialized(self):
+        return self._replace(lda=self.Cin, K1=0, lda2=0) if self.K1 else self
+
     def wgrad_fields(self):
-        return dict(dtype=_DT[self.dt], M=self.M, N=self.N, K=self.K, lda=self.lda, ldy=self.ldy, B=self.B, H=self.H,
-                    W=self.W, Cin=self.Cin, Ho=self.Ho, Wo=self.Wo, KH=self.kh, KW=self.kw, stride=self.stride,
-                    pad_t=self.pad[0], pad_l=self.pad[2], ups=int(self.ups))
+        f = dict(dtype=_DT[self.dt], M=self.M, N=self.N, K=self.K, lda=self.lda, ldy=self.ldy, B=self.B, H=self.H,
+                 W=self.W, Cin=self.Cin, Ho=self.Ho, Wo=self.Wo, KH=self.kh, KW=self.kw, stride=self.stride,
+                 pad_t=self.pad[0], pad_l=self.pad[2], ups=int(self.ups))
+        if self.K1:
+            f.update(lda2=self.lda2, K1=self.K1)
+        return f
 
     def dgrad_fields(self):
         Hs, Ws = (2 * self.H, 2 * self.W) if self.ups else (self.H, self.W)
@@ -117,6 +130,15 @@
     splits: int
     kernel: str
     pair: Optional[PairPlan]
+    materialize: bool = False
+
+
+def two_source_ok(P):
+    one = (P.is_conv and P.kh == 1 and P.kw == 1 and P.stride == 1 and not P.ups and P.pad[0] == 0 and P.pad[2] == 0
+           and P.Ho == P.H and P.Wo == P.W)
+    return (P.K1 > 0 and one and P.dt == torch.bfloat16 and P.K1 % 128 == 0 and P.K1 < P.K and (P.K - P.K1) % 8 == 0
+            and P.lda == P.K1 and P.lda2 == P.K - P.K1 and P.ldy % 8 == 0
+            and (P.M + 2 * P.W + 256) * max(P.lda, P.lda2, P.ldy) * 2 < (1 << 31))
 
 
 def _mstep(P):
@@ -156,7 +178,7 @@
             and (one or (same and kh * kw <= 32 and P.ldy % bk == 0
                          and pad[0] == pad[1] == (kh - 1) // 2 and pad[2] == pad[3] == (kw - 1) // 2))
             and (dalias_cols is None or dalias_cols == P.Cin)
-            and (P.M + (kh + 1) * P.W + 128) * max(P.lda, P.ldy, P.Cin) * 2 < (1 << 31) and P.N * kd * 2 < (1 << 31))
+            and (P.M + (kh + 1) * P.W + 128) * max(P.lda, P.lda2, P.ldy, P.Cin) * 2 < (1 << 31) and P.N * kd * 2 < (1 << 31))
 
 
 def _pair_plan(P, has_bias):
@@ -181,6 +203,9 @@
 
 
 def plan_layer(P, *, need_dx, direct, has_bias, bias_dst, dalias_cols, n_cus, pair_bwd=True, wgrad_halo=True):
+    if P.K1 and not two_source_ok(P):
+        return plan_layer(P.materialized(), need_dx=need_dx, direct=direct, has_bias=has_bias, bias_dst=bias_dst,
+                          dalias_cols=dalias_cols, n_cus=n_cus, pair_bwd=pair_bwd, wgrad_halo=wgrad_halo)._replace(materialize=True)
     splits, kernel = _standalone(P, n_cus, wgrad_halo)
     if pair_bwd and need_dx and _pairable(P, direct, has_bias, bias_dst, dalias_cols):
         return LayerPlan('pair', splits, kernel, _pair_plan(P, has_bias))
diff --git a/slotdiffusion_amd/csrc/bwd_pair.hip b/slotdiffusion_amd/csrc/bwd_pair.hip
--- a/slotdiffusion_amd/csrc/bwd_pair.hip
+++ b/slotdiffusion_amd/csrc/bwd_pair.hip
@@ -108,7 +108,8 @@
                w.lda % 8 == 0 && w.ldy % 8 == 0, "bad wgrad geometry");
   PAIR_REQUIRE(w.splits >= 1 && (w.splits == 1 || w.workspace), "splits > 1 need a workspace");
   const long long mps = ((long long)w.M + w.splits - 1) / w.splits + 64;
-  const long long ld = w.lda > w.ldy ? w.lda : w.ldy;
+  long long ld = w.lda > w.ldy ? w.lda : w.ldy;
+  if (w.a2 && w.lda2 > ld) ld = w.lda2;
   PAIR_REQUIRE((mps + (long long)(w.KH + 1) * w.W + 64) * ld * 2 < (1ll << 31), "wgrad split beyond 31-bit offsets");
   if (f) PAIR_REQUIRE(f->dw && f->workspace && f->splits > 1 && f->N > 0 && f->K > 0 && ((long long)f->N * f->K) % 4 == 0 &&
                       f->dw != w.dw && (!f->dbias || f->dbias != w.dbias), "bad fold problem (or it targets this layer's dW)");
@@ -130,6 +131,12 @@
   PAIR_REQUIRE(a->wgrad_tile == 0 || a->wgrad_tile == 128 || (a->wgrad_tile == 64 && !big),
                "wgrad_tile: 128, or 64 next to 64 x 64 data-gradient tiles");
   const int t = big ? 128 : 64;
+  {
+    const int wt = a->wgrad_tile == 64 ? 64 : 128;
+    PAIR_REQUIRE((!w.a2 && w.K1 <= 0) || (w.a2 && w1x1 && w.K1 > 0 && w.K1 < w.K && w.K1 % wt == 0 && (w.K - w.K1) % 8 == 0 && w.lda2 % 8 == 0 &&
+                           w.lda >= w.K1 && w.lda2 >= w.K - w.K1),
+                 "two-source wgrad: 1x1 / linear, K1 a multiple of the weight-gradient tile inside (0, K)");
+  }
   route = {t, t, wide ? 128 : 64, d1x1 ? 1 : 2, a->wgrad_tile == 64 ? 64 : 128, hw_shift};
   return 0;
 }
diff --git a/slotdiffusion_amd/csrc/norm_bwd.hip b/slotdiffusion_amd/csrc/norm_bwd.hip
--- a/slotdiffusion_amd/csrc/norm_bwd.hip
+++ b/slotdiffusion_amd/csrc/norm_bwd.hip
@@ -9,6 +9,22 @@
   int p = 1;
   while (p < v) p <<= 1;
   return p;
+}
+
+template <typename T>
+__device__ __forceinline__ void gnb_io(const SdmiGroupNormBwdArgs& p, int b, int c, const T*& xs, T*& dxs, int& pitch) {
+  if (p.x2) {
+    const bool hi = c >= p.C1;
+    pitch = hi ? p.C - p.C1 : p.C1;
+    const long long o = (long long)b * p.HW * pitch + (hi ? c - p.C1 : c);
+    xs = (const T*)(hi ? p.x2 : p.x) + o;
+    dxs = (T*)(hi ? p.dx2 : p.dx) + o;
+    return;
+  }
+  pitch = p.C;
+  const long long o = (long long)b * p.HW * p.C + c;
+  xs = (const T*)p.x + o;
+  dxs = (T*)p.dx + o;
 }
 
 template <typename T>
@@ -38,7 +54,10 @@
       be[j] = p.beta[c];
     }
     const long long base = (long long)b * p.HW * p.C + cv * VEC;
-    const T* xb = (const T*)p.x + base;
+    const T* xb;
+    T* dxb;
+    int xp;
+    gnb_io<T>(p, b, cv * VEC, xb, dxb, xp);
     const T* db = (const T*)p.dy + base;
     const T* rb = p.residual ? (const T*)p.residual + base : nullptr;
     const bool drop = p.drop_p > 0.f;
@@ -48,7 +67,7 @@
     for (int row = row_begin + r0; row < row_end; row += R) {
       const long long o = (long long)row * p.C;
       float x[VEC], dy[VEC], rr[VEC];
-      unpack16<T>(*reinterpret_cast<const uint4*>(xb + o), x);
+      unpack16<T>(*reinterpret_cast<const uint4*>(xb + (long long)row * xp), x);
       unpack16<T>(*reinterpret_cast<const uint4*>(db + o), dy);
       if (drop) sdmi_drop_apply<VEC>(dy, dseed, (base + o) / VEC, thr16, dinv);
       if (rb) unpack16<T>(*reinterpret_cast<const uint4*>(rb + o), rr);
@@ -103,7 +122,10 @@
     be[j] = p.beta[c];
   }
   const long long base = (long long)b * p.HW * p.C + c_lo + (act_c ? cv : 0) * VEC;
-  const T* xb = (const T*)p.x + base;
+  const T* xb;
+  T* dxb;
+  int xp;
+  gnb_io<T>(p, b, c_lo + (act_c ? cv : 0) * VEC, xb, dxb, xp);
   const T* db = (const T*)p.dy + base;
   const T* rb = p.residual ? (const T*)p.residual + base : nullptr;
   uint4 xr[NV], dr[NV];
@@ -111,7 +133,7 @@
   for (int i = 0; i < NV; ++i) {
     const int row = r0 + i * R;
     if (act_c && row < p.HW) {
-      xr[i] = *reinterpret_cast<const uint4*>(xb + (long long)row * p.C);
+      xr[i] = *reinterpret_cast<const uint4*>(xb + (long long)row * xp);
       dr[i] = *reinterpret_cast<const uint4*>(db + (long long)row * p.C);
     }
   }
@@ -191,7 +213,6 @@
     s1[j] = gsum[g][0] * inv_n;
     s2[j] = gsum[g][1] * inv_n;
   }
-  T* dxb = (T*)p.dx + base;
   T* drb = p.dresidual ? (T*)p.dresidual + base : nullptr;
   const T* e0 = p.dextra0 ? (const T*)p.dextra0 + base : nullptr;
   const T* e1 = p.dextra1 ? (const T*)p.dextra1 + base : nullptr;
@@ -222,7 +243,7 @@
       }
 #pragma unroll
       for (int j = 0; j < VEC; ++j) sd[j] += dx[j];
-      *reinterpret_cast<uint4*>(dxb + o) = pack16<T>(dx);
+      *reinterpret_cast<uint4*>(dxb + (long long)row * xp) = pack16<T>(dx);
       if (drb) *reinterpret_cast<uint4*>(drb + o) = dr[i];
     }
   }
@@ -275,7 +296,10 @@
   const int g0 = cl0 / cpg;
   const int bnd = (g0 + 1) * cpg - cl0;
   const long long base = (long long)b * p.HW * p.C + c_lo + cl0;
-  const T* xb = (const T*)p.x + base;
+  const T* xb;
+  T* dxb;
+  int xp;
+  gnb_io<T>(p, b, c_lo + cl0, xb, dxb, xp);
   const T* db = (const T*)p.dy + base;
   const T* rb = p.residual ? (const T*)p.residual + base : nullptr;
   uint4 xr[NV], dr[NV];
@@ -283,7 +307,7 @@
   for (int i = 0; i < NV; ++i) {
     const int row = r0 + i * R;
     if (act_c && row < p.HW) {
-      xr[i] = *reinterpret_cast<const uint4*>(xb + (long long)row * p.C);
+      xr[i] = *reinterpret_cast<const uint4*>(xb + (long long)row * xp);
       dr[i] = *reinterpret_cast<const uint4*>(db + (long long)row * p.C);
     }
   }
@@ -396,7 +420,6 @@
 #pragma unroll
   for (int j = 0; j < VEC; ++j) sd[j] = 0.f;
   if (act_c) {
-    T* dxb = (T*)p.dx + base;
     T* drb = p.dresidual ? (T*)p.dresidual + base : nullptr;
     const T* e0 = p.dextra0 ? (const T*)p.dextra0 + base : nullptr;
     const T* e1 = p.dextra1 ? (const T*)p.dextra1 + base : nullptr;
@@ -428,7 +451,7 @@
         }
 #pragma unroll
         for (int j = 0; j < VEC; ++j) sd[j] += dx[j];
-        *reinterpret_cast<uint4*>(dxb + o) = pack16<T>(dx);
+        *reinterpret_cast<uint4*>(dxb + (long long)row * xp) = pack16<T>(dx);
         if (drb) *reinterpret_cast<uint4*>(drb + o) = dr[i];
       }
     }
@@ -579,10 +602,12 @@
     s2[j] = gsum[g][1] * inv_n;
   }
   const long long base = (long long)b * p.HW * p.C + cv * VEC;
-  const T* xb = (const T*)p.x + base;
+  const T* xb;
+  T* dxb;
+  int xp;
+  gnb_io<T>(p, b, cv * VEC, xb, dxb, xp);
   const T* db = (const T*)p.dy + base;
   const T* rb = p.residual ? (const T*)p.residual + base : nullptr;
-  T* dxb = (T*)p.dx + base;
   T* drb = p.dresidual ? (T*)p.dresidual + base : nullptr;
   const T* e0 = p.dextra0 ? (const T*)p.dextra0 + base : nullptr;
   const T* e1 = p.dextra1 ? (const T*)p.dextra1 + base : nullptr;
@@ -593,7 +618,7 @@
   for (int row = row_begin + r0; row < row_end; row += R) {
     const long long o = (long long)row * p.C;
     float x[VEC], dy[VEC], rr[VEC], dx[VEC], dz[VEC];
-    unpack16<T>(*reinterpret_cast<const uint4*>(xb + o), x);
+    unpack16<T>(*reinterpret_cast<const uint4*>(xb + (long long)row * xp), x);
     unpack16<T>(*reinterpret_cast<const uint4*>(db + o), dy);
     if (drop) sdmi_drop_apply<VEC>(dy, dseed, (base + o) / VEC, thr16, dinv);
     if (rb) unpack16<T>(*reinterpret_cast<const uint4*>(rb + o), rr);
@@ -616,7 +641,7 @@
 #pragma unroll
       for (int j = 0; j < VEC; ++j) dx[j] += ex[j];
     }
-    *reinterpret_cast<uint4*>(dxb + o) = pack16<T>(dx);
+    *reinterpret_cast<uint4*>(dxb + (long long)row * xp) = pack16<T>(dx);
     if (drb) *reinterpret_cast<uint4*>(drb + o) = pack16<T>(dz);
   }
 }
@@ -770,6 +795,8 @@
   const int vec = a->dtype == SDMI_BF16 ? 8 : 4;
   SDMI_REQUIRE(a->C % vec == 0 && a->C <= 1024, "C must be a vector multiple <= 1024");
   SDMI_REQUIRE(a->groups > 0 && a->C % a->groups == 0 && a->nsplit >= 1, "bad groups/nsplit");
+  SDMI_REQUIRE(!a->x2 || (a->dx2 && a->C1 > 0 && a->C1 < a->C && a->C1 % vec == 0 && (a->C - a->C1) % vec == 0),
+               "two-source input: dx2, and C1 splits the channels on 16-byte vectors");
   hipStream_t st = (hipStream_t)stream;
   dim3 g1(a->nsplit, a->B);
   const long long row_bytes = (long long)a->C * (a->dtype == SDMI_BF16 ? 2 : 4);
diff --git a/slotdiffusion_amd/csrc/wgrad.hip b/slotdiffusion_amd/csrc/wgrad.hip
--- a/slotdiffusion_amd/csrc/wgrad.hip
+++ b/slotdiffusion_amd/csrc/wgrad.hip
@@ -730,7 +730,8 @@
   const bool is1x1 = wgrad_is1x1(a);
   const bool lin = !is1x1 && !a.ups && a.stride == 1 && a.H == a.Ho && a.W == a.Wo;
   const long long mps = ((long long)a.M + a.splits - 1) / a.splits + 64;
-  const long long ld = a.lda > a.ldy ? a.lda : a.ldy;
+  long long ld = a.lda > a.ldy ? a.lda : a.ldy;
+  if (a.a2 && a.lda2 > ld) ld = a.lda2;
   const bool fits = (mps + (long long)(a.KH + 1) * a.W + 64) * ld * 2 < (1ll << 31);
   return {SDMI_WGRAD_KERNEL_IGEMM, a.N <= 64 ? 64 : 128, a.K <= 64 ? 64 : 128,
           is1x1 && fits ? 1 : (lin && fits ? 2 : 0), 0};
@@ -749,6 +750,15 @@
 #undef WG_TR
 }
 
+const char* wgrad_two_source_error(const SdmiWgradArgs& a, int tk) {
+  if (!a.a2 && a.K1 <= 0) return nullptr;
+  if (a.dtype != SDMI_BF16 || !wgrad_is1x1(a)) return "two-source A: bf16 1x1 / linear problems only";
+  if (a.K1 <= 0 || a.K1 >= a.K || a.K1 % tk != 0 || (a.K - a.K1) % 8 != 0 || a.lda2 % 8 != 0 || a.lda < a.K1 ||
+      a.lda2 < a.K - a.K1)
+    return "two-source A: K1 must be a multiple of the K tile inside (0, K), lda / lda2 must cover their columns";
+  return nullptr;
+}
+
 const char* wgrad_geometry_error(const SdmiWgradArgs& a) {
   if (a.dtype != SDMI_F32 && a.dtype != SDMI_BF16) return "bad dtype";
   const int vec = a.dtype == SDMI_BF16 ? 8 : 4;
@@ -756,6 +766,12 @@
   if (a.Cin % vec != 0 || a.lda % vec != 0 || a.ldy % vec != 0) return "Cin/lda/ldy must be multiples of the 16-byte vector width";
   if (a.M != a.B * a.Ho * a.Wo) return "M != B*Ho*Wo";
   if (a.splits < 1) return "splits";
+  if (a.a2 || a.K1 > 0) {
+    if (a.dtype != SDMI_BF16) return "two-source A: bf16 1x1 / linear problems only";
+    const WgradRoute r = select_wgrad_bf16(a);
+    if (r.family != SDMI_WGRAD_KERNEL_IGEMM || r.mode != 1) return "two-source A: the 1x1 / linear scalar-loader kernel only";
+    return wgrad_two_source_error(a, r.tk);
+  }
   return nullptr;
 }
 
@@ -773,7 +789,7 @@
     for (int i = 0; i < ga->n; ++i) {
       const SdmiWgradArgs& a = ps[i];
       SDMI_REQUIRE(a.a && a.dy && a.dw, "null pointer");
-      SDMI_REQUIRE(a.dtype == SDMI_F32 && wgrad_is1x1(a), "grouped wgrad: one dtype per group, 1x1 / linear problems");
+      SDMI_REQUIRE(a.dtype == SDMI_F32 && wgrad_is1x1(a) && !a.a2, "grouped wgrad: one dtype per group, 1x1 / linear problems");
       SDMI_REQUIRE(a.K == a.Cin && a.Cin % 4 == 0 && a.lda % 4 == 0 && a.ldy % 4 == 0 && a.M == a.B * a.Ho * a.Wo,
                    "bad geometry");
       SDMI_REQUIRE(a.splits >= 1 && (a.splits == 1 || a.workspace), "splits / workspace");
@@ -802,15 +818,18 @@
   }
   for (int i = 0; i < ga->n; ++i) {
     const SdmiWgradArgs& a = ps[i];
-    SDMI_REQUIRE(a.a && a.dy && a.dw, "null pointer");
+    SDMI_REQUIRE(a.a && a.dy && a.dw && (a.a2 || a.K1 <= 0), "null pointer");
     SDMI_REQUIRE(a.dtype == SDMI_BF16 && wgrad_is1x1(a) && a.N > 64 && a.K > 64,
                  "grouped wgrad: bf16 1x1 / linear problems with N, K > 64");
     SDMI_REQUIRE(a.K == a.Cin && a.Cin % 8 == 0 && a.lda % 8 == 0 && a.ldy % 8 == 0 && a.M == a.B * a.Ho * a.Wo,
                  "bad geometry");
     SDMI_REQUIRE(a.splits >= 1 && (a.splits == 1 || a.workspace), "splits / workspace");
     const long long mps_ = ((long long)a.M + a.splits - 1) / a.splits + 64;
-    const long long ld = a.lda > a.ldy ? a.lda : a.ldy;
+    long long ld = a.lda > a.ldy ? a.lda : a.ldy;
+    if (a.a2 && a.lda2 > ld) ld = a.lda2;
     SDMI_REQUIRE((mps_ + 64) * ld * 2 < (1ll << 31), "split too large for 31-bit offsets");
+    const char* e2 = wgrad_two_source_error(a, 128);
+    SDMI_REQUIRE(!e2, e2);
     g.p[i] = a;
     g.tiles_n[i] = (a.N + 127) / 128;
     g.tiles_k[i] = (a.K + 127) / 128;
@@ -856,7 +875,7 @@
 }
 
 extern "C" int sdmi_wgrad(const SdmiWgradArgs* a, void* stream) {
-  SDMI_REQUIRE(a && a->a && a->dy && a->dw && a->workspace, "null pointer");
+  SDMI_REQUIRE(a && a->a && a->dy && a->dw && a->workspace && (a->a2 || a->K1 <= 0), "null pointer");
   const char* err = wgrad_geometry_error(*a);
   SDMI_REQUIRE(!err, err);
   hipStream_t st = (hipStream_t)stream;
diff --git a/slotdiffusion_amd/csrc/wgrad_body.h b/slotdiffusion_amd/csrc/wgrad_body.h
--- a/slotdiffusion_amd/csrc/wgrad_body.h
+++ b/slotdiffusion_amd/csrc/wgrad_body.h
@@ -89,7 +89,10 @@
 
   if (threadIdx.x >= 256) {
     const int tid = threadIdx.x - 256;
-    const T* __restrict__ Ag = (const T*)p.a;
+    const bool src2 = IS1X1 && p.a2 && k0 >= p.K1;
+    const T* __restrict__ Ag = (const T*)(src2 ? p.a2 : p.a);
+    const int lda = src2 ? p.lda2 : p.lda;
+    const int k_src = src2 ? p.K1 : 0;
     const T* __restrict__ Yg = (const T*)p.dy;
     const int ycc = tid % CHY, yr0 = tid / CHY;
     const int acc_ = tid % CHA, ar0 = tid / CHA;
@@ -97,7 +100,7 @@
     const bool y_act = yn < p.N;
     const int ak = k0 + acc_ * 8;
     const bool a_act = ak < p.K;
-    int a_ci = a_act ? ak : 0, a_kh = 0, a_kw = 0;
+    int a_ci = a_act ? ak - k_src : 0, a_kh = 0, a_kw = 0;
     int pb[A_PER], poy[A_PER], pox[A_PER];
     int adv_b = 0, adv_y = 0, adv_x = 0;
     if constexpr (!IS1X1) {
@@ -125,7 +128,7 @@
     const __amdgpu_buffer_rsrc_t rsY = __builtin_amdgcn_make_buffer_rsrc(
         (void*)(Yg + (long long)m_begin * p.ldy), 0, (int)OOB, 0x00020000);
     const __amdgpu_buffer_rsrc_t rsA = __builtin_amdgcn_make_buffer_rsrc(
-        (void*)(Ag + ((long long)m_begin - a_bias) * p.lda), 0, (int)OOB, 0x00020000);
+        (void*)(Ag + ((long long)m_begin - a_bias) * lda), 0, (int)OOB, 0x00020000);
     unsigned y_vo[Y_PER], a_vo[A_PER];
     int lw_sh = 0;
     if constexpr (FAST) {
@@ -135,7 +138,7 @@
 #pragma unroll
       for (int i = 0; i < A_PER; ++i) {
         const unsigned r = ar0 + i * RSA + (MODE == 2 ? a_kh * p.W + a_kw : 0);
-        a_vo[i] = a_act ? (r * (unsigned)p.lda + a_ci) * 2u : OOB;
+        a_vo[i] = a_act ? (r * (unsigned)lda + a_ci) * 2u : OOB;
       }
       while ((1 << lw_sh) < p.W) ++lw_sh;
     }
@@ -148,7 +151,7 @@
         const int rel = mt - m_begin;
         const bool tail = mt + MT > m_end;
         const unsigned so_y = (unsigned)rel * (unsigned)p.ldy * 2u;
-        const unsigned so_a = (unsigned)rel * (unsigned)p.lda * 2u;
+        const unsigned so_a = (unsigned)rel * (unsigned)lda * 2u;
 #pragma unroll
         for (int i = 0; i < Y_PER; ++i) {
           unsigned vo = y_vo[i];
@@ -195,7 +198,7 @@
         bool ok = a_act && m < m_end;
         long long off;
         if constexpr (IS1X1) {
-          off = (long long)m * p.lda + a_ci;
+          off = (long long)m * lda + a_ci;
         } else {
           int iy = poy[i] * p.stride - p.pad_t + a_kh, ix = pox[i] * p.stride - p.pad_l + a_kw;
           if (p.ups) {
@@ -205,7 +208,7 @@
           } else {
             ok = ok && (unsigned)iy < (unsigned)p.H && (unsigned)ix < (unsigned)p.W;
           }
-          off = (((long long)pb[i] * p.H + iy) * p.W + ix) * p.lda + a_ci;
+          off = (((long long)pb[i] * p.H + iy) * p.W + ix) * lda + a_ci;
           pb[i] += adv_b; poy[i] += adv_y; pox[i] += adv_x;
           if (pox[i] >= p.Wo) { pox[i] -= p.Wo; ++poy[i]; }
           if (poy[i] >= p.Ho) { poy[i] -= p.Ho; ++pb[i]; }
diff --git a/slotdiffusion_amd/kern.py b/slotdiffusion_amd/kern.py
--- a/slotdiffusion_amd/kern.py
+++ b/slotdiffusion_amd/kern.py
@@ -31,6 +31,7 @@
 
 FP8_ACT_SCALE = 8.0
 _LAZY_CAT = bool(policy.flag('LAZY_CAT'))
+_LAZY_CAT_TRAIN = bool(policy.flag('LAZY_CAT_TRAIN'))
 _GEGLU_FUSE = bool(policy.flag('GEGLU_FUSE'))
 
 
@@ -46,6 +47,23 @@
 
     def materialize(self):
         return ops.concat_channels(self.a, self.b)
+
+
+class TrainCat(CatPair):
+
+    def __init__(self, a, b, token=None):
+        super().__init__(a, b)
+        self.token = token
+
+    def materialize(self):
+        if self.token is None:
+            return ConcatFn.apply(self.a, self.b)
+        return AliasCatFn.apply(self.token, self.a, self.b)
+
+
+def lazy_cat_train_ok(a, b, fp8=False):
+    return (_LAZY_CAT_TRAIN and not fp8 and a.dim() == 4 and a.dtype == torch.bfloat16 and b.dtype == torch.bfloat16
+            and a.shape[:-1] == b.shape[:-1] and a.shape[-1] % 128 == 0 and b.shape[-1] % 128 == 0)
 
 
 _RES_MERGE = bool(policy.flag('RES_MERGE'))
@@ -1196,8 +1214,21 @@
 class GemmFn(torch.autograd.Function):
 
     @staticmethod
-    def forward(ctx, x, rowvec, residual, anchor, wb, wnames, bnames, geom, out_dtype, ldc, n_alias=0):
+    def forward(ctx, x, rowvec, residual, anchor, wb, wnames, bnames, geom, out_dtype, ldc, n_alias=0, pair=None):
         kh, kw, stride, pad, ups = geom
+        ctx.pair = pair is not None
+        if pair is not None:
+            xa, xb = pair
+            assert (kh, kw, stride, ups, n_alias) == (1, 1, 1, False, 0)
+            out = ops.conv2d(xa, wb.w(wnames, xa.dtype), wb.b(bnames), kh=1, kw=1, pad=pad, rowvec=rowvec,
+                             residual=residual, out_dtype=out_dtype, ldc=ldc, x2=xb)
+            ctx.save_for_backward(xa, xb)
+            ctx.cfg = (wb, wnames, bnames, geom, rowvec is not None, residual is not None,
+                       rowvec.shape if rowvec is not None else None)
+            ctx.rv_sink = getattr(rowvec, '_sdmi_sink', None)
+            ctx.ups4 = False
+            ctx.set_materialize_grads(False)
+            return out
         w = wb.w(wnames, x.dtype)
         b = wb.b(bnames)
         x8 = getattr(x, '_sdmi_fp8', None)
@@ -1227,12 +1258,12 @@
 
     @staticmethod
     def backward(ctx, dy, dalias=None):
-        (x,) = ctx.saved_tensors
+        x, x2 = ctx.saved_tensors if ctx.pair else (ctx.saved_tensors[0], None)
         if dalias is not None:
             dalias = dalias.contiguous()
         wb, wnames, bnames, geom, has_rv, has_res, rv_shape = ctx.cfg
         dx, dy, (N, ldy, B, Ho, Wo, dt) = GemmFn.core(wb, x, dy, wnames, bnames, geom,
-                                                       ctx.needs_input_grad[0], dalias, ctx.ups4)
+                                                       ctx.needs_input_grad[0], dalias, ctx.ups4, x2=x2)
         drv = None
         if has_rv and ctx.needs_input_grad[1]:
             if ctx.rv_sink is not None:
@@ -1250,10 +1281,10 @@
             dres = dy if dy.shape[-1] == N else None
             assert dres is not None
         _dbg(f'gemm {wnames if isinstance(wnames, str) else wnames[0]}', dy=dy, dx=dx, drv=drv)
-        return dx, drv, dres, None, None, None, None, None, None, None, None
-
-    @staticmethod
-    def core(wb, x, dy, wnames, bnames, geom, need_dx, dalias=None, ups4=False):
+        return dx, drv, dres, None, None, None, None, None, None, None, None, None
+
+    @staticmethod
+    def core(wb, x, dy, wnames, bnames, geom, need_dx, dalias=None, ups4=False, x2=None):
         dt = x.dtype
         vec = ops.vec_of(dt)
         N = wb.w(wnames, dt).shape[0]
@@ -1263,7 +1294,7 @@
             dy = ops.cast2d(dy, dt, cols=N, ldd=npad)
         if ups4:
             return GemmFn._ups4(wb, x, dy, wnames, bnames, N, need_dx, dalias)
-        P = bwd.LayerProblem.of(x, dy, geom, dt, N)
+        P = bwd.LayerProblem.of(x, dy, geom, dt, N, x2=x2)
         info = (N, P.ldy, P.B, P.Ho, P.Wo, dt)
         names = (wnames,) if isinstance(wnames, str) else tuple(wnames)
         dst = _grads_of(wb, names)
@@ -1272,16 +1303,18 @@
         plan = bwd.plan_layer(P, need_dx=need_dx, direct=direct, has_bias=bnames is not None, bias_dst=bdst is not None,
                               dalias_cols=(dalias.shape[-1] if dalias is not None else None), n_cus=_n_cus(x.device),
                               pair_bwd=wb.pair_bwd, wgrad_halo=_WGRAD_HALO)
+        if plan.materialize:
+            x, x2, P = ops.concat_channels(x, x2), None, P.materialized()
         if plan.path == 'pair':
             wd = wb.wd(wnames, dt, P.kh, P.kw, P.Cin)
             dx = torch.empty(x.shape if not P.is_conv else (P.B, P.H, P.W, P.Cin), dtype=dt, device=x.device)
             wb.sched.launch_pair(
                 P, plan.pair,
                 dict(P.dgrad_fields(), a=_p(dy), w=_p(wd), out=_p(dx), split_k=1, residual=_p(dalias)),
-                dict(P.wgrad_fields(), a=_p(x), dy=_p(dy), dw=_p(dst), dbias=_p(bdst), accumulate=1), x.device)
+                dict(P.wgrad_fields(), a=_p(x), a2=_p(x2), dy=_p(dy), dw=_p(dst), dbias=_p(bdst), accumulate=1), x.device)
             return dx, dy, info
         wb.sched.side_wgrad(names[0], (_p(dst), _p(bdst)),
-                            lambda: GemmFn._wgrad(wb, x, dy, P, plan, names, bnames, dst, direct), (x, dy))
+                            lambda: GemmFn._wgrad(wb, x, dy, P, plan, names, bnames, dst, direct, x2), (x, dy, x2))
         dx = None
         if need_dx:
             wd = wb.wd(wnames, dt, P.kh, P.kw, P.Cin)
@@ -1357,7 +1390,7 @@
         return dx, dy, (N, N, P.B, P.H, P.W, dt)
 
     @staticmethod
-    def _wgrad(wb, x, dy, P, plan, names, bnames, dst, direct):
+    def _wgrad(wb, x, dy, P, plan, names, bnames, dst, direct, x2=None):
         N, K, Cin = P.N, P.K, P.Cin
         ws = torch.empty((plan.splits * (N * K + N),), dtype=torch.float32, device=x.device)
         acc = 1 if direct else 0
@@ -1372,8 +1405,8 @@
                 btmp = torch.empty((N,), dtype=torch.float32, device=x.device)
                 if acc:
                     ops.zero_(btmp)
-        call('sdmi_wgrad', _st(), a=_p(x), dy=_p(dy), dw=_p(dwbuf), dbias=_p(btmp), workspace=_p(ws), splits=plan.splits,
-             accumulate=acc, **P.wgrad_fields())
+        call('sdmi_wgrad', _st(), a=_p(x), a2=_p(x2), dy=_p(dy), dw=_p(dwbuf), dbias=_p(btmp), workspace=_p(ws),
+             splits=plan.splits, accumulate=acc, **P.wgrad_fields())
         if not direct:
             g = wb.model.grad_arena()
             taps = P.kh * P.kw
@@ -1424,23 +1457,30 @@
 
 class GroupNormFn(torch.autograd.Function):
     @staticmethod
-    def forward(ctx, x, residual, anchor, wb, name, eps, act, n_alias=0, drop=None, rsink=None, f8=None):
+    def forward(ctx, x, residual, anchor, wb, name, eps, act, n_alias=0, drop=None, rsink=None, f8=None, x2=None):
         gamma, beta = wb.f(name + '.weight'), wb.f(name + '.bias')
         y, stats = ops.group_norm(x, gamma, beta, eps=eps, act=act, residual=residual,
                                   return_stats=True, drop=drop, fp8_scale=(f8[0] if f8 else None),
-                                  fp8_also=(f8 if f8 else None))
-        ctx.save_for_backward(x, stats, residual)
+                                  fp8_also=(f8 if f8 else None), x2=x2)
+        ctx.pair = x2 is not None
+        if ctx.pair:
+            ctx.save_for_backward(x, stats, residual, x2)
+        else:
+            ctx.save_for_backward(x, stats, residual)
         ctx.cfg = (wb, name, act)
         ctx.drop = drop if (drop is not None and drop[0] > 0.0) else None
         ctx.rsink = rsink
         ctx.set_materialize_grads(False)
+        if n_alias and ctx.pair:
+            return (y,) + tuple(x.new_empty(1).expand(y.shape) for _ in range(n_alias))
         if n_alias:
             return (y,) + tuple(x.view_as(x) for _ in range(n_alias))
         return y
 
     @staticmethod
     def backward(ctx, dy, *dal):
-        x, stats, residual = ctx.saved_tensors
+        x, stats, residual = ctx.saved_tensors[:3]
+        x2 = ctx.saved_tensors[3] if ctx.pair else None
         wb, name, act = ctx.cfg
         extras = [d.contiguous() for d in dal if d is not None]
         assert len(extras) <= 2 and all(e.dtype == x.dtype for e in extras)
@@ -1448,16 +1488,21 @@
             dx = extras[0]
             for e in extras[1:]:
                 dx = AddFn.apply(dx, e)
-            return dx, None, None, None, None, None, None, None, None, None, None
+            dx2 = None
+            if ctx.pair:
+                dx, dx2 = ConcatFn.split(dx, x.shape[-1], x2.shape[-1])
+            return dx, None, None, None, None, None, None, None, None, None, None, dx2
         dy = dy.contiguous()
-        B, C = x.shape[0], x.shape[-1]
-        HW = x.numel() // (B * C)
+        B, C1 = x.shape[0], x.shape[-1]
+        C = C1 + (x2.shape[-1] if ctx.pair else 0)
+        HW = x.numel() // (B * C1)
         G = 32
         nsplit = max(1, min(16, HW // 64))
         partial = torch.empty((B * nsplit * C * 2 + B * G * 2,), dtype=torch.float32,
                               device=x.device)
         dx = torch.empty_like(x)
-        dres = torch.empty_like(x) if residual is not None else None
+        dx2 = torch.empty_like(x2) if ctx.pair else None
+        dres = torch.empty_like(dy) if residual is not None else None
         dg = _grads_of(wb, name + '.weight')
         db = _grads_of(wb, name + '.bias')
         geo = dict(dtype=_DT[x.dtype], B=B, HW=HW, C=C, groups=G, nsplit=nsplit)
@@ -1465,6 +1510,7 @@
         if defer:
             wb.queue_colsum(partial, _lib.query('sdmi_groupnorm_bwd_entries', **geo), C, db, dg)
         rs_kw, rs_view = {}, None
+        assert not (ctx.pair and ctx.rsink is not None)
         if ctx.rsink is not None and not extras:
             sink, off = ctx.rsink
             rs_view = sink.buffer(x.device)[:, off:off + C]
@@ -1475,6 +1521,7 @@
              partial=_p(partial), defer_colsum=int(defer), **geo, **rs_kw,
              act=_lib.ACT[act], residual=_p(residual), dresidual=_p(dres), accumulate=1,
              dextra0=(_p(extras[0]) if extras else 0), dextra1=(_p(extras[1]) if len(extras) > 1 else 0),
+             **(dict(x2=_p(x2), dx2=_p(dx2), C1=C1) if ctx.pair else {}),
              **(dict(drop_p=float(ctx.drop[0]), drop_seed=int(ctx.drop[1]), drop_seed_dev=_p(ctx.drop[2]))
                 if ctx.drop else {}))
         if rs_view is not None:
@@ -1483,7 +1530,7 @@
                      rows_per=HW, N=C, ldx=C, ldo=rs_view.stride(0))
             ctx.rsink[0].filled.add(ctx.rsink[1])
         _dbg(f'gn {name}', dy=dy, dx=dx, dres=dres)
-        return dx, dres, None, None, None, None, None, None, None, None, None
+        return dx, dres, None, None, None, None, None, None, None, None, None, dx2
 
 
 class LayerNormFn(torch.autograd.Function):
@@ -1666,7 +1713,7 @@
 
 _ST_TRAIN = bool(policy.flag('ST_TRAIN'))
 _ST_TRAIN_MIN_WGS = 200
-_ST_TRAIN_BWD = bool(policy.flag('ST_TRAIN_BWD'))
+_ST_TRAIN_BWD = policy.flag('ST_TRAIN') == 1
 _ST_WGRAD_GROUP = bool(policy.flag('ST_WGRAD_GROUP'))
 
 
@@ -1882,12 +1929,27 @@
 
     @staticmethod
     def backward(ctx, dy):
+        return ConcatFn.split(dy, ctx.ca, ctx.cb)
+
+    @staticmethod
+    def split(dy, ca, cb):
         dy = dy.contiguous()
-        da = torch.empty(dy.shape[:-1] + (ctx.ca,), dtype=dy.dtype, device=dy.device)
-        db = torch.empty(dy.shape[:-1] + (ctx.cb,), dtype=dy.dtype, device=dy.device)
+        da = torch.empty(dy.shape[:-1] + (ca,), dtype=dy.dtype, device=dy.device)
+        db = torch.empty(dy.shape[:-1] + (cb,), dtype=dy.dtype, device=dy.device)
         call('sdmi_split_channels', _st(), y=_p(dy), a=_p(da), b=_p(db), dtype=_DT[dy.dtype],
-             rows=dy.numel() // (ctx.ca + ctx.cb), Ca=ctx.ca, Cb=ctx.cb)
+             rows=dy.numel() // (ca + cb), Ca=ca, Cb=cb)
         return da, db
+
+
+class AliasCatFn(torch.autograd.Function):
+
+    @staticmethod
+    def forward(ctx, token, a, b):
+        return ops.concat_channels(a, b)
+
+    @staticmethod
+    def backward(ctx, dy):
+        return dy, None, None
 
 
 class SaAttendFn(torch.autograd.Function):
@@ -2399,6 +2461,11 @@
 
     def conv(self, x, wname, bname=None, *, kh=3, kw=3, stride=1, pad=(1, 1, 1, 1), ups=False,
              rowvec=None, residual=None, out_dtype=None, ldc=None):
+        if isinstance(x, TrainCat):
+            if x.token is not None and kh == 1 and kw == 1 and stride == 1 and not ups:
+                return GemmFn.apply(x.token, rowvec, residual, self.wb.anchor_for(wname), self.wb, wname, bname,
+                                    (kh, kw, stride, pad, ups), out_dtype, ldc, 0, (x.a, x.b))
+            x = x.materialize()
         return GemmFn.apply(x, rowvec, residual, self.wb.anchor_for(wname), self.wb, wname, bname,
                             (kh, kw, stride, pad, ups), out_dtype, ldc)
 
@@ -2414,6 +2481,8 @@
             if p > 0.0:
                 self._drop_ctr += 1
                 drop = (p, (self.seed << 20) + self._drop_ctr, getattr(self.wb.model, 'step_seed', None))
+        if isinstance(x, TrainCat):
+            x = x.materialize()
         f8 = self._f8_for(x, for_conv)
         y = GroupNormFn.apply(x, residual, self.wb.anchor_for(name), self.wb, name, eps, act, 0, drop,
                               getattr(rowsum_of, '_sdmi_sink', None), f8)
@@ -2444,6 +2513,8 @@
         if (n + '.skip_connection.weight') in self.wb.t:
             skip = self.conv(skip, n + '.skip_connection.weight', n + '.skip_connection.bias', kh=1, kw=1,
                              pad=(0, 0, 0, 0))
+        elif isinstance(skip, TrainCat):
+            skip = skip.materialize()
         return self.conv(h, n + '.out_layers.3.weight', n + '.out_layers.3.bias', residual=skip)
 
     def rowvec_slices(self, rowvecs, bounds):
@@ -2456,6 +2527,13 @@
         return list(outs)
 
     def gn_fan(self, x, name, *, eps, act=None, residual=None, n_alias=1, for_conv=None):
+        if isinstance(x, TrainCat) and x.token is None and self._f8_for(x, for_conv) is None:
+            outs = GroupNormFn.apply(x.a, residual, self.wb.anchor_for(name), self.wb, name, eps, act, n_alias, None, None,
+                                     None, x.b)
+            xa, xb = x.a.detach(), x.b.detach()
+            return (outs[0],) + tuple(TrainCat(xa, xb, t) for t in outs[1:])
+        if isinstance(x, TrainCat):
+            x = x.materialize()
         f8 = self._f8_for(x, for_conv)
         outs = GroupNormFn.apply(x, residual, self.wb.anchor_for(name), self.wb, name, eps, act, n_alias, None, None, f8)
         if f8 is not None and len(f8) > 1:
@@ -2523,6 +2601,8 @@
         return TailTokensFn.apply(x, n, L)
 
     def concat(self, a, b):
+        if lazy_cat_train_ok(a, b, fp8=bool(getattr(self.wb.model, 'fp8_unet', False))):
+            return TrainCat(a, b)
         return ConcatFn.apply(a, b)
 
     def cast(self, x, dtype):
diff --git a/slotdiffusion_amd/policy.py b/slotdiffusion_amd/policy.py
--- a/slotdiffusion_amd/policy.py
+++ b/slotdiffusion_amd/policy.py
@@ -13,14 +13,16 @@
     'DEFER_SPLITK':  (1, 'split-K second stage finished by the GroupNorm behind the convolution'),
     'LAZY_CAT':      (1, 'UNet skip concatenations read in place by their two consumers'),
     'ROLLOUT_FUSED': (1, 'fused SlotFormer rollout layer at inference (sdmi_rollout_layer: 2 launches instead of ~8)'),
-    'ST_TRAIN':      (1, 'fused training forward of the SpatialTransformer block (sdmi_st_train_fwd)'),
-    'ST_TRAIN_BWD':  (1, 'fused backward data path of that block (sdmi_st_train_bwd)'),
+    'ST_TRAIN':      (1, 'fused training form of the SpatialTransformer block -- 1: forward (sdmi_st_train_fwd) and backward '
+                         'data path (sdmi_st_train_bwd), 2: forward only, 0: off'),
     'ST_WGRAD_GROUP': (1, "the block's eight weight gradients as two grouped launches"),
     'BWD_PAIR':      (1, 'data + weight gradient of a conv / linear layer in one launch (sdmi_bwd_pair)'),
     'WGRAD_STREAM':  (1, 'stand-alone weight gradients on side HIP streams'),
     'WGRAD_HALO':    (1, 'direct 3x3 weight gradient on channel pairs where the layer leaves the pair launch'),
     'GEGLU_FUSE':    (1, 'GEGLU in the epilogue of the ff.net.0.proj GEMM (per-layer training path)'),
     'DEFER_COLSUM':  (1, 'dgamma / dbeta column sums of the whole step folded by a few grouped launches'),
+    'LAZY_CAT_TRAIN': (1, 'training: UNet skip concatenations read in place by the GroupNorm and the 1x1 skip convolution, '
+                          'their gradients written apart by the GroupNorm backward (bf16, 128-channel multiples)'),
     'DEBUG_DEFER':   (0, 'poison the outputs of deferred split-K launches until their second stage ran (tests)'),
 }
 
```

After: 2428 images/s, median of 6. About the same (+0.4%).
